# GrokImageCompression/Grok

Measured on NVIDIA H100. Metric: Mpixels/s encode+decode 8K RGB 12-bit HTJ2K; DWT HBM GB/s vs roofline, higher is better.
Workload: dtype i32

## Files before the change

### grok_b200/csrc/dwt.cu

```cuda
#include "b2k_internal.h"

namespace {

__device__ __noinline__ int mirror_rel_slow(int t, int n)
{
  if(n == 1)
    return 0;
  const int period = 2 * (n - 1);
  t %= period;
  if(t < 0)
    t += period;
  return t < n ? t : period - t;
}
__device__ __forceinline__ int mirror_rel(int t, int n)
{
  if((unsigned)t < (unsigned)n)
    return t;
  const int r = t < 0 ? -t : 2 * (n - 1) - t;
  if((unsigned)r < (unsigned)n)
    return r;
  return mirror_rel_slow(t, n);
}

__device__ __forceinline__ void load8_w32(const int32_t* __restrict__ row, int rel, int n, int (&v)[8])
{
  const int32_t* p = row + rel;
  if(rel >= 0 && rel + 8 <= n && ((reinterpret_cast<uintptr_t>(p) & 15) == 0))
  {
    const int4 a = __ldg(reinterpret_cast<const int4*>(p));
    const int4 b = __ldg(reinterpret_cast<const int4*>(p) + 1);
    v[0] = a.x; v[1] = a.y; v[2] = a.z; v[3] = a.w;
    v[4] = b.x; v[5] = b.y; v[6] = b.z; v[7] = b.w;
  }
  else
  {
#pragma unroll
    for(int i = 0; i < 8; ++i)
      v[i] = __ldg(row + mirror_rel(rel + i, n));
  }
}

__device__ __forceinline__ void load4_band(const int32_t* __restrict__ row, int k0, int kb0, int u0, int u1, int odd,
                                           int (&v)[4])
{
  const int ufirst = 2 * k0 + odd, ulast = ufirst + 6;
  const int32_t* p = row + (k0 - kb0);
  if(ufirst >= u0 && ulast < u1 && ((reinterpret_cast<uintptr_t>(p) & 15) == 0))
  {
    const int4 a = __ldg(reinterpret_cast<const int4*>(p));
    v[0] = a.x; v[1] = a.y; v[2] = a.z; v[3] = a.w;
  }
  else
  {
    const int n = u1 - u0;
#pragma unroll
    for(int i = 0; i < 4; ++i)
    {
      const int um = u0 + mirror_rel(ufirst + 2 * i - u0, n);
      v[i] = ((um & 1) == odd) ? __ldg(row + ((um >> 1) - kb0)) : 0;
    }
  }
}

struct Job
{
  int lane, ulane, jbeg, jend, wn, hn, nvalid;
  bool owner, need;
};
__device__ __forceinline__ bool decode_job(const DwtLevelDesc& D, Job& J)
{
  J.lane = threadIdx.x & 31;
  const int job = blockIdx.x * B2K_WARPS_PER_CTA + (threadIdx.x >> 5);
  if(job >= (int)D.nstrips * (int)D.nsegs)
    return false;
  const int strip = job % D.nstrips, seg = job / D.nstrips;
  J.wn = D.u1 - D.u0;
  J.hn = D.v1 - D.v0;
  J.nvalid = D.strip_w >> 3;
  J.ulane = (D.u0 & ~7) + strip * (int)D.strip_w + (J.lane - 1) * 8;
  J.owner = J.lane >= 1 && J.lane <= J.nvalid && J.ulane < D.u1;
  J.need = J.lane <= J.nvalid + 1 && J.ulane < D.u1 + 8;
  const int jlo = D.v0 >> 1, jhi = (D.v1 - 1) >> 1;
  J.jbeg = jlo + seg * (int)D.pairs_per_seg;
  J.jend = min(J.jbeg + (int)D.pairs_per_seg, jhi + 1);
  return true;
}

template <int NC, int N>
__device__ __forceinline__ void rct_fwd(const DwtLevelDesc& D, int (&x)[NC][N])
{
#pragma unroll
  for(int i = 0; i < N; ++i)
  {
    if constexpr(NC == 3)
    {
      const int r = x[0][i] + D.shift[0], g = x[1][i] + D.shift[1], b = x[2][i] + D.shift[2];
      x[0][i] = ((g + g) + b + r) >> 2;
      x[1][i] = b - g;
      x[2][i] = r - g;
    }
    else
      x[0][i] += D.shift[0];
  }
}

template <int NC, int N>
__device__ __forceinline__ void ict_fwd(const DwtLevelDesc& D, const int (&x)[NC][N], float (&out)[NC][N])
{
  const float a_r = 0.299f, a_g = 0.587f, a_b = 0.114f;
  const float cb = __fdiv_rn(0.5f, __fsub_rn(1.0f, a_b)), cr = __fdiv_rn(0.5f, __fsub_rn(1.0f, a_r));
#pragma unroll
  for(int i = 0; i < N; ++i)
  {
    if constexpr(NC == 3)
    {
      const float r = (float)(x[0][i] + D.shift[0]), g = (float)(x[1][i] + D.shift[1]), b = (float)(x[2][i] + D.shift[2]);
      const float y = __fmaf_rn(a_b, b, __fmaf_rn(a_g, g, __fmul_rn(a_r, r)));
      out[0][i] = y;
      out[1][i] = __fmul_rn(cb, __fsub_rn(b, y));
      out[2][i] = __fmul_rn(cr, __fsub_rn(r, y));
    }
    else
      out[0][i] = (float)(x[0][i] + D.shift[0]);
  }
}

template <int NC, int N>
__device__ __forceinline__ void rct_inv(const DwtLevelDesc& D, int (&x)[NC][N])
{
#pragma unroll
  for(int i = 0; i < N; ++i)
  {
    if constexpr(NC == 3)
    {
      const int y = x[0][i], u = x[1][i], w = x[2][i];
      const int gg = y - ((u + w) >> 2);
      x[0][i] = w + gg;
      x[1][i] = gg;
      x[2][i] = u + gg;
    }
#pragma unroll
    for(int c = 0; c < NC; ++c)
      x[c][i] = min(max(x[c][i] - D.shift[c], D.lo[c]), D.hi[c]);
  }
}

template <int NC, int N>
__device__ __forceinline__ void ict_inv(const DwtLevelDesc& D, const float (&x)[NC][N], int (&out)[NC][N])
{
#pragma unroll
  for(int i = 0; i < N; ++i)
  {
    float f[NC];
    if constexpr(NC == 3)
    {
      const float y = x[0][i], u = x[1][i], w = x[2][i];
      f[0] = __fmaf_rn(w, 1.402f, y);
      f[1] = __fmaf_rn(-w, 0.71414f, __fmaf_rn(-u, 0.34413f, y));
      f[2] = __fmaf_rn(u, 1.772f, y);
    }
    else
      f[0] = x[0][i];
#pragma unroll
    for(int c = 0; c < NC; ++c)
      out[c][i] = min(max(__float2int_rn(f[c]) - D.shift[c], D.lo[c]), D.hi[c]);
  }
}

template <int NC>
__device__ __forceinline__ void fetch_int_rows(const DwtLevelDesc& D, const Job& J, int v, int (&out)[NC][8])
{
  const int r = mirror_rel(v - D.v0, J.hn);
#pragma unroll
  for(int c = 0; c < NC; ++c)
  {
    if(!J.need)
    {
#pragma unroll
      for(int i = 0; i < 8; ++i)
        out[c][i] = 0;
      continue;
    }
    load8_w32(reinterpret_cast<const int32_t*>(D.in[c]) + (size_t)r * D.in_pitch, J.ulane - D.u0, J.wn, out[c]);
  }
}

template <int NC>
__device__ __forceinline__ void to_coeffs53(const DwtLevelDesc& D, int (&x)[NC][8])
{
  if(D.first_level)
    rct_fwd<NC>(D, x);
}

template <int NC>
__device__ __forceinline__ void to_coeffs97(const DwtLevelDesc& D, const int (&raw)[NC][8], float (&out)[NC][8])
{
  if(D.first_level)
    ict_fwd<NC>(D, raw, out);
  else
  {
#pragma unroll
    for(int c = 0; c < NC; ++c)
#pragma unroll
      for(int i = 0; i < 8; ++i)
        out[c][i] = __int_as_float(raw[c][i]);
  }
}

template <int NC>
__device__ __forceinline__ void fetch53(const DwtLevelDesc& D, const Job& J, int v, int (&out)[NC][8])
{
  fetch_int_rows<NC>(D, J, v, out);
  to_coeffs53<NC>(D, out);
}

template <int NC>
__device__ __forceinline__ void fetch97(const DwtLevelDesc& D, const Job& J, int v, float (&out)[NC][8])
{
  int raw[NC][8];
  fetch_int_rows<NC>(D, J, v, raw);
  to_coeffs97<NC>(D, raw, out);
}

struct BandGeom
{
  int x0l, x0h, y0l, y0h, snx, sny;
};
__device__ __forceinline__ BandGeom band_geom(const DwtLevelDesc& D)
{
  BandGeom g;
  g.x0l = (D.u0 + 1) >> 1;
  g.x0h = D.u0 >> 1;
  g.y0l = (D.v0 + 1) >> 1;
  g.y0h = D.v0 >> 1;
  g.snx = ((D.u1 + 1) >> 1) - g.x0l;
  g.sny = ((D.v1 + 1) >> 1) - g.y0l;
  return g;
}

struct StoreCtx
{
  unsigned mlo, mhi;
  bool vec_ll, vec_lo, vec_hi;
  int col_ll, col_lo, col_hi;
};
__device__ __forceinline__ StoreCtx store_ctx(const DwtLevelDesc& D, const Job& J, const BandGeom& g)
{
  StoreCtx s;
  s.mlo = s.mhi = 0;
  if(J.owner)
  {
#pragma unroll
    for(int i = 0; i < 4; ++i)
    {
      const int ue = J.ulane + 2 * i;
      if(ue >= D.u0 && ue < D.u1)
        s.mlo |= 1u << i;
      if(ue + 1 >= D.u0 && ue + 1 < D.u1)
        s.mhi |= 1u << i;
    }
  }
  const int k0 = J.ulane >> 1;
  s.col_ll = k0 - g.x0l;
  s.col_lo = k0 - g.x0l;
  s.col_hi = g.snx + k0 - g.x0h;
  const bool pitch_ok = ((D.ll_pitch | D.c_pitch) & 3u) == 0;
  s.vec_ll = pitch_ok && s.mlo == 0xF && (((reinterpret_cast<uintptr_t>(D.out_ll[0]) >> 2) + (unsigned)s.col_ll) & 3u) == 0;
  s.vec_lo = pitch_ok && s.mlo == 0xF && (((reinterpret_cast<uintptr_t>(D.out_c[0]) >> 2) + (unsigned)s.col_lo) & 3u) == 0;
  s.vec_hi = pitch_ok && s.mhi == 0xF && (((reinterpret_cast<uintptr_t>(D.out_c[0]) >> 2) + (unsigned)s.col_hi) & 3u) == 0;
  return s;
}
__device__ __forceinline__ void store4v(int32_t* __restrict__ p, const int (&v)[4], unsigned mask, bool vec)
{
  if(vec)
    *reinterpret_cast<int4*>(p) = make_int4(v[0], v[1], v[2], v[3]);
  else
  {
#pragma unroll
    for(int i = 0; i < 4; ++i)
      if(mask & (1u << i))
        p[i] = v[i];
  }
}
__device__ __forceinline__ void store_rows(const DwtLevelDesc& D, const BandGeom& g, const StoreCtx& S, int c, int j,
                                           bool vhigh, const int (&lo)[4], const int (&hi)[4])
{
  const int v = 2 * j + (vhigh ? 1 : 0);
  if(v < D.v0 || v >= D.v1 || (S.mlo | S.mhi) == 0)
    return;
  if(!vhigh)
  {
    const int r = j - g.y0l;
    store4v(reinterpret_cast<int32_t*>(D.out_ll[c]) + (r * (int)D.ll_pitch + S.col_ll), lo, S.mlo, S.vec_ll);
    store4v(reinterpret_cast<int32_t*>(D.out_c[c]) + (r * (int)D.c_pitch + S.col_hi), hi, S.mhi, S.vec_hi);
  }
  else
  {
    const int r = g.sny + j - g.y0h;
    int32_t* crow = reinterpret_cast<int32_t*>(D.out_c[c]) + r * (int)D.c_pitch;
    store4v(crow + S.col_lo, lo, S.mlo, S.vec_lo);
    store4v(crow + S.col_hi, hi, S.mhi, S.vec_hi);
  }
}

template <bool DEGEN = true>
__device__ __forceinline__ void hfwd53(const int (&r)[8], int wn, int (&lo)[4], int (&hi)[4])
{
  const int en = __shfl_down_sync(0xffffffffu, r[0], 1);
  hi[0] = r[1] - ((r[0] + r[2]) >> 1);
  hi[1] = r[3] - ((r[2] + r[4]) >> 1);
  hi[2] = r[5] - ((r[4] + r[6]) >> 1);
  hi[3] = r[7] - ((r[6] + en) >> 1);
  const int dp = __shfl_up_sync(0xffffffffu, hi[3], 1);
  lo[0] = r[0] + ((dp + hi[0] + 2) >> 2);
  lo[1] = r[2] + ((hi[0] + hi[1] + 2) >> 2);
  lo[2] = r[4] + ((hi[1] + hi[2] + 2) >> 2);
  lo[3] = r[6] + ((hi[2] + hi[3] + 2) >> 2);
  if(DEGEN && wn == 1)
  {
#pragma unroll
    for(int i = 0; i < 4; ++i)
    {
      lo[i] = r[2 * i];
      hi[i] = r[2 * i + 1] << 1;
    }
  }
}

#define F97_ALPHA (-1.586134342f)
#define F97_BETA (-0.052980118f)
#define F97_GAMMA (0.882911075f)
#define F97_DELTA (0.443506852f)
#define F97_K (1.230174105f)

__device__ __forceinline__ void hfwd97(const float (&r)[8], int wn, float invK, float deltaS, int (&lo)[4],
                                       int (&hi)[4])
{
  float e[5], d[4], s[5];
#pragma unroll
  for(int i = 0; i < 4; ++i)
    e[i] = r[2 * i];
  e[4] = __shfl_down_sync(0xffffffffu, r[0], 1);
#pragma unroll
  for(int i = 0; i < 4; ++i)
    d[i] = fmaf(e[i] + e[i + 1], F97_ALPHA, r[2 * i + 1]);
  float dm = __shfl_up_sync(0xffffffffu, d[3], 1);
  s[0] = fmaf(dm + d[0], F97_BETA, e[0]);
#pragma unroll
  for(int i = 1; i < 4; ++i)
    s[i] = fmaf(d[i - 1] + d[i], F97_BETA, e[i]);
  s[4] = __shfl_down_sync(0xffffffffu, s[0], 1);
#pragma unroll
  for(int i = 0; i < 4; ++i)
    d[i] = __fmul_rn(fmaf(s[i] + s[i + 1], F97_GAMMA, d[i]), F97_K);
  dm = __shfl_up_sync(0xffffffffu, d[3], 1);
  float o0 = __fmul_rn(fmaf(dm + d[0], deltaS, s[0]), invK);
  lo[0] = __float_as_int(o0);
#pragma unroll
  for(int i = 1; i < 4; ++i)
    lo[i] = __float_as_int(__fmul_rn(fmaf(d[i - 1] + d[i], deltaS, s[i]), invK));
#pragma unroll
  for(int i = 0; i < 4; ++i)
    hi[i] = __float_as_int(d[i]);
  if(wn == 1)
  {
#pragma unroll
    for(int i = 0; i < 4; ++i)
    {
      lo[i] = __float_as_int(r[2 * i]);
      hi[i] = __float_as_int(__fmul_rn(r[2 * i + 1], 2.0f));
    }
  }
}

__device__ __forceinline__ void cp_async16(void* smem_dst, const void* gmem_src)
{
  const unsigned s = (unsigned)__cvta_generic_to_shared(smem_dst);
  asm volatile("cp.async.cg.shared.global [%0], [%1], 16;" ::"r"(s), "l"(gmem_src) : "memory");
}
__device__ __forceinline__ void cp_async4(void* smem_dst, const void* gmem_src)
{
  const unsigned s = (unsigned)__cvta_generic_to_shared(smem_dst);
  asm volatile("cp.async.ca.shared.global [%0], [%1], 4;" ::"r"(s), "l"(gmem_src) : "memory");
}
__device__ __forceinline__ void cp_async_commit() { asm volatile("cp.async.commit_group;" ::: "memory"); }
template <int N>
__device__ __forceinline__ void cp_async_wait()
{
  asm volatile("cp.async.wait_group %0;" ::"n"(N) : "memory");
}

__device__ __forceinline__ void mbar_init(uint64_t* bar, unsigned count)
{
  asm volatile("mbarrier.init.shared::cta.b64 [%0], %1;" ::"r"((unsigned)__cvta_generic_to_shared(bar)), "r"(count) : "memory");
}
__device__ __forceinline__ void mbar_fence_init() { asm volatile("fence.mbarrier_init.release.cluster;" ::: "memory"); }
__device__ __forceinline__ void mbar_expect_tx(uint64_t* bar, unsigned bytes)
{
  asm volatile("mbarrier.arrive.expect_tx.shared::cta.b64 _, [%0], %1;" ::"r"((unsigned)__cvta_generic_to_shared(bar)), "r"(bytes)
               : "memory");
}
__device__ __forceinline__ void bulk_g2s(void* smem_dst, const void* gmem_src, unsigned bytes, uint64_t* bar)
{
  asm volatile("cp.async.bulk.shared::cluster.global.mbarrier::complete_tx::bytes [%0], [%1], %2, [%3];" ::"r"(
                   (unsigned)__cvta_generic_to_shared(smem_dst)),
               "l"(gmem_src), "r"(bytes), "r"((unsigned)__cvta_generic_to_shared(bar))
               : "memory");
}
__device__ __forceinline__ void mbar_wait(uint64_t* bar, unsigned parity)
{
  asm volatile("{\n"
               ".reg .pred p;\n"
               "MBAR_WAIT_%=:\n"
               "mbarrier.try_wait.parity.shared::cta.b64 p, [%0], %1;\n"
               "@p bra MBAR_DONE_%=;\n"
               "bra MBAR_WAIT_%=;\n"
               "MBAR_DONE_%=:\n"
               "}" ::"r"((unsigned)__cvta_generic_to_shared(bar)),
               "r"(parity)
               : "memory");
}

constexpr int DWT_STAGES = 3;

template <class Stage>
struct WarpPipe
{
  static constexpr size_t SLOT_BYTES = (size_t)B2K_WARPS_PER_CTA * DWT_STAGES * Stage::PAIRB;
  static constexpr size_t SMEM_BYTES = SLOT_BYTES + (size_t)B2K_WARPS_PER_CTA * DWT_STAGES * sizeof(uint64_t);

  uint8_t* slots;
  uint64_t* bars;
  int tfirst, tlast, tfill;
  bool bulk;

  __device__ __forceinline__ WarpPipe(uint8_t* smem, bool bulk_, int tfirst_, int tlast_)
      : slots(smem + (size_t)(threadIdx.x >> 5) * DWT_STAGES * Stage::PAIRB),
        bars(reinterpret_cast<uint64_t*>(smem + SLOT_BYTES) + (threadIdx.x >> 5) * DWT_STAGES), tfirst(tfirst_),
        tlast(tlast_), tfill(tfirst_), bulk(bulk_)
  {
  }
  template <class Bulk, class Async>
  __device__ __forceinline__ void refill(const Bulk& fill_bulk, const Async& fill_async)
  {
    if(tfill <= tlast)
    {
      const int slot = (tfill - tfirst) % DWT_STAGES;
      uint8_t* st = slots + (size_t)slot * Stage::PAIRB;
      if(bulk)
      {
        if((threadIdx.x & 31) == 0)
        {
          mbar_expect_tx(bars + slot, Stage::PAIRB);
          fill_bulk(st, tfill, bars + slot);
        }
      }
      else
        fill_async(st, tfill);
    }
    cp_async_commit();
    ++tfill;
  }
  template <class Bulk, class Async>
  __device__ __forceinline__ void prime(const Bulk& fill_bulk, const Async& fill_async)
  {
    if(bulk)
    {
      if((threadIdx.x & 31) == 0)
      {
#pragma unroll
        for(int s = 0; s < DWT_STAGES; ++s)
          mbar_init(bars + s, 1);
        mbar_fence_init();
      }
      __syncwarp();
    }
#pragma unroll
    for(int s = 0; s < DWT_STAGES - 1; ++s)
      refill(fill_bulk, fill_async);
  }
  template <class Bulk, class Async>
  __device__ __forceinline__ const uint8_t* acquire(int t, const Bulk& fill_bulk, const Async& fill_async)
  {
    if(Stage::COOPERATIVE || bulk)
      __syncwarp();
    refill(fill_bulk, fill_async);
    const int k = t - tfirst;
    if(bulk)
      mbar_wait(bars + k % DWT_STAGES, (unsigned)((k / DWT_STAGES) & 1));
    else
    {
      cp_async_wait<DWT_STAGES - 1>();
      if(Stage::COOPERATIVE)
        __syncwarp();
    }
    return slots + (size_t)(k % DWT_STAGES) * Stage::PAIRB;
  }
  __device__ __forceinline__ void drain() const { cp_async_wait<0>(); }
};

template <int NC>
struct RowStage
{
  static constexpr int ROWB = 1024;
  static constexpr int PAIRB = 2 * NC * ROWB;
  static constexpr bool COOPERATIVE = true;
  static __device__ __forceinline__ int swz(int k) { return k ^ ((k >> 3) & 1); }

  static __device__ __forceinline__ void fill(uint8_t* stage, int which, const DwtLevelDesc& D, const Job& J, int v,
                                              bool fast, unsigned fastmask, const int (&mcol)[8])
  {
    const int r = mirror_rel(v - D.v0, J.hn);
    const int rel = J.ulane - D.u0;
#pragma unroll
    for(int c = 0; c < NC; ++c)
    {
      uint8_t* dst = stage + (which * NC + c) * ROWB;
      const int32_t* row = reinterpret_cast<const int32_t*>(D.in[c]) + (size_t)r * D.in_pitch;
      const int rel0 = rel - 8 * J.lane;
#pragma unroll
      for(int h = 0; h < 2; ++h)
      {
        const int k = J.lane + 32 * h;
        if((fastmask >> (k >> 1)) & 1u)
          cp_async16(dst + swz(k) * 16, row + rel0 + 4 * k);
      }
      if(J.need && !fast)
      {
        uint8_t* d0 = dst + swz(2 * J.lane) * 16;
        uint8_t* d1 = dst + swz(2 * J.lane + 1) * 16;
#pragma unroll
        for(int i = 0; i < 4; ++i)
        {
          cp_async4(d0 + 4 * i, row + mcol[i]);
          cp_async4(d1 + 4 * i, row + mcol[4 + i]);
        }
      }
    }
  }
  static __device__ __forceinline__ void fill_bulk(uint8_t* stage, int which, const DwtLevelDesc& D, const Job& J, int v, uint64_t* bar)
  {
    const int r = mirror_rel(v - D.v0, J.hn);
    const int rel0 = J.ulane - D.u0 - 8 * J.lane;
#pragma unroll
    for(int c = 0; c < NC; ++c)
      bulk_g2s(stage + (which * NC + c) * ROWB, reinterpret_cast<const int32_t*>(D.in[c]) + (size_t)r * D.in_pitch + rel0, ROWB, bar);
  }
  static __device__ __forceinline__ void read(const uint8_t* stage, int which, const Job& J, bool linear, int (&out)[NC][8])
  {
#pragma unroll
    for(int c = 0; c < NC; ++c)
    {
      const uint8_t* row = stage + (which * NC + c) * ROWB;
      int4 a, b;
      if(linear)
      {
        a = *reinterpret_cast<const int4*>(row + J.lane * 32);
        b = *reinterpret_cast<const int4*>(row + J.lane * 32 + 16);
      }
      else
      {
        a = *reinterpret_cast<const int4*>(row + swz(2 * J.lane) * 16);
        b = *reinterpret_cast<const int4*>(row + swz(2 * J.lane + 1) * 16);
      }
      out[c][0] = a.x; out[c][1] = a.y; out[c][2] = a.z; out[c][3] = a.w;
      out[c][4] = b.x; out[c][5] = b.y; out[c][6] = b.z; out[c][7] = b.w;
    }
  }
  static __device__ __forceinline__ bool lane_fast(const DwtLevelDesc& D, const Job& J)
  {
    const int rel = J.ulane - D.u0;
    bool ok = J.need && rel >= 0 && rel + 8 <= J.wn && (D.in_pitch & 3u) == 0;
#pragma unroll
    for(int c = 0; c < NC; ++c)
      ok = ok && (((reinterpret_cast<uintptr_t>(D.in[c]) + (size_t)rel * 4) & 15) == 0);
    return ok;
  }
};

template <int NC>
__device__ __noinline__ void fwd53_degenerate_job(const DwtLevelDesc* __restrict__ dptr, const Job J)
{
  const DwtLevelDesc& D = *dptr;
  const BandGeom g = band_geom(D);
  int E[NC][8], DP[NC][8];
  {
    int A[NC][8], B[NC][8];
    fetch53<NC>(D, J, 2 * J.jbeg - 2, A);
    fetch53<NC>(D, J, 2 * J.jbeg - 1, B);
    fetch53<NC>(D, J, 2 * J.jbeg, E);
#pragma unroll
    for(int c = 0; c < NC; ++c)
#pragma unroll
      for(int i = 0; i < 8; ++i)
        DP[c][i] = B[c][i] - ((A[c][i] + E[c][i]) >> 1);
  }
  for(int j = J.jbeg; j < J.jend; ++j)
  {
    int O[NC][8], E2[NC][8];
    fetch53<NC>(D, J, 2 * j + 1, O);
    fetch53<NC>(D, J, 2 * j + 2, E2);
#pragma unroll 1
    for(int c = 0; c < NC; ++c)
    {
      int s[8], d[8];
#pragma unroll
      for(int i = 0; i < 8; ++i)
      {
        d[i] = O[c][i] - ((E[c][i] + E2[c][i]) >> 1);
        s[i] = E[c][i] + ((DP[c][i] + d[i] + 2) >> 2);
        if(J.hn == 1)
        {
          s[i] = E[c][i];
          d[i] = O[c][i] << 1;
        }
        DP[c][i] = d[i];
        E[c][i] = E2[c][i];
      }
      int lo[4], hi[4];
      hfwd53<true>(s, J.wn, lo, hi);
      store_rows(D, g, store_ctx(D, J, g), c, j, false, lo, hi);
      hfwd53<true>(d, J.wn, lo, hi);
      store_rows(D, g, store_ctx(D, J, g), c, j, true, lo, hi);
    }
  }
}

template <int NC>
__global__ void __launch_bounds__(B2K_WARPS_PER_CTA * 32) k_dwt53_fwd(const DwtLevelDesc* __restrict__ descs)
{
  extern __shared__ __align__(16) uint8_t smem_dwt[];
  typedef RowStage<NC> RS;
  const DwtLevelDesc D = descs[blockIdx.y];
  Job J;
  if(!decode_job(D, J))
    return;
  if(J.hn == 1 || J.wn == 1)
  {
    fwd53_degenerate_job<NC>(descs + blockIdx.y, J);
    return;
  }
  const BandGeom g = band_geom(D);
  const StoreCtx SC = store_ctx(D, J, g);
  const bool fast = RS::lane_fast(D, J);
  const unsigned fastmask = __ballot_sync(0xffffffffu, fast);
  int mcol[8];
#pragma unroll
  for(int i = 0; i < 8; ++i)
    mcol[i] = mirror_rel(J.ulane - D.u0 + i, J.wn);

  const int tfirst = J.jbeg - 1, tlast = J.jend - 1;
  WarpPipe<RS> pipe(smem_dwt, fastmask == 0xffffffffu, tfirst, tlast);
  auto fill_bulk = [&](uint8_t* st, int tf, uint64_t* bar) {
    RS::fill_bulk(st, 0, D, J, 2 * tf + 1, bar);
    RS::fill_bulk(st, 1, D, J, 2 * tf + 2, bar);
  };
  auto fill_async = [&](uint8_t* st, int tf) {
    RS::fill(st, 0, D, J, 2 * tf + 1, fast, fastmask, mcol);
    RS::fill(st, 1, D, J, 2 * tf + 2, fast, fastmask, mcol);
  };
  pipe.prime(fill_bulk, fill_async);
  int E[NC][8], DP[NC][8];
  fetch53<NC>(D, J, 2 * tfirst, E);
#pragma unroll
  for(int c = 0; c < NC; ++c)
#pragma unroll
    for(int i = 0; i < 8; ++i)
      DP[c][i] = 0;

  for(int t = tfirst; t <= tlast; ++t)
  {
    const uint8_t* st = pipe.acquire(t, fill_bulk, fill_async);
    int O[NC][8], E2[NC][8];
    RS::read(st, 0, J, pipe.bulk, O);
    RS::read(st, 1, J, pipe.bulk, E2);
    to_coeffs53<NC>(D, O);
    to_coeffs53<NC>(D, E2);
    const bool emit = t >= J.jbeg;
#pragma unroll
    for(int c = 0; c < NC; ++c)
    {
      int s[8], d[8];
#pragma unroll
      for(int i = 0; i < 8; ++i)
      {
        d[i] = O[c][i] - ((E[c][i] + E2[c][i]) >> 1);
        s[i] = E[c][i] + ((DP[c][i] + d[i] + 2) >> 2);
        DP[c][i] = d[i];
        E[c][i] = E2[c][i];
      }
      if(emit)
      {
        int lo[4], hi[4];
        hfwd53<false>(s, J.wn, lo, hi);
        store_rows(D, g, SC, c, t, false, lo, hi);
        hfwd53<false>(d, J.wn, lo, hi);
        store_rows(D, g, SC, c, t, true, lo, hi);
      }
    }
  }
  pipe.drain();
}

template <int NC>
__device__ __noinline__ void fwd97_degenerate_job(const DwtLevelDesc* __restrict__ dptr, const Job J)
{
  const DwtLevelDesc& D = *dptr;
  const BandGeom g = band_geom(D);
  const float invK = (float)(1.0 / 1.230174105);
  const float deltaS = __fmul_rn(F97_DELTA, invK);

  float Ev[NC][8], D1[NC][8], S1[NC][8], D2[NC][8];
  fetch97<NC>(D, J, 2 * (J.jbeg - 2), Ev);
#pragma unroll
  for(int c = 0; c < NC; ++c)
#pragma unroll
    for(int i = 0; i < 8; ++i)
      D1[c][i] = S1[c][i] = D2[c][i] = 0.f;

  for(int t = J.jbeg - 2; t <= J.jend; ++t)
  {
    float O[NC][8], E2[NC][8];
    fetch97<NC>(D, J, 2 * t + 1, O);
    fetch97<NC>(D, J, 2 * t + 2, E2);
    const bool emit = (t - 1) >= J.jbeg;
#pragma unroll
    for(int c = 0; c < NC; ++c)
    {
      float lowrow[8], highrow[8];
#pragma unroll
      for(int i = 0; i < 8; ++i)
      {
        const float d1 = fmaf(Ev[c][i] + E2[c][i], F97_ALPHA, O[c][i]);
        const float s1 = fmaf(D1[c][i] + d1, F97_BETA, Ev[c][i]);
        const float d2 = __fmul_rn(fmaf(S1[c][i] + s1, F97_GAMMA, D1[c][i]), F97_K);
        const float s2 = __fmul_rn(fmaf(D2[c][i] + d2, deltaS, S1[c][i]), invK);
        lowrow[i] = s2;
        highrow[i] = d2;
        if(J.hn == 1)
        {
          lowrow[i] = Ev[c][i];
          highrow[i] = __fmul_rn(O[c][i], 2.0f);
        }
        D2[c][i] = d2;
        D1[c][i] = d1;
        S1[c][i] = s1;
        Ev[c][i] = E2[c][i];
      }
      int lo[4], hi[4];
      hfwd97(lowrow, J.wn, invK, deltaS, lo, hi);
      if(emit)
        store_rows(D, g, store_ctx(D, J, g), c, t - 1, false, lo, hi);
      hfwd97(highrow, J.wn, invK, deltaS, lo, hi);
      if(emit)
        store_rows(D, g, store_ctx(D, J, g), c, t - 1, true, lo, hi);
    }
  }
}

template <int NC>
__global__ void __launch_bounds__(B2K_WARPS_PER_CTA * 32) k_dwt97_fwd(const DwtLevelDesc* __restrict__ descs)
{
  extern __shared__ __align__(16) uint8_t smem_dwt[];
  typedef RowStage<NC> RS;
  const DwtLevelDesc D = descs[blockIdx.y];
  Job J;
  if(!decode_job(D, J))
    return;
  if(J.hn == 1 || J.wn == 1)
  {
    fwd97_degenerate_job<NC>(descs + blockIdx.y, J);
    return;
  }
  const BandGeom g = band_geom(D);
  const StoreCtx SC = store_ctx(D, J, g);
  const bool fast = RS::lane_fast(D, J);
  const unsigned fastmask = __ballot_sync(0xffffffffu, fast);
  int mcol[8];
#pragma unroll
  for(int i = 0; i < 8; ++i)
    mcol[i] = mirror_rel(J.ulane - D.u0 + i, J.wn);
  const float invK = (float)(1.0 / 1.230174105);
  const float deltaS = __fmul_rn(F97_DELTA, invK);

  const int tfirst = J.jbeg - 2, tlast = J.jend;
  WarpPipe<RS> pipe(smem_dwt, fastmask == 0xffffffffu, tfirst, tlast);
  auto fill_bulk = [&](uint8_t* st, int tf, uint64_t* bar) {
    RS::fill_bulk(st, 0, D, J, 2 * tf + 1, bar);
    RS::fill_bulk(st, 1, D, J, 2 * tf + 2, bar);
  };
  auto fill_async = [&](uint8_t* st, int tf) {
    RS::fill(st, 0, D, J, 2 * tf + 1, fast, fastmask, mcol);
    RS::fill(st, 1, D, J, 2 * tf + 2, fast, fastmask, mcol);
  };
  pipe.prime(fill_bulk, fill_async);
  float Ev[NC][8], D1[NC][8], S1[NC][8], D2[NC][8];
  fetch97<NC>(D, J, 2 * tfirst, Ev);
#pragma unroll
  for(int c = 0; c < NC; ++c)
#pragma unroll
    for(int i = 0; i < 8; ++i)
      D1[c][i] = S1[c][i] = D2[c][i] = 0.f;

  for(int t = tfirst; t <= tlast; ++t)
  {
    const uint8_t* st = pipe.acquire(t, fill_bulk, fill_async);
    float O[NC][8], E2[NC][8];
    {
      int raw[NC][8];
      RS::read(st, 0, J, pipe.bulk, raw);
      to_coeffs97<NC>(D, raw, O);
      RS::read(st, 1, J, pipe.bulk, raw);
      to_coeffs97<NC>(D, raw, E2);
    }
    const bool emit = (t - 1) >= J.jbeg;
#pragma unroll
    for(int c = 0; c < NC; ++c)
    {
      float lowrow[8], highrow[8];
#pragma unroll
      for(int i = 0; i < 8; ++i)
      {
        const float d1 = fmaf(Ev[c][i] + E2[c][i], F97_ALPHA, O[c][i]);
        const float s1 = fmaf(D1[c][i] + d1, F97_BETA, Ev[c][i]);
        const float d2 = __fmul_rn(fmaf(S1[c][i] + s1, F97_GAMMA, D1[c][i]), F97_K);
        const float s2 = __fmul_rn(fmaf(D2[c][i] + d2, deltaS, S1[c][i]), invK);
        lowrow[i] = s2;
        highrow[i] = d2;
        D2[c][i] = d2;
        D1[c][i] = d1;
        S1[c][i] = s1;
        Ev[c][i] = E2[c][i];
      }
      if(emit)
      {
        int lo[4], hi[4];
        hfwd97(lowrow, 2, invK, deltaS, lo, hi);
        store_rows(D, g, SC, c, t - 1, false, lo, hi);
        hfwd97(highrow, 2, invK, deltaS, lo, hi);
        store_rows(D, g, SC, c, t - 1, true, lo, hi);
      }
    }
  }
  pipe.drain();
}

template <int NC>
__device__ __forceinline__ void fetch_band_rows(const DwtLevelDesc& D, const Job& J, const BandGeom& g, int j,
                                                bool vhigh, int (&lo)[NC][4], int (&hi)[NC][4])
{
  const int vm = D.v0 + mirror_rel(2 * j + (vhigh ? 1 : 0) - D.v0, J.hn);
  const int jm = vm >> 1;
  const int k0 = J.ulane >> 1;
#pragma unroll
  for(int c = 0; c < NC; ++c)
  {
    if(!J.need || (vm & 1) != (vhigh ? 1 : 0))
    {
#pragma unroll
      for(int i = 0; i < 4; ++i)
        lo[c][i] = hi[c][i] = 0;
      continue;
    }
    const int32_t* lrow;
    const int32_t* hrow;
    if(!vhigh)
    {
      lrow = reinterpret_cast<const int32_t*>(D.out_ll[c]) + (size_t)(jm - g.y0l) * D.ll_pitch;
      hrow = reinterpret_cast<const int32_t*>(D.out_c[c]) + (size_t)(jm - g.y0l) * D.c_pitch + g.snx;
    }
    else
    {
      lrow = reinterpret_cast<const int32_t*>(D.out_c[c]) + (size_t)(g.sny + jm - g.y0h) * D.c_pitch;
      hrow = lrow + g.snx;
    }
    load4_band(lrow, k0, g.x0l, D.u0, D.u1, 0, lo[c]);
    load4_band(hrow, k0, g.x0h, D.u0, D.u1, 1, hi[c]);
  }
}

template <bool DEGEN = true>
__device__ __forceinline__ void hinv53(const int (&lo)[4], const int (&hi)[4], int wn, int (&r)[8])
{
  const int dm = __shfl_up_sync(0xffffffffu, hi[3], 1);
  int e[5];
  e[0] = lo[0] - ((dm + hi[0] + 2) >> 2);
  e[1] = lo[1] - ((hi[0] + hi[1] + 2) >> 2);
  e[2] = lo[2] - ((hi[1] + hi[2] + 2) >> 2);
  e[3] = lo[3] - ((hi[2] + hi[3] + 2) >> 2);
  e[4] = __shfl_down_sync(0xffffffffu, e[0], 1);
#pragma unroll
  for(int i = 0; i < 4; ++i)
  {
    r[2 * i] = e[i];
    r[2 * i + 1] = hi[i] + ((e[i] + e[i + 1]) >> 1);
  }
  if(DEGEN && wn == 1)
  {
#pragma unroll
    for(int i = 0; i < 4; ++i)
    {
      r[2 * i] = lo[i];
      r[2 * i + 1] = hi[i] >> 1;
    }
  }
}

__device__ __forceinline__ void hinv97(const int (&loi)[4], const int (&hii)[4], int wn, float (&r)[8])
{
  const float K = 1.230174105f, twice_invK = 1.625732422f;
  float s[5], d[4];
#pragma unroll
  for(int i = 0; i < 4; ++i)
  {
    s[i] = __fmul_rn(__int_as_float(loi[i]), K);
    d[i] = __fmul_rn(__int_as_float(hii[i]), twice_invK);
  }
  float dm = __shfl_up_sync(0xffffffffu, d[3], 1);
  s[0] = fmaf(dm + d[0], -0.443506852f, s[0]);
#pragma unroll
  for(int i = 1; i < 4; ++i)
    s[i] = fmaf(d[i - 1] + d[i], -0.443506852f, s[i]);
  s[4] = __shfl_down_sync(0xffffffffu, s[0], 1);
#pragma unroll
  for(int i = 0; i < 4; ++i)
    d[i] = fmaf(s[i] + s[i + 1], -0.882911075f, d[i]);
  dm = __shfl_up_sync(0xffffffffu, d[3], 1);
  s[0] = fmaf(dm + d[0], 0.052980118f, s[0]);
#pragma unroll
  for(int i = 1; i < 4; ++i)
    s[i] = fmaf(d[i - 1] + d[i], 0.052980118f, s[i]);
  s[4] = __shfl_down_sync(0xffffffffu, s[0], 1);
#pragma unroll
  for(int i = 0; i < 4; ++i)
  {
    r[2 * i] = s[i];
    r[2 * i + 1] = fmaf(s[i] + s[i + 1], 1.586134342f, d[i]);
  }
  if(wn == 1)
  {
#pragma unroll
    for(int i = 0; i < 4; ++i)
    {
      r[2 * i] = __int_as_float(loi[i]);
      r[2 * i + 1] = __int_as_float(hii[i]);
    }
  }
}

struct OutCtx
{
  unsigned m;
  bool vec;
  int col;
};
__device__ __forceinline__ OutCtx out_ctx(const DwtLevelDesc& D, const Job& J)
{
  OutCtx o;
  o.m = 0;
  if(J.owner)
  {
#pragma unroll
    for(int i = 0; i < 8; ++i)
      if(J.ulane + i >= D.u0 && J.ulane + i < D.u1)
        o.m |= 1u << i;
  }
  o.col = J.ulane - D.u0;
  o.vec = o.m == 0xFF && (D.in_pitch & 3u) == 0 && (((reinterpret_cast<uintptr_t>(D.in[0]) >> 2) + (unsigned)o.col) & 3u) == 0;
  return o;
}
template <int NC>
__device__ __forceinline__ void store_out_rows(const DwtLevelDesc& D, const OutCtx& O, int v, const int (&x)[NC][8])
{
#pragma unroll
  for(int c = 0; c < NC; ++c)
  {
    int32_t* p = reinterpret_cast<int32_t*>(const_cast<void*>(D.in[c])) + ((v - D.v0) * (int)D.in_pitch + O.col);
    if(O.vec)
    {
      reinterpret_cast<int4*>(p)[0] = make_int4(x[c][0], x[c][1], x[c][2], x[c][3]);
      reinterpret_cast<int4*>(p)[1] = make_int4(x[c][4], x[c][5], x[c][6], x[c][7]);
    }
    else
    {
#pragma unroll
      for(int i = 0; i < 8; ++i)
        if(O.m & (1u << i))
          p[i] = x[c][i];
    }
  }
}
template <int NC>
__device__ __forceinline__ void store_rows53(const DwtLevelDesc& D, const OutCtx& O, int v, int (&x)[NC][8])
{
  if(v < D.v0 || v >= D.v1 || O.m == 0)
    return;
  if(D.first_level)
    rct_inv<NC>(D, x);
  store_out_rows<NC>(D, O, v, x);
}
template <int NC>
__device__ __forceinline__ void store_rows97(const DwtLevelDesc& D, const OutCtx& O, int v, const float (&x)[NC][8])
{
  if(v < D.v0 || v >= D.v1 || O.m == 0)
    return;
  int o[NC][8];
  if(D.first_level)
    ict_inv<NC>(D, x, o);
  else
  {
#pragma unroll
    for(int c = 0; c < NC; ++c)
#pragma unroll
      for(int i = 0; i < 8; ++i)
        o[c][i] = __float_as_int(x[c][i]);
  }
  store_out_rows<NC>(D, O, v, o);
}

template <int NC>
__device__ __noinline__ void inv53_degenerate_job(const DwtLevelDesc* __restrict__ dptr, const Job J)
{
  const DwtLevelDesc& D = *dptr;
  const BandGeom g = band_geom(D);
  int DV[NC][8], EP[NC][8];
#pragma unroll
  for(int c = 0; c < NC; ++c)
#pragma unroll
    for(int i = 0; i < 8; ++i)
      DV[c][i] = EP[c][i] = 0;

  for(int t = J.jbeg - 1; t <= J.jend; ++t)
  {
    int lo[NC][4], hi[NC][4];
    int sv[NC][8], dv[NC][8];
    fetch_band_rows<NC>(D, J, g, t, false, lo, hi);
#pragma unroll
    for(int c = 0; c < NC; ++c)
      hinv53(lo[c], hi[c], J.wn, sv[c]);
    fetch_band_rows<NC>(D, J, g, t, true, lo, hi);
#pragma unroll
    for(int c = 0; c < NC; ++c)
      hinv53(lo[c], hi[c], J.wn, dv[c]);
    int Er[NC][8], Or[NC][8];
#pragma unroll
    for(int c = 0; c < NC; ++c)
#pragma unroll
      for(int i = 0; i < 8; ++i)
      {
        const int e = sv[c][i] - ((DV[c][i] + dv[c][i] + 2) >> 2);
        Or[c][i] = DV[c][i] + ((EP[c][i] + e) >> 1);
        Er[c][i] = EP[c][i];
        EP[c][i] = e;
        DV[c][i] = dv[c][i];
      }
    if(J.hn == 1)
    {
      if(t >= J.jbeg && t < J.jend)
      {
        int hv[NC][8];
#pragma unroll
        for(int c = 0; c < NC; ++c)
#pragma unroll
          for(int i = 0; i < 8; ++i)
            hv[c][i] = dv[c][i] >> 1;
        store_rows53<NC>(D, out_ctx(D, J), 2 * t, sv);
        store_rows53<NC>(D, out_ctx(D, J), 2 * t + 1, hv);
      }
    }
    else if(t - 1 >= J.jbeg)
    {
      store_rows53<NC>(D, out_ctx(D, J), 2 * (t - 1), Er);
      store_rows53<NC>(D, out_ctx(D, J), 2 * (t - 1) + 1, Or);
    }
  }
}


template <int NC>
struct BandStage
{
  static constexpr int ROWB = 512;
  static constexpr int PAIRB = 4 * NC * ROWB;
  static constexpr bool COOPERATIVE = false;
  struct Lane
  {
    bool need;
    bool fast[4];
    int col[4];
    int mlo[4], mhi[4];
  };
  static __device__ __forceinline__ void setup(const DwtLevelDesc& D, const Job& J, const BandGeom& g, Lane& L)
  {
    const int k0 = J.ulane >> 1;
    L.need = J.need;
#pragma unroll
    for(int i = 0; i < 4; ++i)
    {
      const int ul = D.u0 + mirror_rel(2 * (k0 + i) - D.u0, J.wn), uh = D.u0 + mirror_rel(2 * (k0 + i) + 1 - D.u0, J.wn);
      L.mlo[i] = (ul >> 1) - g.x0l;
      L.mhi[i] = (uh >> 1) - g.x0h;
    }
    const bool in_lo = 2 * k0 >= D.u0 && 2 * k0 + 6 < D.u1, in_hi = 2 * k0 + 1 >= D.u0 && 2 * k0 + 7 < D.u1;
    const int clo = k0 - g.x0l, chi = k0 - g.x0h;
    L.col[0] = clo; L.col[1] = g.snx + chi; L.col[2] = clo; L.col[3] = g.snx + chi;
    const bool pitch_ok = ((D.ll_pitch | D.c_pitch) & 3u) == 0;
    L.fast[0] = J.need && pitch_ok && in_lo && (((reinterpret_cast<uintptr_t>(D.out_ll[0]) >> 2) + (unsigned)clo) & 3u) == 0;
    L.fast[1] = J.need && pitch_ok && in_hi && (((reinterpret_cast<uintptr_t>(D.out_c[0]) >> 2) + (unsigned)(g.snx + chi)) & 3u) == 0;
    L.fast[2] = J.need && pitch_ok && in_lo && (((reinterpret_cast<uintptr_t>(D.out_c[0]) >> 2) + (unsigned)clo) & 3u) == 0;
    L.fast[3] = L.fast[1];
  }
  static __device__ __forceinline__ void fill(uint8_t* stage, const DwtLevelDesc& D, const Job& J, const BandGeom& g,
                                              const Lane& L, int t)
  {
    if(!L.need)
      return;
    const int jl = ((D.v0 + mirror_rel(2 * t - D.v0, J.hn)) >> 1), jh = ((D.v0 + mirror_rel(2 * t + 1 - D.v0, J.hn)) >> 1);
#pragma unroll
    for(int c = 0; c < NC; ++c)
    {
      const int32_t* src[4];
      src[0] = reinterpret_cast<const int32_t*>(D.out_ll[c]) + (jl - g.y0l) * (int)D.ll_pitch;
      src[1] = reinterpret_cast<const int32_t*>(D.out_c[c]) + (jl - g.y0l) * (int)D.c_pitch;
      src[2] = reinterpret_cast<const int32_t*>(D.out_c[c]) + (g.sny + jh - g.y0h) * (int)D.c_pitch;
      src[3] = src[2];
#pragma unroll
      for(int b = 0; b < 4; ++b)
      {
        uint8_t* dst = stage + (b * NC + c) * ROWB + J.lane * 16;
        if(L.fast[b])
          cp_async16(dst, src[b] + L.col[b]);
        else
        {
          const int base = (b & 1) ? g.snx : 0;
#pragma unroll
          for(int i = 0; i < 4; ++i)
            cp_async4(dst + 4 * i, src[b] + base + ((b & 1) ? L.mhi[i] : L.mlo[i]));
        }
      }
    }
  }
  static __device__ __forceinline__ void fill_bulk(uint8_t* stage, const DwtLevelDesc& D, const Job& J, const BandGeom& g,
                                                   const Lane& L, int t, uint64_t* bar)
  {
    const int jl = ((D.v0 + mirror_rel(2 * t - D.v0, J.hn)) >> 1), jh = ((D.v0 + mirror_rel(2 * t + 1 - D.v0, J.hn)) >> 1);
#pragma unroll
    for(int c = 0; c < NC; ++c)
    {
      const int32_t* src[4];
      src[0] = reinterpret_cast<const int32_t*>(D.out_ll[c]) + (jl - g.y0l) * (int)D.ll_pitch;
      src[1] = reinterpret_cast<const int32_t*>(D.out_c[c]) + (jl - g.y0l) * (int)D.c_pitch;
      src[2] = reinterpret_cast<const int32_t*>(D.out_c[c]) + (g.sny + jh - g.y0h) * (int)D.c_pitch;
      src[3] = src[2];
#pragma unroll
      for(int b = 0; b < 4; ++b)
        bulk_g2s(stage + (b * NC + c) * ROWB, src[b] + L.col[b], ROWB, bar);
    }
  }
  static __device__ __forceinline__ bool all_fast(const Lane& L)
  {
    return __all_sync(0xffffffffu, L.fast[0] && L.fast[1] && L.fast[2] && L.fast[3]);
  }
  static __device__ __forceinline__ void read(const uint8_t* stage, const Job& J, int b, int c, int (&v)[4])
  {
    const int4 a = *reinterpret_cast<const int4*>(stage + (b * NC + c) * ROWB + J.lane * 16);
    v[0] = a.x; v[1] = a.y; v[2] = a.z; v[3] = a.w;
  }
};

template <int NC>
__global__ void __launch_bounds__(B2K_WARPS_PER_CTA * 32) k_dwt53_inv(const DwtLevelDesc* __restrict__ descs)
{
  extern __shared__ __align__(16) uint8_t smem_dwt[];
  typedef BandStage<NC> BS;
  const DwtLevelDesc D = descs[blockIdx.y];
  Job J;
  if(!decode_job(D, J))
    return;
  if(J.hn == 1 || J.wn == 1)
  {
    inv53_degenerate_job<NC>(descs + blockIdx.y, J);
    return;
  }
  const BandGeom g = band_geom(D);
  typename BS::Lane L;
  BS::setup(D, J, g, L);
  const OutCtx OC = out_ctx(D, J);

  const int tfirst = J.jbeg - 1, tlast = J.jend;
  WarpPipe<BS> pipe(smem_dwt, BS::all_fast(L), tfirst, tlast);
  auto fill_bulk = [&](uint8_t* st, int tf, uint64_t* bar) { BS::fill_bulk(st, D, J, g, L, tf, bar); };
  auto fill_async = [&](uint8_t* st, int tf) { BS::fill(st, D, J, g, L, tf); };
  pipe.prime(fill_bulk, fill_async);
  int DV[NC][8], EP[NC][8];
#pragma unroll
  for(int c = 0; c < NC; ++c)
#pragma unroll
    for(int i = 0; i < 8; ++i)
      DV[c][i] = EP[c][i] = 0;

  for(int t = tfirst; t <= tlast; ++t)
  {
    const uint8_t* st = pipe.acquire(t, fill_bulk, fill_async);
    int Er[NC][8], Or[NC][8];
#pragma unroll
    for(int c = 0; c < NC; ++c)
    {
      int lo[4], hi[4], sv[8], dv[8];
      BS::read(st, J, 0, c, lo);
      BS::read(st, J, 1, c, hi);
      hinv53<false>(lo, hi, J.wn, sv);
      BS::read(st, J, 2, c, lo);
      BS::read(st, J, 3, c, hi);
      hinv53<false>(lo, hi, J.wn, dv);
#pragma unroll
      for(int i = 0; i < 8; ++i)
      {
        const int e = sv[i] - ((DV[c][i] + dv[i] + 2) >> 2);
        Or[c][i] = DV[c][i] + ((EP[c][i] + e) >> 1);
        Er[c][i] = EP[c][i];
        EP[c][i] = e;
        DV[c][i] = dv[i];
      }
    }
    if(t - 1 >= J.jbeg)
    {
      store_rows53<NC>(D, OC, 2 * (t - 1), Er);
      store_rows53<NC>(D, OC, 2 * (t - 1) + 1, Or);
    }
  }
  pipe.drain();
}

template <int NC>
__device__ __noinline__ void inv97_degenerate_job(const DwtLevelDesc* __restrict__ dptr, const Job J)
{
  const DwtLevelDesc& D = *dptr;
  const BandGeom g = band_geom(D);
  const float K = 1.230174105f, twice_invK = 1.625732422f;
  float D0[NC][8], S1[NC][8], D1[NC][8], S2[NC][8];
#pragma unroll
  for(int c = 0; c < NC; ++c)
#pragma unroll
    for(int i = 0; i < 8; ++i)
      D0[c][i] = S1[c][i] = D1[c][i] = S2[c][i] = 0.f;

  for(int t = J.jbeg - 2; t <= J.jend + 1; ++t)
  {
    int lo[NC][4], hi[NC][4];
    float sv[NC][8], dv[NC][8];
    fetch_band_rows<NC>(D, J, g, t, false, lo, hi);
#pragma unroll
    for(int c = 0; c < NC; ++c)
      hinv97(lo[c], hi[c], J.wn, sv[c]);
    fetch_band_rows<NC>(D, J, g, t, true, lo, hi);
#pragma unroll
    for(int c = 0; c < NC; ++c)
      hinv97(lo[c], hi[c], J.wn, dv[c]);
    float Er[NC][8], Or[NC][8];
#pragma unroll
    for(int c = 0; c < NC; ++c)
#pragma unroll
      for(int i = 0; i < 8; ++i)
      {
        const float s0 = __fmul_rn(sv[c][i], K), d0 = __fmul_rn(dv[c][i], twice_invK);
        const float s1 = fmaf(D0[c][i] + d0, -0.443506852f, s0);
        const float d1 = fmaf(S1[c][i] + s1, -0.882911075f, D0[c][i]);
        const float s2 = fmaf(D1[c][i] + d1, 0.052980118f, S1[c][i]);
        const float d2 = fmaf(S2[c][i] + s2, 1.586134342f, D1[c][i]);
        Er[c][i] = S2[c][i];
        Or[c][i] = d2;
        D0[c][i] = d0;
        S1[c][i] = s1;
        D1[c][i] = d1;
        S2[c][i] = s2;
      }
    if(J.hn == 1)
    {
      if(t >= J.jbeg && t < J.jend)
      {
        store_rows97<NC>(D, out_ctx(D, J), 2 * t, sv);
        store_rows97<NC>(D, out_ctx(D, J), 2 * t + 1, dv);
      }
    }
    else if(t - 2 >= J.jbeg)
    {
      store_rows97<NC>(D, out_ctx(D, J), 2 * (t - 2), Er);
      store_rows97<NC>(D, out_ctx(D, J), 2 * (t - 2) + 1, Or);
    }
  }
}

template <int NC>
__global__ void __launch_bounds__(B2K_WARPS_PER_CTA * 32) k_dwt97_inv(const DwtLevelDesc* __restrict__ descs)
{
  extern __shared__ __align__(16) uint8_t smem_dwt[];
  typedef BandStage<NC> BS;
  const DwtLevelDesc D = descs[blockIdx.y];
  Job J;
  if(!decode_job(D, J))
    return;
  if(J.hn == 1 || J.wn == 1)
  {
    inv97_degenerate_job<NC>(descs + blockIdx.y, J);
    return;
  }
  const BandGeom g = band_geom(D);
  typename BS::Lane L;
  BS::setup(D, J, g, L);
  const OutCtx OC = out_ctx(D, J);
  const float K = 1.230174105f, twice_invK = 1.625732422f;

  const int tfirst = J.jbeg - 2, tlast = J.jend + 1;
  WarpPipe<BS> pipe(smem_dwt, BS::all_fast(L), tfirst, tlast);
  auto fill_bulk = [&](uint8_t* st, int tf, uint64_t* bar) { BS::fill_bulk(st, D, J, g, L, tf, bar); };
  auto fill_async = [&](uint8_t* st, int tf) { BS::fill(st, D, J, g, L, tf); };
  pipe.prime(fill_bulk, fill_async);
  float D0[NC][8], S1[NC][8], D1[NC][8], S2[NC][8];
#pragma unroll
  for(int c = 0; c < NC; ++c)
#pragma unroll
    for(int i = 0; i < 8; ++i)
      D0[c][i] = S1[c][i] = D1[c][i] = S2[c][i] = 0.f;

  for(int t = tfirst; t <= tlast; ++t)
  {
    const uint8_t* st = pipe.acquire(t, fill_bulk, fill_async);
    float Er[NC][8], Or[NC][8];
#pragma unroll
    for(int c = 0; c < NC; ++c)
    {
      int lo[4], hi[4];
      float sv[8], dv[8];
      BS::read(st, J, 0, c, lo);
      BS::read(st, J, 1, c, hi);
      hinv97(lo, hi, 2, sv);
      BS::read(st, J, 2, c, lo);
      BS::read(st, J, 3, c, hi);
      hinv97(lo, hi, 2, dv);
#pragma unroll
      for(int i = 0; i < 8; ++i)
      {
        const float s0 = __fmul_rn(sv[i], K), d0 = __fmul_rn(dv[i], twice_invK);
        const float s1 = fmaf(D0[c][i] + d0, -0.443506852f, s0);
        const float d1 = fmaf(S1[c][i] + s1, -0.882911075f, D0[c][i]);
        const float s2 = fmaf(D1[c][i] + d1, 0.052980118f, S1[c][i]);
        const float d2 = fmaf(S2[c][i] + s2, 1.586134342f, D1[c][i]);
        Er[c][i] = S2[c][i];
        Or[c][i] = d2;
        D0[c][i] = d0;
        S1[c][i] = s1;
        D1[c][i] = d1;
        S2[c][i] = s2;
      }
    }
    if(t - 2 >= J.jbeg)
    {
      store_rows97<NC>(D, OC, 2 * (t - 2), Er);
      store_rows97<NC>(D, OC, 2 * (t - 2) + 1, Or);
    }
  }
  pipe.drain();
}

template <int S> struct Sample;
template <> struct Sample<1> { typedef uint8_t U; typedef int8_t I; };
template <> struct Sample<2> { typedef uint16_t U; typedef int16_t I; };
template <> struct Sample<4> { typedef uint32_t U; typedef int32_t I; };

template <int S>
__device__ __forceinline__ int widen_sample(uint32_t u, int sgnd)
{
  if constexpr(S == 4)
    return (int)u;
  else
  {
    u &= (1u << (8 * S)) - 1;
    return sgnd ? (int)(typename Sample<S>::I)u : (int)u;
  }
}

template <int BYTES>
__device__ __forceinline__ void load_group(const void* p, uint32_t (&wd)[BYTES / 4])
{
  if constexpr(BYTES % 16 == 0)
  {
#pragma unroll
    for(int i = 0; i < BYTES / 16; ++i)
    {
      const uint4 a = __ldg(reinterpret_cast<const uint4*>(p) + i);
      wd[4 * i] = a.x; wd[4 * i + 1] = a.y; wd[4 * i + 2] = a.z; wd[4 * i + 3] = a.w;
    }
  }
  else
  {
#pragma unroll
    for(int i = 0; i < BYTES / 8; ++i)
    {
      const uint2 a = __ldg(reinterpret_cast<const uint2*>(p) + i);
      wd[2 * i] = a.x; wd[2 * i + 1] = a.y;
    }
  }
}
template <int BYTES>
__device__ __forceinline__ void store_group(void* p, const uint32_t (&wd)[BYTES / 4])
{
  if constexpr(BYTES % 16 == 0)
  {
#pragma unroll
    for(int i = 0; i < BYTES / 16; ++i)
      reinterpret_cast<uint4*>(p)[i] = make_uint4(wd[4 * i], wd[4 * i + 1], wd[4 * i + 2], wd[4 * i + 3]);
  }
  else
  {
#pragma unroll
    for(int i = 0; i < BYTES / 8; ++i)
      reinterpret_cast<uint2*>(p)[i] = make_uint2(wd[2 * i], wd[2 * i + 1]);
  }
}

struct Ptr4
{
  int32_t* p[4];
};
struct CPtr4
{
  const int32_t* p[4];
};

template <int S, int NC>
__global__ void __launch_bounds__(128) k_container_to_planes(const void* __restrict__ src, uint32_t spitch, uint32_t step, Ptr4 dst,
                                                             uint32_t dpitch, uint32_t w, uint32_t h, int sgnd)
{
  typedef typename Sample<S>::U U;
  constexpr int BYTES = 8 * NC * S, V = BYTES % 16 == 0 ? 16 : 8;
  const uint32_t x8 = (blockIdx.x * blockDim.x + threadIdx.x) * 8;
  if(x8 >= w)
    return;
  for(uint32_t y = blockIdx.y; y < h; y += gridDim.y)
  {
    const U* s = static_cast<const U*>(src) + (size_t)y * spitch + (size_t)x8 * step;
    const size_t doff = (size_t)y * dpitch + x8;
    bool vec = x8 + 8 <= w && step == NC && (reinterpret_cast<uintptr_t>(s) & (V - 1)) == 0;
#pragma unroll
    for(int c = 0; c < NC; ++c)
      vec = vec && (reinterpret_cast<uintptr_t>(dst.p[c] + doff) & 15) == 0;
    if(vec)
    {
      uint32_t wd[BYTES / 4];
      load_group<BYTES>(s, wd);
#pragma unroll
      for(int c = 0; c < NC; ++c)
      {
        int v[8];
#pragma unroll
        for(int i = 0; i < 8; ++i)
        {
          const int e = (i * NC + c) * S;
          v[i] = widen_sample<S>(wd[e >> 2] >> ((e & 3) * 8), sgnd);
        }
        int4* d = reinterpret_cast<int4*>(dst.p[c] + doff);
        d[0] = make_int4(v[0], v[1], v[2], v[3]);
        d[1] = make_int4(v[4], v[5], v[6], v[7]);
      }
    }
    else
    {
      const uint32_t n = w - x8 < 8 ? w - x8 : 8;
#pragma unroll 1
      for(uint32_t i = 0; i < n; ++i)
#pragma unroll
        for(int c = 0; c < NC; ++c)
          dst.p[c][doff + i] = widen_sample<S>(s[(size_t)i * step + c], sgnd);
    }
  }
}

template <int S, int NC>
__global__ void __launch_bounds__(128) k_planes_to_container(CPtr4 src, uint32_t spitch, void* __restrict__ dst, uint32_t dpitch,
                                                             uint32_t step, uint32_t w, uint32_t h)
{
  typedef typename Sample<S>::U U;
  constexpr int BYTES = 8 * NC * S, V = BYTES % 16 == 0 ? 16 : 8;
  constexpr uint32_t MASK = S == 4 ? 0xFFFFFFFFu : (1u << (8 * S)) - 1;
  const uint32_t x8 = (blockIdx.x * blockDim.x + threadIdx.x) * 8;
  if(x8 >= w)
    return;
  for(uint32_t y = blockIdx.y; y < h; y += gridDim.y)
  {
    const size_t soff = (size_t)y * spitch + x8;
    U* d = static_cast<U*>(dst) + (size_t)y * dpitch + (size_t)x8 * step;
    bool vec = x8 + 8 <= w && step == NC && (reinterpret_cast<uintptr_t>(d) & (V - 1)) == 0;
#pragma unroll
    for(int c = 0; c < NC; ++c)
      vec = vec && (reinterpret_cast<uintptr_t>(src.p[c] + soff) & 15) == 0;
    if(vec)
    {
      uint32_t wd[BYTES / 4];
#pragma unroll
      for(int k = 0; k < BYTES / 4; ++k)
        wd[k] = 0;
#pragma unroll
      for(int c = 0; c < NC; ++c)
      {
        const int4 a = __ldg(reinterpret_cast<const int4*>(src.p[c] + soff)), b = __ldg(reinterpret_cast<const int4*>(src.p[c] + soff) + 1);
        const int v[8] = {a.x, a.y, a.z, a.w, b.x, b.y, b.z, b.w};
#pragma unroll
        for(int i = 0; i < 8; ++i)
        {
          const int e = (i * NC + c) * S;
          wd[e >> 2] |= ((uint32_t)v[i] & MASK) << ((e & 3) * 8);
        }
      }
      store_group<BYTES>(d, wd);
    }
    else
    {
      const uint32_t n = w - x8 < 8 ? w - x8 : 8;
#pragma unroll 1
      for(uint32_t i = 0; i < n; ++i)
#pragma unroll
        for(int c = 0; c < NC; ++c)
          d[(size_t)i * step + c] = (U)src.p[c][soff + i];
    }
  }
}

dim3 convert_grid(uint32_t w, uint32_t h) { return dim3((w + 8 * 128 - 1) / (8 * 128), h < 65535u ? h : 65535u); }

template <int S>
void launch_container_to_planes(const void* src, uint32_t spitch, uint32_t step, const Ptr4& P, int nc, uint32_t dpitch, uint32_t w,
                                uint32_t h, int sgnd, cudaStream_t st)
{
  const dim3 grid = convert_grid(w, h), block(128);
  switch(nc)
  {
    case 1: k_container_to_planes<S, 1><<<grid, block, 0, st>>>(src, spitch, step, P, dpitch, w, h, sgnd); break;
    case 2: k_container_to_planes<S, 2><<<grid, block, 0, st>>>(src, spitch, step, P, dpitch, w, h, sgnd); break;
    case 3: k_container_to_planes<S, 3><<<grid, block, 0, st>>>(src, spitch, step, P, dpitch, w, h, sgnd); break;
    default: k_container_to_planes<S, 4><<<grid, block, 0, st>>>(src, spitch, step, P, dpitch, w, h, sgnd); break;
  }
}
template <int S>
void launch_planes_to_container(const CPtr4& P, int nc, uint32_t spitch, void* dst, uint32_t dpitch, uint32_t step, uint32_t w,
                                uint32_t h, cudaStream_t st)
{
  const dim3 grid = convert_grid(w, h), block(128);
  switch(nc)
  {
    case 1: k_planes_to_container<S, 1><<<grid, block, 0, st>>>(P, spitch, dst, dpitch, step, w, h); break;
    case 2: k_planes_to_container<S, 2><<<grid, block, 0, st>>>(P, spitch, dst, dpitch, step, w, h); break;
    case 3: k_planes_to_container<S, 3><<<grid, block, 0, st>>>(P, spitch, dst, dpitch, step, w, h); break;
    default: k_planes_to_container<S, 4><<<grid, block, 0, st>>>(P, spitch, dst, dpitch, step, w, h); break;
  }
}

}

void b2k_launch_container_to_planes(const void* src, uint32_t spitch, uint32_t step, uint32_t sample_bytes, int32_t* const* dst, int nc,
                                    uint32_t dpitch, uint32_t w, uint32_t h, int sgnd, cudaStream_t st)
{
  if(!w || !h)
    return;
  Ptr4 P{};
  for(int c = 0; c < nc && c < 4; ++c)
    P.p[c] = dst[c];
  switch(sample_bytes)
  {
    case 1: launch_container_to_planes<1>(src, spitch, step, P, nc, dpitch, w, h, sgnd, st); break;
    case 2: launch_container_to_planes<2>(src, spitch, step, P, nc, dpitch, w, h, sgnd, st); break;
    default: launch_container_to_planes<4>(src, spitch, step, P, nc, dpitch, w, h, sgnd, st); break;
  }
  b2k_count_launch();
}
void b2k_launch_planes_to_container(const int32_t* const* src, int nc, uint32_t spitch, void* dst, uint32_t dpitch, uint32_t step,
                                    uint32_t sample_bytes, uint32_t w, uint32_t h, cudaStream_t st)
{
  if(!w || !h)
    return;
  CPtr4 P{};
  for(int c = 0; c < nc && c < 4; ++c)
    P.p[c] = src[c];
  switch(sample_bytes)
  {
    case 1: launch_planes_to_container<1>(P, nc, spitch, dst, dpitch, step, w, h, st); break;
    case 2: launch_planes_to_container<2>(P, nc, spitch, dst, dpitch, step, w, h, st); break;
    default: launch_planes_to_container<4>(P, nc, spitch, dst, dpitch, step, w, h, st); break;
  }
  b2k_count_launch();
}

template <class Stage, void (*KERNEL)(const DwtLevelDesc*)>
static void launch_dwt(dim3 grid, dim3 block, cudaStream_t st, const DwtLevelDesc* d)
{
  const size_t smem = WarpPipe<Stage>::SMEM_BYTES;
  static DeviceOnce once;
  once.run([&] { cudaFuncSetAttribute(KERNEL, cudaFuncAttributeMaxDynamicSharedMemorySize, (int)smem); });
  KERNEL<<<grid, block, smem, st>>>(d);
}

void b2k_launch_dwt_fwd(const DwtLevelDesc* d, int ndesc, int max_jobs, int nc, bool irreversible, cudaStream_t st)
{
  if(ndesc <= 0 || max_jobs <= 0)
    return;
  dim3 grid((max_jobs + B2K_WARPS_PER_CTA - 1) / B2K_WARPS_PER_CTA, ndesc), block(B2K_WARPS_PER_CTA * 32);
  if(!irreversible)
  {
    if(nc == 3) launch_dwt<RowStage<3>, k_dwt53_fwd<3>>(grid, block, st, d);
    else launch_dwt<RowStage<1>, k_dwt53_fwd<1>>(grid, block, st, d);
  }
  else
  {
    if(nc == 3) launch_dwt<RowStage<3>, k_dwt97_fwd<3>>(grid, block, st, d);
    else launch_dwt<RowStage<1>, k_dwt97_fwd<1>>(grid, block, st, d);
  }
  b2k_count_launch();
}

template <int NC, bool IRREV, bool FWD>
__global__ void k_point_transform(const DwtLevelDesc* __restrict__ descs, int ndesc)
{
  for(int di = blockIdx.z; di < ndesc; di += gridDim.z)
  {
  const DwtLevelDesc& D = descs[di];
  const int w = D.u1 - D.u0, h = D.v1 - D.v0;
  const int x = blockIdx.x * blockDim.x + threadIdx.x;
  if(x >= w)
    continue;
  for(int y = blockIdx.y; y < h; y += gridDim.y)
  {
  const size_t ii = (size_t)y * D.in_pitch + x, oi = (size_t)y * D.c_pitch + x;
  if(FWD)
  {
    int v[NC][1];
#pragma unroll
    for(int c = 0; c < NC; ++c)
      v[c][0] = static_cast<const int32_t*>(D.in[c])[ii];
    if(!IRREV)
    {
      rct_fwd<NC>(D, v);
#pragma unroll
      for(int c = 0; c < NC; ++c)
        static_cast<int32_t*>(D.out_c[c])[oi] = v[c][0];
    }
    else
    {
      float f[NC][1];
      ict_fwd<NC>(D, v, f);
#pragma unroll
      for(int c = 0; c < NC; ++c)
        static_cast<float*>(D.out_c[c])[oi] = f[c][0];
    }
  }
  else
  {
    int o[NC][1];
    if(!IRREV)
    {
#pragma unroll
      for(int c = 0; c < NC; ++c)
        o[c][0] = static_cast<const int32_t*>(D.out_c[c])[oi];
      rct_inv<NC>(D, o);
    }
    else
    {
      float f[NC][1];
#pragma unroll
      for(int c = 0; c < NC; ++c)
        f[c][0] = static_cast<const float*>(D.out_c[c])[oi];
      ict_inv<NC>(D, f, o);
    }
#pragma unroll
    for(int c = 0; c < NC; ++c)
      static_cast<int32_t*>(const_cast<void*>(D.in[c]))[ii] = o[c][0];
  }
  }
  }
}

void b2k_launch_point_transform(const DwtLevelDesc* d, int ndesc, uint32_t max_w, uint32_t max_h, int nc, bool irreversible,
                                bool forward, cudaStream_t st)
{
  if(ndesc <= 0 || !max_w || !max_h)
    return;
  dim3 grid((max_w + 127) / 128, std::min<uint32_t>(max_h, 65535u), (unsigned)std::min(ndesc, 65535)), block(128);
#define B2K_PT(NC_, IR_, FW_) k_point_transform<NC_, IR_, FW_><<<grid, block, 0, st>>>(d, ndesc)
  if(nc == 3)
  {
    if(irreversible) { if(forward) B2K_PT(3, true, true); else B2K_PT(3, true, false); }
    else { if(forward) B2K_PT(3, false, true); else B2K_PT(3, false, false); }
  }
  else
  {
    if(irreversible) { if(forward) B2K_PT(1, true, true); else B2K_PT(1, true, false); }
    else { if(forward) B2K_PT(1, false, true); else B2K_PT(1, false, false); }
  }
#undef B2K_PT
  b2k_count_launch();
}

void b2k_launch_dwt_inv(const DwtLevelDesc* d, int ndesc, int max_jobs, int nc, bool irreversible, cudaStream_t st)
{
  if(ndesc <= 0 || max_jobs <= 0)
    return;
  dim3 grid((max_jobs + B2K_WARPS_PER_CTA - 1) / B2K_WARPS_PER_CTA, ndesc), block(B2K_WARPS_PER_CTA * 32);
  if(!irreversible)
  {
    if(nc == 3) launch_dwt<BandStage<3>, k_dwt53_inv<3>>(grid, block, st, d);
    else launch_dwt<BandStage<1>, k_dwt53_inv<1>>(grid, block, st, d);
  }
  else
  {
    if(nc == 3) launch_dwt<BandStage<3>, k_dwt97_inv<3>>(grid, block, st, d);
    else launch_dwt<BandStage<1>, k_dwt97_inv<1>>(grid, block, st, d);
  }
  b2k_count_launch();
}
```

### grok_b200/csrc/engine.cu

```cuda
#include <algorithm>
#include <atomic>
#include <chrono>
#include <cstdio>
#include <cstdlib>
#include <cstring>
#include <functional>
#include <map>
#include <mutex>
#include <unordered_map>
#include <string>
#include <vector>

#include "b2k_internal.h"
#include "geometry.h"

using namespace b2k;

static thread_local std::string g_err;
static std::atomic<uint64_t> g_launches{0};
static std::atomic<int> g_pack_policy{-1};
static std::atomic<int> g_last_pack[2]{{-1}, {-1}};
void b2k_count_launch(void) { g_launches.fetch_add(1, std::memory_order_relaxed); }

#define CUDA_TRY(expr)                                                                             \
  do                                                                                               \
  {                                                                                                \
    cudaError_t _e = (expr);                                                                       \
    if(_e != cudaSuccess)                                                                          \
    {                                                                                              \
      g_err = std::string(#expr) + ": " + cudaGetErrorString(_e);                                  \
      return -1;                                                                                   \
    }                                                                                              \
  } while(0)

struct b2k_engine
{
  int device = 0;
  cudaStream_t stream = nullptr, copy_stream = nullptr, h2d_stream = nullptr;
  cudaStream_t aux[4] = {nullptr, nullptr, nullptr, nullptr};
  cudaDeviceProp prop{};
  std::mutex mu;
  b2k_device_job* cached = nullptr;
  cudaEvent_t caller_ev = nullptr;
};

namespace {
struct DevCache
{
  std::mutex mu;
  std::multimap<size_t, void*> free_;
  std::unordered_map<void*, size_t> live;
  size_t cached = 0;
};
DevCache g_devcache[32];
size_t dev_cache_limit()
{
  static const size_t v = [] {
    const char* e = getenv("B2K_DEV_CACHE_GB");
    return (size_t)(e ? atof(e) : 16.0) << 30;
  }();
  return v;
}
cudaError_t dev_alloc(void** p, size_t n)
{
  int dev = 0;
  cudaGetDevice(&dev);
  DevCache& C = g_devcache[dev & 31];
  const size_t gran = std::max<size_t>(256u << 10, n >> 4);
  const size_t want = (n + gran - 1) / gran * gran;
  {
    std::lock_guard<std::mutex> lk(C.mu);
    auto it = C.free_.lower_bound(want);
    if(it != C.free_.end() && it->first <= want + want / 4)
    {
      *p = it->second;
      C.live[*p] = it->first;
      C.cached -= it->first;
      C.free_.erase(it);
      return cudaSuccess;
    }
  }
  cudaError_t e = cudaMalloc(p, want);
  if(e != cudaSuccess)
  {
    (void)cudaGetLastError();
    std::vector<void*> drop;
    {
      std::lock_guard<std::mutex> lk(C.mu);
      for(auto& kv : C.free_)
        drop.push_back(kv.second);
      C.free_.clear();
      C.cached = 0;
    }
    for(void* q : drop)
      cudaFree(q);
    e = cudaMalloc(p, want);
  }
  if(e == cudaSuccess)
  {
    std::lock_guard<std::mutex> lk(C.mu);
    C.live[*p] = want;
  }
  return e;
}
cudaError_t dev_free(void* p)
{
  if(!p)
    return cudaSuccess;
  int dev = 0;
  cudaGetDevice(&dev);
  DevCache& C = g_devcache[dev & 31];
  std::vector<void*> drop;
  {
    std::lock_guard<std::mutex> lk(C.mu);
    auto it = C.live.find(p);
    if(it == C.live.end())
      drop.push_back(p);
    else
    {
      C.free_.insert({it->second, p});
      C.cached += it->second;
      C.live.erase(it);
      while(C.cached > dev_cache_limit() && !C.free_.empty())
      {
        auto big = std::prev(C.free_.end());
        drop.push_back(big->second);
        C.cached -= big->first;
        C.free_.erase(big);
      }
    }
  }
  for(void* q : drop)
    cudaFree(q);
  return cudaSuccess;
}
}
template <class T>
static inline cudaError_t dev_alloc_t(T** p, size_t n) { return dev_alloc(reinterpret_cast<void**>(p), n); }

namespace {
struct HostCache
{
  std::mutex mu;
  std::multimap<size_t, void*> free_;
  std::unordered_map<void*, size_t> live;
  size_t cached = 0;
} g_hostcache;
cudaError_t host_alloc(void** p, size_t n)
{
  const size_t gran = std::max<size_t>(64u << 10, n >> 4);
  const size_t want = (n + gran - 1) / gran * gran;
  {
    std::lock_guard<std::mutex> lk(g_hostcache.mu);
    auto it = g_hostcache.free_.lower_bound(want);
    if(it != g_hostcache.free_.end() && it->first <= want + want / 4)
    {
      *p = it->second;
      g_hostcache.live[*p] = it->first;
      g_hostcache.cached -= it->first;
      g_hostcache.free_.erase(it);
      return cudaSuccess;
    }
  }
  const cudaError_t e = cudaHostAlloc(p, want, cudaHostAllocDefault);
  if(e == cudaSuccess)
  {
    std::lock_guard<std::mutex> lk(g_hostcache.mu);
    g_hostcache.live[*p] = want;
  }
  return e;
}
cudaError_t host_free(void* p)
{
  if(!p)
    return cudaSuccess;
  std::vector<void*> drop;
  {
    std::lock_guard<std::mutex> lk(g_hostcache.mu);
    auto it = g_hostcache.live.find(p);
    if(it == g_hostcache.live.end())
      drop.push_back(p);
    else
    {
      g_hostcache.free_.insert({it->second, p});
      g_hostcache.cached += it->second;
      g_hostcache.live.erase(it);
      while(g_hostcache.cached > ((size_t)8 << 30) && !g_hostcache.free_.empty())
      {
        auto big = std::prev(g_hostcache.free_.end());
        drop.push_back(big->second);
        g_hostcache.cached -= big->first;
        g_hostcache.free_.erase(big);
      }
    }
  }
  for(void* q : drop)
    cudaFreeHost(q);
  return cudaSuccess;
}
}
template <class T>
static inline cudaError_t host_alloc_t(T** p, size_t n) { return host_alloc(reinterpret_cast<void**>(p), n); }
#define cudaMalloc(p, n) dev_alloc_t((p), (n))
#define cudaFree(p) dev_free((void*)(p))
#define cudaHostAlloc(p, n, flags) host_alloc_t((p), (n))
#define cudaFreeHost(p) host_free((void*)(p))

struct Planes
{
  int32_t* base = nullptr;
  uint32_t pitch = 0, rows = 0;
  uint32_t X0 = 0, Y0 = 0;
  int n = 0;
  size_t plane_elems() const { return (size_t)pitch * rows; }
  int32_t* at(int c, uint32_t x, uint32_t y) const { return base + (size_t)c * plane_elems() + (size_t)(y - Y0) * pitch + (x - X0); }
};

static int alloc_planes(Planes& p, int n, uint32_t cx0, uint32_t cy0, uint32_t cx1, uint32_t cy1)
{
  p.n = n;
  p.X0 = cx0 & ~31u;
  p.Y0 = cy0;
  p.pitch = ((cx1 - p.X0) + 31u + 32u) & ~31u;
  p.rows = (cy1 - cy0) + 2;
  CUDA_TRY(cudaMalloc(&p.base, (size_t)n * p.plane_elems() * sizeof(int32_t)));
  CUDA_TRY(cudaMemset(p.base, 0, (size_t)n * p.plane_elems() * sizeof(int32_t)));
  return 0;
}

struct LevelLaunch
{
  std::vector<DwtLevelDesc> descs;
  DwtLevelDesc* d_descs = nullptr;
  int nc = 1, max_jobs = 0;
  bool point = false;
  uint32_t max_w = 0, max_h = 0;
  uint64_t alg_bytes = 0;
  std::vector<uint32_t> tile_first;
};

#define B2K_MAX_CHUNKS 32
#define CEV(purpose, k) ((purpose) * (B2K_MAX_CHUNKS + 1) + (int)(k))

struct PackTuner
{
  int calls = 0;
  double best[2] = {1e30, 1e30};
  double recent = 0;
  int choice = -1;
  bool probing_other = false;
  bool next_mode()
  {
    if(choice < 0)
      return (calls & 1) == 0;
    probing_other = (calls % 64) == 63;
    return probing_other ? !choice : (choice != 0);
  }
  void record(bool packed, double ms)
  {
    ++calls;
    if(choice < 0)
    {
      if(calls > 1 || !packed)
        best[packed ? 1 : 0] = std::min(best[packed ? 1 : 0], ms);
      if(calls >= 6)
      {
        choice = best[1] < best[0] ? 1 : 0;
        recent = best[choice];
      }
      return;
    }
    if(probing_other)
    {
      if(ms < 0.9 * recent)
      {
        choice = packed ? 1 : 0;
        recent = ms;
      }
      probing_other = false;
      return;
    }
    recent = 0.9 * recent + 0.1 * ms;
  }
};

struct b2k_device_job
{
  b2k_engine* eng = nullptr;
  b2k_coding cp{};
  uint32_t tile_mod = 1, tile_rem = 0;
  TileGrid grid{};
  std::vector<uint32_t> tiles;
  std::vector<Rect> tile_rects;
  std::vector<BandQuant> quant;
  std::vector<b2k_block> blocks;
  std::vector<uint32_t> coded_index;
  std::vector<float> dec_quant;
  std::vector<uint32_t> coded_first;
  std::vector<uint32_t> chunk_tile;
  cudaEvent_t chunk_ev[4 * (B2K_MAX_CHUNKS + 1)]{};
  uint32_t max_cblk_w = 0;
  HtEncodeLimits enc_limits{0, 0};

  Planes img, coef, ll[2];
  uint16_t* d_stage = nullptr;
  std::vector<LevelLaunch> fwd, inv;
  HtBlockDesc* d_enc_desc = nullptr;
  HtBlockDesc* d_dec_desc = nullptr;
  std::vector<HtBlockDesc> h_enc_desc;
  HtBlockDesc* h_dec_desc = nullptr;
  HtBlockOut* d_out = nullptr;
  uint64_t* d_offsets = nullptr;
  uint32_t* d_recs = nullptr;
  float* d_dec_quant = nullptr;
  HtBlockOut* d_dec_status = nullptr;
  uint64_t total_quads = 0, group_quads = 0;
  uint8_t* d_scratch = nullptr;
  uint64_t scratch_bytes = 0;
  uint8_t* d_bytes = nullptr;
  uint64_t bytes_cap = 0, bytes_used = 0;
  int* d_err = nullptr;
  HtBlockOut* h_out = nullptr;
  uint64_t* h_offsets = nullptr;
  cudaEvent_t ev[8]{};
  float last_level1_ms = 0.f, last_inv_level1_ms = 0.f;
  uint64_t level1_alg_bytes = 0;
  uint16_t* h_ring = nullptr;
  uint32_t ring_slots = 0;
  uint64_t ring_slot_elems = 0, ring_elems = 0;
  cudaEvent_t ring_ev[16]{};
  PackTuner tune_enc, tune_dec;
  std::vector<cudaEvent_t> q_ev;
  std::vector<cudaEvent_t> p_ev;
  std::vector<cudaStream_t> p_streams;
  bool dec_has_refinement = false;
};

extern "C" const char* b2k_last_error(void) { return g_err.c_str(); }
void b2k_set_error(const char* msg) { g_err = msg ? msg : ""; }
extern "C" uint64_t b2k_launch_count(void) { return g_launches.load(); }

extern "C" int32_t b2k_engine_create(int32_t device, b2k_engine** out)
{
  if(!out)
    return -1;
  *out = nullptr;
  int n = 0;
  cudaError_t e = cudaGetDeviceCount(&n);
  if(e != cudaSuccess || n == 0)
  {
    g_err = std::string("no CUDA device: ") + cudaGetErrorString(e) +
            " (this engine has no CPU path; the host keeps its own)";
    return -1;
  }
  if(device < 0 || device >= n)
  {
    g_err = "device index out of range";
    return -1;
  }
  CUDA_TRY(cudaSetDevice(device));
  b2k_engine* eng = new b2k_engine();
  eng->device = device;
  CUDA_TRY(cudaGetDeviceProperties(&eng->prop, device));
  CUDA_TRY(cudaStreamCreateWithFlags(&eng->stream, cudaStreamNonBlocking));
  CUDA_TRY(cudaStreamCreateWithFlags(&eng->copy_stream, cudaStreamNonBlocking));
  CUDA_TRY(cudaStreamCreateWithFlags(&eng->h2d_stream, cudaStreamNonBlocking));
  for(cudaStream_t& a : eng->aux)
    CUDA_TRY(cudaStreamCreateWithFlags(&a, cudaStreamNonBlocking));
  CUDA_TRY(cudaEventCreateWithFlags(&eng->caller_ev, cudaEventDisableTiming));
  *out = eng;
  return 0;
}

extern "C" void b2k_engine_destroy(b2k_engine* e)
{
  if(!e)
    return;
  cudaSetDevice(e->device);
  if(e->cached)
  {
    b2k_job_destroy(e->cached);
    e->cached = nullptr;
  }
  if(e->stream)
    cudaStreamDestroy(e->stream);
  if(e->copy_stream)
    cudaStreamDestroy(e->copy_stream);
  if(e->h2d_stream)
    cudaStreamDestroy(e->h2d_stream);
  for(cudaStream_t a : e->aux)
    if(a)
      cudaStreamDestroy(a);
  if(e->caller_ev)
    cudaEventDestroy(e->caller_ev);
  delete e;
}

extern "C" void* b2k_host_alloc(size_t bytes)
{
  void* p = nullptr;
  if(cudaHostAlloc(&p, bytes, cudaHostAllocDefault) != cudaSuccess)
    return nullptr;
  return p;
}
extern "C" int32_t b2k_set_host_threads(int32_t n)
{
  b2k_host_set_threads(n);
  g_pack_policy.store(n < 0 ? -1 : n == 0 ? 0 : 1);
  return b2k_host_threads();
}

extern "C" int32_t b2k_host_pack_last(int32_t decode) { return g_last_pack[decode ? 1 : 0].load(); }

extern "C" void b2k_host_free(void* p)
{
  if(p)
    cudaFreeHost(p);
}

extern "C" int64_t b2k_enumerate(const b2k_coding* cp, uint32_t tile_mod, uint32_t tile_rem, b2k_block* out, uint64_t cap)
{
  if(!cp || tile_mod == 0)
    return -1;
  if(const char* why = unsupported_reason(*cp))
  {
    g_err = why;
    return -1;
  }
  const TileGrid g = tile_grid(*cp);
  const std::vector<BandQuant> q = band_quant(*cp);
  std::vector<b2k_block> v;
  for(uint32_t t = 0; t < g.nx * g.ny; ++t)
    if(t % tile_mod == tile_rem)
      enumerate_tile_blocks(*cp, t, tile_rect(*cp, g, t), q, v);
  for(uint64_t i = 0; i < v.size() && i < cap; ++i)
    out[i] = v[i];
  return (int64_t)v.size();
}

static void fill_strips(DwtLevelDesc& d, int pairs_per_seg)
{
  const int span = d.u1 - (d.u0 & ~7);
  const int nstrips = std::max(1, (span + 239) / 240);
  int sw = (span + nstrips - 1) / nstrips;
  sw = (sw + 7) & ~7;
  d.nstrips = (uint16_t)nstrips;
  d.strip_w = (uint16_t)sw;
  const int npairs = ((d.v1 - 1) >> 1) - (d.v0 >> 1) + 1;
  d.pairs_per_seg = (uint16_t)pairs_per_seg;
  d.nsegs = (uint16_t)((npairs + pairs_per_seg - 1) / pairs_per_seg);
}

static int upload_descs(LevelLaunch& L)
{
  L.max_jobs = 0;
  for(const DwtLevelDesc& d : L.descs)
    L.max_jobs = std::max(L.max_jobs, (int)d.nstrips * (int)d.nsegs);
  if(L.descs.empty())
    return 0;
  CUDA_TRY(cudaMalloc(&L.d_descs, L.descs.size() * sizeof(DwtLevelDesc)));
  CUDA_TRY(cudaMemcpy(L.d_descs, L.descs.data(), L.descs.size() * sizeof(DwtLevelDesc), cudaMemcpyHostToDevice));
  return 0;
}

static int build_dwt_plan(b2k_device_job* J)
{
  const b2k_coding& cp = J->cp;
  const int L = cp.numres - 1;
  const int ncomp = cp.numcomps;
  const int pairs53 = 32, pairs97 = 32;
  const int P = cp.irreversible ? pairs97 : pairs53;
  const int32_t dc = cp.sgnd ? 0 : -(1 << (cp.prec - 1));
  const int32_t lo = cp.sgnd ? -(1 << (cp.prec - 1)) : 0, hi = cp.sgnd ? (1 << (cp.prec - 1)) - 1 : (1 << cp.prec) - 1;

  if(L == 0)
  {
    for(int dir = 0; dir < 2; ++dir)
    {
      std::vector<LevelLaunch>& out = dir == 0 ? J->fwd : J->inv;
      LevelLaunch mctL, sglL;
      mctL.nc = 3;
      sglL.nc = 1;
      mctL.point = sglL.point = true;
      for(size_t ti = 0; ti < J->tiles.size(); ++ti)
      {
        mctL.tile_first.push_back((uint32_t)mctL.descs.size());
        sglL.tile_first.push_back((uint32_t)sglL.descs.size());
        const Rect tc = J->tile_rects[ti];
        if(tc.empty())
          continue;
        for(int c = 0; c < ncomp;)
        {
          const bool group = cp.mct && c == 0;
          const int nc = group ? 3 : 1;
          LevelLaunch& LL = group ? mctL : sglL;
          DwtLevelDesc d{};
          d.u0 = (int32_t)tc.x0; d.v0 = (int32_t)tc.y0; d.u1 = (int32_t)tc.x1; d.v1 = (int32_t)tc.y1;
          d.first_level = 1;
          d.comp0 = (uint8_t)c;
          for(int k = 0; k < nc; ++k)
          {
            d.in[k] = J->img.at(c + k, tc.x0, tc.y0);
            d.in_pitch = J->img.pitch;
            d.out_c[k] = J->coef.at(c + k, tc.x0, tc.y0);
            d.out_ll[k] = d.out_c[k];
            d.c_pitch = d.ll_pitch = J->coef.pitch;
            d.shift[k] = dc;
            d.lo[k] = lo;
            d.hi[k] = hi;
          }
          LL.descs.push_back(d);
          LL.max_w = std::max(LL.max_w, tc.w());
          LL.max_h = std::max(LL.max_h, tc.h());
          LL.alg_bytes += (uint64_t)tc.w() * tc.h() * nc * 8;
          c += nc;
        }
      }
      mctL.tile_first.push_back((uint32_t)mctL.descs.size());
      sglL.tile_first.push_back((uint32_t)sglL.descs.size());
      if(!mctL.descs.empty()) out.push_back(std::move(mctL));
      if(!sglL.descs.empty()) out.push_back(std::move(sglL));
      for(LevelLaunch& Lh : out)
      {
        Lh.max_jobs = 1;
        if(upload_descs(Lh))
          return -1;
      }
    }
    return 0;
  }
  for(int dir = 0; dir < 2; ++dir)
  {
    std::vector<LevelLaunch>& out = dir == 0 ? J->fwd : J->inv;
    for(int lvl = 1; lvl <= L; ++lvl)
    {
      const int resno = cp.numres - lvl;
      LevelLaunch mctL, sglL;
      mctL.nc = 3;
      sglL.nc = 1;
      for(size_t ti = 0; ti < J->tiles.size(); ++ti)
      {
        mctL.tile_first.push_back((uint32_t)mctL.descs.size());
        sglL.tile_first.push_back((uint32_t)sglL.descs.size());
        const Rect tc = J->tile_rects[ti];
        const Rect r = resolution_rect(tc, cp.numres, resno);
        if(r.empty())
          continue;
        for(int c = 0; c < ncomp;)
        {
          const bool group = (lvl == 1 && cp.mct && c == 0);
          const int nc = group ? 3 : 1;
          DwtLevelDesc d{};
          d.u0 = (int32_t)r.x0; d.v0 = (int32_t)r.y0; d.u1 = (int32_t)r.x1; d.v1 = (int32_t)r.y1;
          d.first_level = lvl == 1;
          d.comp0 = (uint8_t)c;
          const uint32_t llx = (r.x0 + 1) >> 1, lly = (r.y0 + 1) >> 1;
          for(int k = 0; k < nc; ++k)
          {
            const int cc = c + k;
            const Planes& fine = (lvl == 1) ? J->img : J->ll[(lvl - 1) & 1];
            d.in[k] = fine.at(cc, r.x0, r.y0);
            d.in_pitch = fine.pitch;
            d.out_c[k] = J->coef.at(cc, tc.x0, tc.y0);
            d.c_pitch = J->coef.pitch;
            if(lvl == L)
            {
              d.out_ll[k] = d.out_c[k];
              d.ll_pitch = J->coef.pitch;
            }
            else
            {
              const Planes& coarse = J->ll[lvl & 1];
              d.out_ll[k] = coarse.at(cc, llx, lly);
              d.ll_pitch = coarse.pitch;
            }
            d.shift[k] = dc;
            d.lo[k] = lo;
            d.hi[k] = hi;
          }
          fill_strips(d, P);
          (group ? mctL : sglL).descs.push_back(d);
          const uint64_t samples = (uint64_t)r.w() * r.h() * nc;
          (group ? mctL : sglL).alg_bytes += samples * 8;
          c += nc;
        }
      }
      mctL.tile_first.push_back((uint32_t)mctL.descs.size());
      sglL.tile_first.push_back((uint32_t)sglL.descs.size());
      for(LevelLaunch* LL : {&mctL, &sglL})
      {
        int Pl = P;
        auto jobs = [&] {
          uint64_t n = 0;
          for(const DwtLevelDesc& d : LL->descs)
            n += (uint64_t)d.nstrips * d.nsegs;
          return n;
        };
        while(!LL->descs.empty() && Pl > 8 && jobs() < 3552)
        {
          Pl >>= 1;
          for(DwtLevelDesc& d : LL->descs)
            fill_strips(d, Pl);
        }
      }
      if(dir == 0)
      {
        if(!mctL.descs.empty()) out.push_back(std::move(mctL));
        if(!sglL.descs.empty()) out.push_back(std::move(sglL));
      }
      else
      {
        if(!sglL.descs.empty()) out.insert(out.begin(), std::move(sglL));
        if(!mctL.descs.empty()) out.insert(out.begin(), std::move(mctL));
      }
    }
    for(LevelLaunch& Lh : out)
      if(upload_descs(Lh))
        return -1;
  }
  return 0;
}

static uint32_t slot_capacity(uint32_t w, uint32_t h, uint32_t kmax)
{
  const uint64_t samples = (uint64_t)w * h, quads = (uint64_t)((w + 1) / 2) * ((h + 1) / 2);
  const uint64_t ms = (samples * (kmax + 2) + 6) / 7 + 16;
  const uint64_t vlc = (quads * 15 + 6) / 7 + 16;
  return (uint32_t)((ms + vlc + 256 + 15) & ~15ull);
}

static int build_block_plan(b2k_device_job* J)
{
  const b2k_coding& cp = J->cp;
  J->blocks.clear();
  for(size_t ti = 0; ti < J->tiles.size(); ++ti)
    enumerate_tile_blocks(cp, J->tiles[ti], J->tile_rects[ti], J->quant, J->blocks);
  std::vector<Rect> rect_of(J->grid.nx * J->grid.ny);
  for(size_t ti = 0; ti < J->tiles.size(); ++ti)
    rect_of[J->tiles[ti]] = J->tile_rects[ti];
  uint64_t off = 0;
  std::vector<uint32_t> sel_of(J->grid.nx * J->grid.ny, 0);
  for(size_t ti = 0; ti < J->tiles.size(); ++ti)
    sel_of[J->tiles[ti]] = (uint32_t)ti;
  J->coded_first.assign(J->tiles.size() + 1, 0);
  for(uint32_t i = 0; i < J->blocks.size(); ++i)
  {
    const b2k_block& b = J->blocks[i];
    if(b.x1 <= b.x0 || b.y1 <= b.y0)
      continue;
    J->coded_first[sel_of[b.tile] + 1] = (uint32_t)J->h_enc_desc.size() + 1;
    const Rect& tr = rect_of[b.tile];
    const BandQuant& bq = J->quant[band_quant_index(b.resno, b.orient)];
    HtBlockDesc d{};
    d.coef = J->coef.at(b.comp, tr.x0 + b.buf_x, tr.y0 + b.buf_y);
    d.pitch = J->coef.pitch;
    d.w = (uint16_t)(b.x1 - b.x0);
    d.h = (uint16_t)(b.y1 - b.y0);
    d.kmax = bq.kmax;
    d.irreversible = cp.irreversible;
    d.quant = 1.0f / bq.step_enc;
    d.slot_cap = slot_capacity(d.w, d.h, bq.kmax);
    d.slot_off = off;
    off += d.slot_cap;
    {
      const size_t j = J->h_enc_desc.size() & 31u;
      const uint64_t quads = (uint64_t)((d.w + 1) / 2) * ((d.h + 1) / 2);
      if(j == 0)
      {
        J->total_quads += 32 * J->group_quads;
        J->group_quads = 0;
      }
      J->group_quads = std::max(J->group_quads, quads);
      d.rec_off = (uint32_t)(J->total_quads + j);
    }
    J->max_cblk_w = std::max<uint32_t>(J->max_cblk_w, d.w);
    J->enc_limits.stage_words = std::max(J->enc_limits.stage_words, b2k_ht_encode_stage_words(d.w));
    J->enc_limits.max_kmax = std::max<uint32_t>(J->enc_limits.max_kmax, d.kmax);
    J->h_enc_desc.push_back(d);
    J->dec_quant.push_back(bq.step_dec / (float)(1u << (31 - bq.kmax)));
    J->coded_index.push_back(i);
  }
  J->scratch_bytes = off;
  for(size_t ti = 1; ti <= J->tiles.size(); ++ti)
    J->coded_first[ti] = std::max(J->coded_first[ti], J->coded_first[ti - 1]);
  {
    const uint32_t nt = (uint32_t)J->tiles.size();
    uint32_t want = 8;
    if(const char* ev = getenv("B2K_CHUNKS"))
      want = (uint32_t)std::max(1, std::min(B2K_MAX_CHUNKS, atoi(ev)));
    const uint32_t nchunks = std::max(1u, std::min(want, nt));
    J->chunk_tile.clear();
    for(uint32_t k = 0; k <= nchunks; ++k)
      J->chunk_tile.push_back((uint32_t)((uint64_t)k * nt / nchunks));
  }
  const size_t n = J->h_enc_desc.size();
  if(n)
  {
    CUDA_TRY(cudaMalloc(&J->d_enc_desc, n * sizeof(HtBlockDesc)));
    CUDA_TRY(cudaMemcpy(J->d_enc_desc, J->h_enc_desc.data(), n * sizeof(HtBlockDesc), cudaMemcpyHostToDevice));
    CUDA_TRY(cudaMalloc(&J->d_dec_desc, n * sizeof(HtBlockDesc)));
    CUDA_TRY(cudaMalloc(&J->d_out, n * sizeof(HtBlockOut)));
    CUDA_TRY(cudaMalloc(&J->d_offsets, (n + 1) * sizeof(uint64_t)));
    CUDA_TRY(cudaMemset(J->d_offsets, 0, (n + 1) * sizeof(uint64_t)));
    CUDA_TRY(cudaMalloc(&J->d_scratch, J->scratch_bytes + 64));
    CUDA_TRY(cudaMalloc(&J->d_recs, (J->total_quads + 32 * J->group_quads + 64) * sizeof(uint32_t)));
    CUDA_TRY(cudaMalloc(&J->d_dec_status, n * sizeof(HtBlockOut)));
    CUDA_TRY(cudaMalloc(&J->d_dec_quant, n * sizeof(float)));
    CUDA_TRY(cudaMemcpy(J->d_dec_quant, J->dec_quant.data(), n * sizeof(float), cudaMemcpyHostToDevice));
    CUDA_TRY(cudaHostAlloc(&J->h_out, n * sizeof(HtBlockOut), cudaHostAllocDefault));
    CUDA_TRY(cudaHostAlloc(&J->h_dec_desc, n * sizeof(HtBlockDesc), cudaHostAllocDefault));
    CUDA_TRY(cudaHostAlloc(&J->h_offsets, (n + 1) * sizeof(uint64_t), cudaHostAllocDefault));
  }
  CUDA_TRY(cudaMalloc(&J->d_err, sizeof(int)));
  CUDA_TRY(cudaMemset(J->d_err, 0, sizeof(int)));
  return 0;
}

extern "C" int32_t b2k_job_create(b2k_engine* e, const b2k_coding* cp, uint32_t tile_mod, uint32_t tile_rem,
                                  b2k_device_job** out)
{
  if(!e || !cp || !out || tile_mod == 0)
    return -1;
  *out = nullptr;
  if(const char* why = unsupported_reason(*cp))
  {
    g_err = why;
    return 1;
  }
  CUDA_TRY(cudaSetDevice(e->device));
  b2k_device_job* J = new b2k_device_job();
  J->eng = e;
  J->cp = *cp;
  J->tile_mod = tile_mod;
  J->tile_rem = tile_rem;
  J->grid = tile_grid(*cp);
  J->quant = band_quant(*cp);
  for(uint32_t t = 0; t < J->grid.nx * J->grid.ny; ++t)
    if(t % tile_mod == tile_rem)
    {
      const Rect r = tile_rect(*cp, J->grid, t);
      if(r.empty())
        continue;
      J->tiles.push_back(t);
      J->tile_rects.push_back(r);
    }
  const int nc = cp->numcomps;
  if(alloc_planes(J->img, nc, cp->x0, cp->y0, cp->x1, cp->y1) || alloc_planes(J->coef, nc, cp->x0, cp->y0, cp->x1, cp->y1))
  {
    b2k_job_destroy(J);
    return -1;
  }
  if(alloc_planes(J->ll[1], nc, 0, 0, ((cp->x1 + 1) >> 1) + 1, ((cp->y1 + 1) >> 1) + 1) ||
     alloc_planes(J->ll[0], nc, 0, 0, ((cp->x1 + 3) >> 2) + 1, ((cp->y1 + 3) >> 2) + 1))
  {
    b2k_job_destroy(J);
    return -1;
  }
  if(build_dwt_plan(J) || build_block_plan(J))
  {
    b2k_job_destroy(J);
    return -1;
  }
  for(cudaEvent_t& ev : J->ev)
    CUDA_TRY(cudaEventCreate(&ev));
  for(cudaEvent_t& ev : J->chunk_ev)
    CUDA_TRY(cudaEventCreateWithFlags(&ev, cudaEventDisableTiming));
  *out = J;
  return 0;
}

extern "C" void b2k_job_destroy(b2k_device_job* J)
{
  if(!J)
    return;
  cudaSetDevice(J->eng->device);
  cudaStreamSynchronize(J->eng->stream);
  cudaFree(J->img.base);
  cudaFree(J->d_stage);
  cudaFree(J->coef.base);
  cudaFree(J->ll[0].base);
  cudaFree(J->ll[1].base);
  for(LevelLaunch& L : J->fwd) cudaFree(L.d_descs);
  for(LevelLaunch& L : J->inv) cudaFree(L.d_descs);
  cudaFree(J->d_enc_desc);
  cudaFree(J->d_dec_desc);
  cudaFree(J->d_out);
  cudaFree(J->d_offsets);
  cudaFree(J->d_scratch);
  cudaFree(J->d_recs);
  cudaFree(J->d_dec_quant);
  cudaFree(J->d_dec_status);
  cudaFree(J->d_bytes);
  cudaFree(J->d_err);
  cudaFreeHost(J->h_out);
  cudaFreeHost(J->h_dec_desc);
  cudaFreeHost(J->h_offsets);
  cudaFreeHost(J->h_ring);
  for(cudaEvent_t ev : J->q_ev)
    cudaEventDestroy(ev);
  for(cudaEvent_t ev : J->p_ev)
    cudaEventDestroy(ev);
  for(cudaStream_t ps : J->p_streams)
    cudaStreamDestroy(ps);
  for(cudaEvent_t& ev : J->ring_ev)
    if(ev)
      cudaEventDestroy(ev);
  for(cudaEvent_t& ev : J->ev)
    if(ev)
      cudaEventDestroy(ev);
  for(cudaEvent_t& ev : J->chunk_ev)
    if(ev)
      cudaEventDestroy(ev);
  delete J;
}

extern "C" uint64_t b2k_job_num_blocks(const b2k_device_job* J) { return J ? J->blocks.size() : 0; }

struct Container
{
  b2k_device_planes d{};
  uint32_t ox = 0, oy = 0;
  bool device = false;
  bool interleaved = false;
  uint8_t* at(int c, uint32_t x, uint32_t y) const
  {
    return static_cast<uint8_t*>(d.comp[c]) +
           ((size_t)(y - oy) * d.row_pitch[c] + (size_t)(x - ox) * d.col_step[c]) * d.sample_bytes;
  }
};

static Container planar_container(int nc, void* const* comp, const uint32_t* pitch, uint32_t sample_bytes, uint32_t ox, uint32_t oy,
                                  bool device)
{
  Container C;
  for(int c = 0; c < nc && c < 4; ++c)
  {
    C.d.comp[c] = comp[c];
    C.d.row_pitch[c] = pitch[c];
    C.d.col_step[c] = 1;
  }
  C.d.sample_bytes = sample_bytes;
  C.ox = ox;
  C.oy = oy;
  C.device = device;
  return C;
}
static Container interleaved_container(int nc, void* base, uint32_t pitch, uint32_t sample_bytes, uint32_t ox, uint32_t oy, bool device)
{
  Container C;
  for(int c = 0; c < nc && c < 4; ++c)
  {
    C.d.comp[c] = static_cast<uint8_t*>(base) + (size_t)c * sample_bytes;
    C.d.row_pitch[c] = pitch;
    C.d.col_step[c] = (uint32_t)nc;
  }
  C.d.sample_bytes = sample_bytes;
  C.ox = ox;
  C.oy = oy;
  C.device = device;
  C.interleaved = true;
  return C;
}
static Container plane_container(const Planes& P)
{
  void* comp[4];
  uint32_t pitch[4];
  for(int c = 0; c < P.n && c < 4; ++c)
  {
    comp[c] = P.at(c, P.X0, P.Y0);
    pitch[c] = P.pitch;
  }
  return planar_container(P.n, comp, pitch, 4, P.X0, P.Y0, true);
}

static uint32_t stage_pitch(const b2k_coding& cp, bool interleaved)
{
  return interleaved ? ((cp.x1 - cp.x0) * cp.numcomps + 7u) & ~7u : ((cp.x1 - (cp.x0 & ~63u)) + 7u) & ~7u;
}
static size_t stage_plane_elems(const b2k_coding& cp) { return (size_t)stage_pitch(cp, false) * (cp.y1 - cp.y0 + 2); }
static Container stage_container(const b2k_device_job* J, bool interleaved)
{
  const b2k_coding& cp = J->cp;
  const uint32_t pitch = stage_pitch(cp, interleaved);
  if(interleaved)
    return interleaved_container(cp.numcomps, J->d_stage, pitch, 2, cp.x0, cp.y0, true);
  void* comp[4];
  const uint32_t pitches[4] = {pitch, pitch, pitch, pitch};
  for(int c = 0; c < cp.numcomps; ++c)
    comp[c] = J->d_stage + c * stage_plane_elems(cp);
  return planar_container(cp.numcomps, comp, pitches, 2, cp.x0 & ~63u, cp.y0, true);
}
static int ensure_stage(b2k_device_job* J)
{
  if(J->d_stage)
    return 0;
  const b2k_coding& cp = J->cp;
  const size_t bytes = std::max(cp.numcomps * stage_plane_elems(cp), (size_t)stage_pitch(cp, true) * (cp.y1 - cp.y0)) * sizeof(uint16_t);
  CUDA_TRY(cudaMalloc(&J->d_stage, bytes));
  CUDA_TRY(cudaMemset(J->d_stage, 0, bytes));
  CUDA_TRY(cudaStreamSynchronize(0));
  return 0;
}

template <typename F>
static void for_tile_row_runs(const b2k_device_job* J, size_t t0, size_t t1, const Rect* window, F&& fn)
{
  t1 = std::min(t1, J->tiles.size());
  for(size_t ti = t0; ti < t1;)
  {
    Rect r = J->tile_rects[ti];
    size_t tj = ti + 1;
    while(tj < t1 && J->tile_rects[tj].y0 == r.y0 && J->tile_rects[tj].y1 == r.y1 && J->tile_rects[tj].x0 == r.x1)
    {
      r.x1 = J->tile_rects[tj].x1;
      ++tj;
    }
    ti = tj;
    if(window)
    {
      r.x0 = std::max(r.x0, window->x0); r.y0 = std::max(r.y0, window->y0);
      r.x1 = std::min(r.x1, window->x1); r.y1 = std::min(r.y1, window->y1);
      if(r.empty())
        continue;
    }
    fn(r);
  }
}

static cudaError_t copy_rows(void* dst, size_t dpitch, const void* src, size_t spitch, size_t row, uint32_t rows, cudaMemcpyKind kind,
                             cudaStream_t st)
{
  if(dpitch == row && spitch == row)
    return cudaMemcpyAsync(dst, src, row * rows, kind, st);
  return cudaMemcpy2DAsync(dst, dpitch, src, spitch, row, rows, kind, st);
}

static int copy_runs(const b2k_device_job* J, const Container& dst, const Container& src, cudaStream_t st, size_t t0, size_t t1,
                     const Rect* window)
{
  const int nc = J->cp.numcomps, group = src.interleaved ? nc : 1;
  const size_t sb = src.d.sample_bytes;
  const cudaMemcpyKind kind = !src.device ? cudaMemcpyHostToDevice : dst.device ? cudaMemcpyDeviceToDevice : cudaMemcpyDeviceToHost;
  cudaError_t err = cudaSuccess;
  for_tile_row_runs(J, t0, t1, window, [&](const Rect& r) {
    for(int c = 0; c < nc; c += group)
    {
      const cudaError_t e = copy_rows(dst.at(c, r.x0, r.y0), dst.d.row_pitch[c] * sb, src.at(c, r.x0, r.y0), src.d.row_pitch[c] * sb,
                                      (size_t)r.w() * group * sb, r.h(), kind, st);
      if(e != cudaSuccess)
        err = e;
    }
  });
  CUDA_TRY(err);
  return 0;
}

extern "C" int32_t b2k_job_upload(b2k_device_job* J, const int32_t* const* planes, const uint32_t* strides)
{
  if(!J) return -1;
  CUDA_TRY(cudaSetDevice(J->eng->device));
  const Container host = planar_container(J->cp.numcomps, (void* const*)planes, strides, 4, J->cp.x0, J->cp.y0, false);
  if(copy_runs(J, plane_container(J->img), host, J->eng->stream, 0, J->tiles.size(), nullptr)) return -1;
  CUDA_TRY(cudaStreamSynchronize(J->eng->stream));
  return 0;
}
extern "C" int32_t b2k_job_download(b2k_device_job* J, int32_t* const* planes, const uint32_t* strides)
{
  if(!J) return -1;
  CUDA_TRY(cudaSetDevice(J->eng->device));
  const Container host = planar_container(J->cp.numcomps, (void* const*)planes, strides, 4, J->cp.x0, J->cp.y0, false);
  if(copy_runs(J, host, plane_container(J->img), J->eng->stream, 0, J->tiles.size(), nullptr)) return -1;
  CUDA_TRY(cudaStreamSynchronize(J->eng->stream));
  return 0;
}
extern "C" int32_t b2k_job_download_coeffs(b2k_device_job* J, int32_t* const* planes, const uint32_t* strides)
{
  if(!J) return -1;
  CUDA_TRY(cudaSetDevice(J->eng->device));
  const Container host = planar_container(J->cp.numcomps, (void* const*)planes, strides, 4, J->cp.x0, J->cp.y0, false);
  if(copy_runs(J, host, plane_container(J->coef), J->eng->stream, 0, J->tiles.size(), nullptr)) return -1;
  CUDA_TRY(cudaStreamSynchronize(J->eng->stream));
  return 0;
}
extern "C" int32_t b2k_job_upload_coeffs(b2k_device_job* J, const int32_t* const* planes, const uint32_t* strides)
{
  if(!J) return -1;
  CUDA_TRY(cudaSetDevice(J->eng->device));
  const Container host = planar_container(J->cp.numcomps, (void* const*)planes, strides, 4, J->cp.x0, J->cp.y0, false);
  if(copy_runs(J, plane_container(J->coef), host, J->eng->stream, 0, J->tiles.size(), nullptr)) return -1;
  CUDA_TRY(cudaStreamSynchronize(J->eng->stream));
  return 0;
}

static int check_device_planes(const b2k_engine* e, const b2k_coding* cp, const b2k_device_planes* img)
{
  if(!img)
  {
    g_err = "no device image";
    return -1;
  }
  if(img->sample_bytes != 1 && img->sample_bytes != 2 && img->sample_bytes != 4)
  {
    g_err = "sample_bytes must be 1, 2 or 4";
    return -1;
  }
  if(cp->numcomps > 4)
  {
    g_err = "a device image holds at most 4 components";
    return 1;
  }
  if(img->sample_bytes * 8 < cp->prec)
  {
    g_err = std::to_string(img->sample_bytes * 8) + "-bit containers cannot hold " + std::to_string(cp->prec) + "-bit samples";
    return 1;
  }
  for(int c = 0; c < cp->numcomps; ++c)
  {
    const std::string comp = "device image component " + std::to_string(c) + ": ";
    cudaPointerAttributes a{};
    const cudaError_t err = img->comp[c] ? cudaPointerGetAttributes(&a, img->comp[c]) : cudaErrorInvalidValue;
    if(err != cudaSuccess)
      (void)cudaGetLastError();
    if(err != cudaSuccess || (a.type != cudaMemoryTypeDevice && a.type != cudaMemoryTypeManaged) || a.device != e->device)
    {
      g_err = comp + "not device or managed memory of the engine's device (" + std::to_string(e->device) + ")";
      return -1;
    }
    if(reinterpret_cast<uintptr_t>(img->comp[c]) % img->sample_bytes)
    {
      g_err = comp + "address not a multiple of sample_bytes";
      return -1;
    }
    if(!img->col_step[c])
    {
      g_err = comp + "col_step is 0";
      return -1;
    }
  }
  return 0;
}

static int device_group(const b2k_device_planes& img, int nc)
{
  const uint8_t* base = static_cast<const uint8_t*>(img.comp[0]);
  for(int c = 1; c < nc; ++c)
    if(static_cast<const uint8_t*>(img.comp[c]) != base + (size_t)c * img.sample_bytes || img.row_pitch[c] != img.row_pitch[0] ||
       img.col_step[c] != img.col_step[0])
      return 1;
  return nc;
}

static int device_convert(b2k_device_job* J, const Container& img, bool to_planes, cudaStream_t st, size_t t0, size_t t1,
                          const Rect* window)
{
  const b2k_coding& cp = J->cp;
  const int nc = cp.numcomps;
  bool planar32 = img.d.sample_bytes == 4;
  for(int c = 0; c < nc; ++c)
    planar32 = planar32 && img.d.col_step[c] == 1;
  if(planar32)
  {
    const Container planes = plane_container(J->img);
    return to_planes ? copy_runs(J, planes, img, st, t0, t1, window) : copy_runs(J, img, planes, st, t0, t1, window);
  }
  const int group = device_group(img.d, nc);
  for_tile_row_runs(J, t0, t1, window, [&](const Rect& r) {
    for(int c = 0; c < nc; c += group)
    {
      int32_t* planes[4];
      for(int k = 0; k < group; ++k)
        planes[k] = J->img.at(c + k, r.x0, r.y0);
      if(to_planes)
        b2k_launch_container_to_planes(img.at(c, r.x0, r.y0), img.d.row_pitch[c], img.d.col_step[c], img.d.sample_bytes, planes, group,
                                       J->img.pitch, r.w(), r.h(), cp.sgnd, st);
      else
        b2k_launch_planes_to_container(planes, group, J->img.pitch, img.at(c, r.x0, r.y0), img.d.row_pitch[c], img.d.col_step[c],
                                       img.d.sample_bytes, r.w(), r.h(), st);
    }
  });
  CUDA_TRY(cudaGetLastError());
  return 0;
}

static bool host_pack_eligible(const b2k_device_job* J)
{
  const b2k_coding& cp = J->cp;
  const uint64_t samples = (uint64_t)(cp.x1 - cp.x0) * (cp.y1 - cp.y0) * cp.numcomps;
  return cp.prec <= 16 && samples >= (1u << 22) && J->chunk_tile.size() > 2 && b2k_host_threads() > 0;
}

struct StagePiece
{
  uint32_t chunk, comp, x0, y0, w, rows;
};
struct RingGeom
{
  uint32_t slot_mb, slots;
};
static RingGeom ring_geom(bool decode)
{
  auto parse = [](const char* name, RingGeom r) {
    if(const char* e = getenv(name))
    {
      r.slot_mb = (uint32_t)std::max(1, atoi(e));
      if(const char* c = strchr(e, ','))
        r.slots = (uint32_t)std::max(2, std::min(16, atoi(c + 1)));
    }
    return r;
  };
  static const RingGeom g[2] = {parse("B2K_RING_ENC", {8, 4}), parse("B2K_RING_DEC", {16, 4})};
  return g[decode ? 1 : 0];
}
static int ensure_ring(b2k_device_job* J, bool decode)
{
  const RingGeom g = ring_geom(decode);
  const uint64_t min_elems = (uint64_t)(J->cp.x1 - J->cp.x0) * 4;
  const uint64_t slot_elems = std::max<uint64_t>((uint64_t)g.slot_mb * (1u << 20) / sizeof(uint16_t), min_elems);
  const uint64_t need = slot_elems * g.slots;
  if(need > J->ring_elems)
  {
    if(J->h_ring)
      cudaFreeHost(J->h_ring);
    J->h_ring = nullptr;
    CUDA_TRY(cudaHostAlloc(&J->h_ring, need * sizeof(uint16_t), cudaHostAllocDefault));
    J->ring_elems = need;
  }
  for(uint32_t i = 0; i < g.slots; ++i)
    if(!J->ring_ev[i])
      CUDA_TRY(cudaEventCreateWithFlags(&J->ring_ev[i], cudaEventDisableTiming));
  J->ring_slots = g.slots;
  J->ring_slot_elems = slot_elems;
  return 0;
}
static void chunk_pieces(const b2k_device_job* J, uint32_t chunk, std::vector<StagePiece>& out)
{
  for_tile_row_runs(J, J->chunk_tile[chunk], J->chunk_tile[chunk + 1], nullptr, [&](const Rect& r) {
    const uint32_t rows_per = (uint32_t)std::max<uint64_t>(1, J->ring_slot_elems / r.w());
    for(uint32_t y = r.y0; y < r.y1; y += rows_per)
      for(uint32_t c = 0; c < J->cp.numcomps; ++c)
        out.push_back({chunk, c, r.x0, y, r.w(), std::min(rows_per, r.y1 - y)});
  });
}
static int ring_upload_chunk(b2k_device_job* J, const Container& user, const Container& stage, uint32_t chunk, cudaStream_t cs,
                             uint64_t& counter, const std::function<int()>& between_pieces)
{
  std::vector<StagePiece> pcs;
  chunk_pieces(J, chunk, pcs);
  for(const StagePiece& pc : pcs)
  {
    const uint32_t slot = (uint32_t)(counter % J->ring_slots);
    if(counter >= J->ring_slots)
      CUDA_TRY(cudaEventSynchronize(J->ring_ev[slot]));
    uint16_t* sp = J->h_ring + (uint64_t)slot * J->ring_slot_elems;
    const b2k_host_rect hr{user.at(pc.comp, pc.x0, pc.y0), sp, user.d.row_pitch[pc.comp], pc.w, pc.w, pc.rows};
    b2k_host_convert(&hr, 1, false, J->cp.sgnd != 0, true);
    CUDA_TRY(copy_rows(stage.at(pc.comp, pc.x0, pc.y0), (size_t)stage.d.row_pitch[pc.comp] * 2, sp, (size_t)pc.w * 2,
                       (size_t)pc.w * 2, pc.rows, cudaMemcpyHostToDevice, cs));
    CUDA_TRY(cudaEventRecord(J->ring_ev[slot], cs));
    ++counter;
    if(between_pieces())
      return -1;
  }
  return 0;
}
static int ring_download_all(b2k_device_job* J, const Container& user, const Container& stage, cudaStream_t cs)
{
  std::vector<StagePiece> pcs;
  for(uint32_t k = 0; k + 1 < J->chunk_tile.size(); ++k)
    chunk_pieces(J, k, pcs);
  const size_t N = pcs.size(), S = J->ring_slots;
  auto issue = [&](size_t p) -> int {
    const StagePiece& pc = pcs[p];
    const uint32_t slot = (uint32_t)(p % S);
    uint16_t* sp = J->h_ring + (uint64_t)slot * J->ring_slot_elems;
    if(p == 0 || pcs[p - 1].chunk != pc.chunk)
      CUDA_TRY(cudaStreamWaitEvent(cs, J->chunk_ev[CEV(0, pc.chunk)], 0));
    CUDA_TRY(copy_rows(sp, (size_t)pc.w * 2, stage.at(pc.comp, pc.x0, pc.y0), (size_t)stage.d.row_pitch[pc.comp] * 2,
                       (size_t)pc.w * 2, pc.rows, cudaMemcpyDeviceToHost, cs));
    CUDA_TRY(cudaEventRecord(J->ring_ev[slot], cs));
    return 0;
  };
  for(size_t p = 0; p < std::min(S, N); ++p)
    if(issue(p)) return -1;
  for(size_t p = 0; p < N; ++p)
  {
    const StagePiece& pc = pcs[p];
    const uint32_t slot = (uint32_t)(p % S);
    CUDA_TRY(cudaEventSynchronize(J->ring_ev[slot]));
    const uint16_t* sp = J->h_ring + (uint64_t)slot * J->ring_slot_elems;
    const b2k_host_rect hr{sp, user.at(pc.comp, pc.x0, pc.y0), pc.w, user.d.row_pitch[pc.comp], pc.w, pc.rows};
    b2k_host_convert(&hr, 1, true, J->cp.sgnd != 0);
    if(p + S < N)
      if(issue(p + S)) return -1;
  }
  return 0;
}

struct Transport
{
  Container user;
  const Rect* window = nullptr;
  Container stage;
  bool staged = false;
  bool ring = false;
  uint64_t ring_pieces = 0;
  PackTuner* tuner = nullptr;
  Transport() = default;
  Transport(const Transport&) = delete;
  ~Transport()
  {
    if(ring)
      b2k_host_session(false);
  }
};

static int resolve_transport(b2k_device_job* J, Transport& T, bool decode)
{
  if(T.user.device)
    return 0;
  if(T.user.d.sample_bytes == 4)
  {
    const bool eligible = !T.window && host_pack_eligible(J);
    const bool tuned = eligible && g_pack_policy.load() < 0 && b2k_host_local_peers() == 1;
    PackTuner& tuner = decode ? J->tune_dec : J->tune_enc;
    const bool pack = eligible && (tuned ? tuner.next_mode() : g_pack_policy.load() > 0);
    g_last_pack[decode ? 1 : 0].store(pack ? 1 : 0);
    T.tuner = tuned ? &tuner : nullptr;
    if(!pack)
      return 0;
    if(ensure_ring(J, decode))
      return -1;
    T.ring = true;
    b2k_host_session(true);
  }
  if(ensure_stage(J))
    return -1;
  T.stage = stage_container(J, T.user.interleaved);
  T.staged = true;
  return 0;
}

static int upload_chunk(b2k_device_job* J, Transport& T, size_t k, cudaStream_t st, cudaStream_t cs,
                        const std::function<int()>& between_pieces)
{
  if(T.ring ? ring_upload_chunk(J, T.user, T.stage, (uint32_t)k, cs, T.ring_pieces, between_pieces)
            : copy_runs(J, T.staged ? T.stage : plane_container(J->img), T.user, cs, J->chunk_tile[k], J->chunk_tile[k + 1], nullptr))
    return -1;
  CUDA_TRY(cudaEventRecord(J->chunk_ev[CEV(0, k)], cs));
  CUDA_TRY(cudaStreamWaitEvent(st, J->chunk_ev[CEV(0, k)], 0));
  return 0;
}

static int download_chunk(b2k_device_job* J, const Transport& T, size_t k, cudaStream_t st, cudaStream_t cs)
{
  const size_t t0 = J->chunk_tile[k], t1 = J->chunk_tile[k + 1];
  if(T.user.device)
    return device_convert(J, T.user, false, st, t0, t1, T.window);
  if(T.staged && device_convert(J, T.stage, false, st, t0, t1, T.window))
    return -1;
  CUDA_TRY(cudaEventRecord(J->chunk_ev[CEV(0, k)], st));
  if(T.ring)
    return 0;
  CUDA_TRY(cudaStreamWaitEvent(cs, J->chunk_ev[CEV(0, k)], 0));
  return copy_runs(J, T.user, T.staged ? T.stage : plane_container(J->img), cs, t0, t1, T.window);
}

static int enqueue_forward(b2k_device_job* J, cudaStream_t st, bool time_level1, size_t t0 = 0, size_t t1 = (size_t)-1,
                           cudaEvent_t l1_begin = nullptr, cudaEvent_t l1_end = nullptr)
{
  if(!l1_begin) l1_begin = J->ev[4];
  if(!l1_end) l1_end = J->ev[5];
  t1 = std::min(t1, J->tiles.size());
  bool first = true;
  for(size_t li = 0; li < J->fwd.size(); ++li)
  {
    LevelLaunch& L = J->fwd[li];
    const uint32_t d0 = L.tile_first[t0], d1 = L.tile_first[t1];
    if(first && time_level1)
      CUDA_TRY(cudaEventRecord(l1_begin, st));
    if(d1 > d0 && L.point)
      b2k_launch_point_transform(L.d_descs + d0, (int)(d1 - d0), L.max_w, L.max_h, L.nc, J->cp.irreversible, true, st);
    else if(d1 > d0)
      b2k_launch_dwt_fwd(L.d_descs + d0, (int)(d1 - d0), L.max_jobs, L.nc, J->cp.irreversible, st);
    if(first && time_level1)
    {
      CUDA_TRY(cudaEventRecord(l1_end, st));
      J->level1_alg_bytes = L.alg_bytes;
    }
    first = false;
  }
  CUDA_TRY(cudaGetLastError());
  return 0;
}

static int enqueue_inverse(b2k_device_job* J, cudaStream_t st, size_t t0 = 0, size_t t1 = (size_t)-1)
{
  t1 = std::min(t1, J->tiles.size());
  for(size_t li = 0; li < J->inv.size(); ++li)
  {
    LevelLaunch& L = J->inv[li];
    const uint32_t d0 = L.tile_first[t0], d1 = L.tile_first[t1];
    if(d1 > d0 && L.point)
      b2k_launch_point_transform(L.d_descs + d0, (int)(d1 - d0), L.max_w, L.max_h, L.nc, J->cp.irreversible, false, st);
    else if(d1 > d0)
      b2k_launch_dwt_inv(L.d_descs + d0, (int)(d1 - d0), L.max_jobs, L.nc, J->cp.irreversible, st);
  }
  CUDA_TRY(cudaGetLastError());
  return 0;
}

static int enqueue_t1_blocks(b2k_device_job* J, cudaStream_t st, size_t t0, size_t t1)
{
  t1 = std::min(t1, J->tiles.size());
  const uint32_t b0 = J->coded_first[t0], b1 = J->coded_first[t1];
  if(b1 > b0)
    b2k_launch_ht_encode(J->d_enc_desc + b0, J->d_out + b0, J->d_scratch, b1 - b0, J->enc_limits, J->cp.irreversible, st);
  CUDA_TRY(cudaGetLastError());
  return 0;
}

static int enqueue_t1_encode(b2k_device_job* J, cudaStream_t st)
{
  const uint32_t n = (uint32_t)J->h_enc_desc.size();
  b2k_launch_ht_encode(J->d_enc_desc, J->d_out, J->d_scratch, n, J->enc_limits, J->cp.irreversible, st);
  b2k_launch_scan_lengths(J->d_out, J->d_offsets, n, st);
  CUDA_TRY(cudaGetLastError());
  return 0;
}

static int finish_t1_encode(b2k_device_job* J, cudaStream_t st)
{
  const uint32_t n = (uint32_t)J->h_enc_desc.size();
  uint64_t total = 0;
  CUDA_TRY(cudaMemcpyAsync(&J->h_offsets[n], J->d_offsets + n, sizeof(uint64_t), cudaMemcpyDeviceToHost, st));
  CUDA_TRY(cudaStreamSynchronize(st));
  total = J->h_offsets[n];
  if(total + 64 > J->bytes_cap)
  {
    cudaFree(J->d_bytes);
    J->bytes_cap = total + total / 8 + 4096;
    CUDA_TRY(cudaMalloc(&J->d_bytes, J->bytes_cap));
  }
  J->bytes_used = total;
  b2k_launch_ht_gather(J->d_enc_desc, J->d_out, J->d_offsets, J->d_scratch, J->d_bytes, n, J->bytes_cap, st);
  CUDA_TRY(cudaGetLastError());
  return 0;
}

extern "C" int32_t b2k_job_forward(b2k_device_job* J, float* ms)
{
  if(!J) return -1;
  CUDA_TRY(cudaSetDevice(J->eng->device));
  cudaStream_t st = J->eng->stream;
  CUDA_TRY(cudaEventRecord(J->ev[0], st));
  if(enqueue_forward(J, st, true)) return -1;
  CUDA_TRY(cudaEventRecord(J->ev[1], st));
  CUDA_TRY(cudaEventSynchronize(J->ev[1]));
  float t = 0;
  CUDA_TRY(cudaEventElapsedTime(&t, J->ev[0], J->ev[1]));
  if(ms) *ms = t;
  CUDA_TRY(cudaEventElapsedTime(&J->last_level1_ms, J->ev[4], J->ev[5]));
  return 0;
}

extern "C" int32_t b2k_job_inverse(b2k_device_job* J, float* ms)
{
  if(!J) return -1;
  CUDA_TRY(cudaSetDevice(J->eng->device));
  cudaStream_t st = J->eng->stream;
  CUDA_TRY(cudaEventRecord(J->ev[0], st));
  if(enqueue_inverse(J, st)) return -1;
  CUDA_TRY(cudaEventRecord(J->ev[1], st));
  CUDA_TRY(cudaEventSynchronize(J->ev[1]));
  float t = 0;
  CUDA_TRY(cudaEventElapsedTime(&t, J->ev[0], J->ev[1]));
  if(ms) *ms = t;
  return 0;
}

extern "C" int32_t b2k_job_t1_encode(b2k_device_job* J, float* ms, uint64_t* total_bytes)
{
  if(!J) return -1;
  CUDA_TRY(cudaSetDevice(J->eng->device));
  cudaStream_t st = J->eng->stream;
  CUDA_TRY(cudaEventRecord(J->ev[0], st));
  if(enqueue_t1_encode(J, st)) return -1;
  if(finish_t1_encode(J, st)) return -1;
  CUDA_TRY(cudaEventRecord(J->ev[1], st));
  CUDA_TRY(cudaEventSynchronize(J->ev[1]));
  float t = 0;
  CUDA_TRY(cudaEventElapsedTime(&t, J->ev[0], J->ev[1]));
  if(ms) *ms = t;
  if(total_bytes) *total_bytes = J->bytes_used;
  return 0;
}

static int prepare_decode(b2k_device_job* J, const b2k_block* blocks, uint64_t num_blocks, cudaStream_t st, size_t k0 = 0,
                          size_t k1 = (size_t)-1)
{
  const size_t n = J->h_enc_desc.size();
  k1 = std::min(k1, n);
  if(num_blocks != J->blocks.size())
  {
    g_err = "block count does not match this coding's enumeration";
    return -1;
  }
  for(size_t k = k0; k < k1; ++k)
  {
    const b2k_block& b = blocks[J->coded_index[k]];
    HtBlockDesc d = J->h_enc_desc[k];
    d.length = b.length;
    d.slot_off = b.offset;
    if(b.numpasses > 3)
    {
      g_err = "an HT code block with more than 3 coding passes";
      return 1;
    }
    const int nb = b.length ? b.numbps : 0;
    d.mmsbs = (uint8_t)std::max(0, (int)d.kmax - nb);
    d.passes = (b.length && b.numpasses > 1 && b.length2 > 0 && d.mmsbs < 29) ? b.numpasses : 1;
    d.length2 = d.passes > 1 ? b.length2 : 0;
    if(d.passes > 1)
      J->dec_has_refinement = true;
    d.quant = J->dec_quant[k];
    J->h_dec_desc[k] = d;
  }
  if(k1 > k0)
    CUDA_TRY(cudaMemcpyAsync(J->d_dec_desc + k0, J->h_dec_desc + k0, (k1 - k0) * sizeof(HtBlockDesc), cudaMemcpyHostToDevice, st));
  return 0;
}

static int enqueue_t1_decode_own(b2k_device_job* J, cudaStream_t st)
{
  const uint32_t n = (uint32_t)J->h_enc_desc.size();
  b2k_launch_build_dec_desc(J->d_enc_desc, J->d_out, J->d_offsets, J->d_dec_quant, J->d_dec_desc, n, st);
  b2k_launch_ht_decode(J->d_dec_desc, J->d_bytes, J->d_recs, J->d_dec_status, n, J->max_cblk_w, J->d_err, J->cp.irreversible, 0, st);
  CUDA_TRY(cudaGetLastError());
  return 0;
}

extern "C" int32_t b2k_job_t1_decode(b2k_device_job* J, float* ms)
{
  if(!J) return -1;
  CUDA_TRY(cudaSetDevice(J->eng->device));
  cudaStream_t st = J->eng->stream;
  CUDA_TRY(cudaMemsetAsync(J->d_err, 0, sizeof(int), st));
  CUDA_TRY(cudaEventRecord(J->ev[0], st));
  if(enqueue_t1_decode_own(J, st)) return -1;
  CUDA_TRY(cudaEventRecord(J->ev[1], st));
  CUDA_TRY(cudaEventSynchronize(J->ev[1]));
  float t = 0;
  CUDA_TRY(cudaEventElapsedTime(&t, J->ev[0], J->ev[1]));
  if(ms) *ms = t;
  int herr = 0;
  CUDA_TRY(cudaMemcpy(&herr, J->d_err, sizeof(int), cudaMemcpyDeviceToHost));
  if(herr)
  {
    g_err = "HT decoder rejected " + std::to_string(herr) + " block(s)";
    return -2;
  }
  return 0;
}

extern "C" int32_t b2k_job_t1_decode_blocks(b2k_device_job* J, const b2k_block* blocks, uint64_t num_blocks,
                                            const uint8_t* bytes, uint64_t num_bytes, float* ms)
{
  if(!J || !blocks || (!bytes && num_bytes)) return -1;
  CUDA_TRY(cudaSetDevice(J->eng->device));
  cudaStream_t st = J->eng->stream;
  if(num_bytes + 64 > J->bytes_cap)
  {
    CUDA_TRY(cudaStreamSynchronize(st));
    cudaFree(J->d_bytes);
    J->bytes_cap = num_bytes + 4096;
    CUDA_TRY(cudaMalloc(&J->d_bytes, J->bytes_cap));
  }
  J->dec_has_refinement = false;
  if(int prc = prepare_decode(J, blocks, num_blocks, st)) return prc;
  const uint32_t n = (uint32_t)J->h_enc_desc.size();
  for(uint32_t k = 0; k < n; ++k)
    if((uint64_t)J->h_dec_desc[k].slot_off + J->h_dec_desc[k].length + J->h_dec_desc[k].length2 > num_bytes)
    {
      g_err = "block offsets exceed the byte arena";
      return -1;
    }
  CUDA_TRY(cudaMemsetAsync(J->d_err, 0, sizeof(int), st));
  if(num_bytes)
    CUDA_TRY(cudaMemcpyAsync(J->d_bytes, bytes, num_bytes, cudaMemcpyHostToDevice, st));
  CUDA_TRY(cudaEventRecord(J->ev[0], st));
  b2k_launch_ht_decode(J->d_dec_desc, J->d_bytes, J->d_recs, J->d_dec_status, n, J->max_cblk_w, J->d_err, J->cp.irreversible,
                       J->dec_has_refinement, st);
  if(J->dec_has_refinement)
    b2k_launch_ht_decode_refine(J->d_dec_desc, J->d_bytes, J->d_dec_status, n, (J->cp.cblk_sty & 0x08) != 0, st);
  CUDA_TRY(cudaEventRecord(J->ev[1], st));
  CUDA_TRY(cudaEventSynchronize(J->ev[1]));
  CUDA_TRY(cudaGetLastError());
  float t = 0;
  CUDA_TRY(cudaEventElapsedTime(&t, J->ev[0], J->ev[1]));
  if(ms) *ms = t;
  int herr = 0;
  CUDA_TRY(cudaMemcpy(&herr, J->d_err, sizeof(int), cudaMemcpyDeviceToHost));
  if(herr)
  {
    g_err = "HT decoder rejected " + std::to_string(herr) + " block(s)";
    return -2;
  }
  return 0;
}

extern "C" int32_t b2k_job_roundtrip(b2k_device_job* J, float* ms_total, float* stage_ms, uint64_t* total_bytes)
{
  if(!J) return -1;
  CUDA_TRY(cudaSetDevice(J->eng->device));
  cudaStream_t st = J->eng->stream;
  const uint32_t n = (uint32_t)J->h_enc_desc.size();
  if(J->bytes_cap == 0)
  {
    float t;
    uint64_t b;
    if(int rc = b2k_job_forward(J, &t)) return rc;
    if(int rc = b2k_job_t1_encode(J, &t, &b)) return rc;
  }
  CUDA_TRY(cudaMemsetAsync(J->d_err, 0, sizeof(int), st));
  CUDA_TRY(cudaEventRecord(J->ev[0], st));
  if(enqueue_forward(J, st, true)) return -1;
  CUDA_TRY(cudaEventRecord(J->ev[1], st));
  if(enqueue_t1_encode(J, st)) return -1;
  b2k_launch_ht_gather(J->d_enc_desc, J->d_out, J->d_offsets, J->d_scratch, J->d_bytes, n, J->bytes_cap, st);
  CUDA_TRY(cudaMemcpyAsync(&J->h_offsets[n], J->d_offsets + n, sizeof(uint64_t), cudaMemcpyDeviceToHost, st));
  CUDA_TRY(cudaEventRecord(J->ev[2], st));
  if(enqueue_t1_decode_own(J, st)) return -1;
  CUDA_TRY(cudaEventRecord(J->ev[3], st));
  if(enqueue_inverse(J, st)) return -1;
  CUDA_TRY(cudaEventRecord(J->ev[6], st));
  CUDA_TRY(cudaEventSynchronize(J->ev[6]));
  CUDA_TRY(cudaGetLastError());
  if(J->h_offsets[n] > J->bytes_cap)
  {
    cudaFree(J->d_bytes);
    J->bytes_cap = J->h_offsets[n] + J->h_offsets[n] / 8 + 4096;
    CUDA_TRY(cudaMalloc(&J->d_bytes, J->bytes_cap));
    g_err = "coded size grew past the arena: arena resized, call again";
    return 2;
  }
  J->bytes_used = J->h_offsets[n];
  float t[5] = {0, 0, 0, 0, 0};
  cudaEventElapsedTime(&t[0], J->ev[0], J->ev[1]);
  cudaEventElapsedTime(&t[1], J->ev[1], J->ev[2]);
  cudaEventElapsedTime(&t[2], J->ev[2], J->ev[3]);
  cudaEventElapsedTime(&t[3], J->ev[3], J->ev[6]);
  cudaEventElapsedTime(&t[4], J->ev[0], J->ev[6]);
  cudaEventElapsedTime(&J->last_level1_ms, J->ev[4], J->ev[5]);
  if(ms_total) *ms_total = t[4];
  if(stage_ms)
    for(int i = 0; i < 4; ++i)
      stage_ms[i] = t[i];
  if(total_bytes) *total_bytes = J->bytes_used;
  int herr = 0;
  CUDA_TRY(cudaMemcpy(&herr, J->d_err, sizeof(int), cudaMemcpyDeviceToHost));
  if(herr)
  {
    g_err = "HT decoder rejected " + std::to_string(herr) + " block(s)";
    return -2;
  }
  return 0;
}

extern "C" int32_t b2k_job_roundtrip_n(b2k_device_job* J, uint32_t steps, float* ms_total, float* stage_ms, float* level1_ms,
                                       uint64_t* total_bytes)
{
  if(!J || !steps) return -1;
  CUDA_TRY(cudaSetDevice(J->eng->device));
  cudaStream_t st = J->eng->stream;
  const uint32_t n = (uint32_t)J->h_enc_desc.size();
  if(J->bytes_cap == 0)
  {
    float t;
    uint64_t b;
    if(int rc = b2k_job_forward(J, &t)) return rc;
    if(int rc = b2k_job_t1_encode(J, &t, &b)) return rc;
  }
  const size_t per = 7;
  while(J->q_ev.size() < per * steps)
  {
    cudaEvent_t ev;
    CUDA_TRY(cudaEventCreate(&ev));
    J->q_ev.push_back(ev);
  }
  CUDA_TRY(cudaMemsetAsync(J->d_err, 0, sizeof(int), st));
  for(uint32_t s = 0; s < steps; ++s)
  {
    cudaEvent_t* e = J->q_ev.data() + per * s;
    CUDA_TRY(cudaEventRecord(e[0], st));
    if(enqueue_forward(J, st, true, 0, (size_t)-1, e[1], e[2])) return -1;
    CUDA_TRY(cudaEventRecord(e[3], st));
    if(enqueue_t1_encode(J, st)) return -1;
    b2k_launch_ht_gather(J->d_enc_desc, J->d_out, J->d_offsets, J->d_scratch, J->d_bytes, n, J->bytes_cap, st);
    if(s + 1 == steps)
      CUDA_TRY(cudaMemcpyAsync(&J->h_offsets[n], J->d_offsets + n, sizeof(uint64_t), cudaMemcpyDeviceToHost, st));
    CUDA_TRY(cudaEventRecord(e[4], st));
    if(enqueue_t1_decode_own(J, st)) return -1;
    CUDA_TRY(cudaEventRecord(e[5], st));
    if(enqueue_inverse(J, st)) return -1;
    CUDA_TRY(cudaEventRecord(e[6], st));
  }
  CUDA_TRY(cudaEventSynchronize(J->q_ev[per * (steps - 1) + 6]));
  CUDA_TRY(cudaGetLastError());
  if(J->h_offsets[n] > J->bytes_cap)
  {
    cudaFree(J->d_bytes);
    J->bytes_cap = J->h_offsets[n] + J->h_offsets[n] / 8 + 4096;
    CUDA_TRY(cudaMalloc(&J->d_bytes, J->bytes_cap));
    g_err = "coded size grew past the arena: arena resized, call again";
    return 2;
  }
  J->bytes_used = J->h_offsets[n];
  float sums[4] = {0, 0, 0, 0}, l1 = 0, tot = 0;
  for(uint32_t s = 0; s < steps; ++s)
  {
    cudaEvent_t* e = J->q_ev.data() + per * s;
    float t = 0;
    cudaEventElapsedTime(&t, e[0], e[3]); sums[0] += t;
    cudaEventElapsedTime(&t, e[3], e[4]); sums[1] += t;
    cudaEventElapsedTime(&t, e[4], e[5]); sums[2] += t;
    cudaEventElapsedTime(&t, e[5], e[6]); sums[3] += t;
    cudaEventElapsedTime(&t, e[1], e[2]); l1 += t;
  }
  cudaEventElapsedTime(&tot, J->q_ev[0], J->q_ev[per * (steps - 1) + 6]);
  J->last_level1_ms = l1 / steps;
  if(ms_total) *ms_total = tot;
  if(stage_ms)
    for(int i = 0; i < 4; ++i)
      stage_ms[i] = sums[i];
  if(level1_ms) *level1_ms = l1;
  if(total_bytes) *total_bytes = J->bytes_used;
  int herr = 0;
  CUDA_TRY(cudaMemcpy(&herr, J->d_err, sizeof(int), cudaMemcpyDeviceToHost));
  if(herr)
  {
    g_err = "HT decoder rejected " + std::to_string(herr) + " block(s)";
    return -2;
  }
  return 0;
}

extern "C" int32_t b2k_job_roundtrip_pipelined_n(b2k_device_job* J, uint32_t steps, uint32_t chunks, uint32_t streams, float* ms_total,
                                                 float* stage_ms, float* level1_ms, uint64_t* total_bytes)
{
  if(!J || !steps) return -1;
  CUDA_TRY(cudaSetDevice(J->eng->device));
  cudaStream_t st = J->eng->stream;
  const uint32_t n = (uint32_t)J->h_enc_desc.size();
  if(J->bytes_cap == 0)
  {
    float t;
    uint64_t b;
    if(int rc = b2k_job_forward(J, &t)) return rc;
    if(int rc = b2k_job_t1_encode(J, &t, &b)) return rc;
  }
  chunks = std::max(1u, std::min(chunks ? chunks : 2u, 64u));
  streams = std::max(1u, std::min(streams ? streams : 2u, 8u));
  const uint32_t per_chunk = std::max(128u, (((n + chunks - 1) / chunks) + 127u) & ~127u);
  const uint32_t nch = n ? (n + per_chunk - 1) / per_chunk : 0;
  while(J->p_streams.size() < streams)
  {
    cudaStream_t ps;
    CUDA_TRY(cudaStreamCreateWithFlags(&ps, cudaStreamNonBlocking));
    J->p_streams.push_back(ps);
  }
  while(J->p_ev.size() < 2 * (size_t)nch)
  {
    cudaEvent_t ev;
    CUDA_TRY(cudaEventCreateWithFlags(&ev, cudaEventDisableTiming));
    J->p_ev.push_back(ev);
  }
  const size_t per = 5;
  while(J->q_ev.size() < per * steps + 1)
  {
    cudaEvent_t ev;
    CUDA_TRY(cudaEventCreate(&ev));
    J->q_ev.push_back(ev);
  }
  CUDA_TRY(cudaMemsetAsync(J->d_err, 0, sizeof(int), st));
  for(uint32_t s = 0; s < steps; ++s)
  {
    cudaEvent_t* e = J->q_ev.data() + per * s;
    CUDA_TRY(cudaEventRecord(e[0], st));
    if(enqueue_forward(J, st, true, 0, (size_t)-1, e[1], e[2])) return -1;
    CUDA_TRY(cudaEventRecord(e[3], st));
    for(uint32_t k = 0; k < streams && k < nch; ++k)
      CUDA_TRY(cudaStreamWaitEvent(J->p_streams[k], e[3], 0));
    for(uint32_t c = 0; c < nch; ++c)
    {
      cudaStream_t ps = J->p_streams[c % streams];
      const uint32_t b0 = c * per_chunk, b1 = std::min(n, b0 + per_chunk), nb = b1 - b0;
      b2k_launch_ht_encode(J->d_enc_desc + b0, J->d_out + b0, J->d_scratch, nb, J->enc_limits, J->cp.irreversible, ps);
      if(c > 0)
        CUDA_TRY(cudaStreamWaitEvent(ps, J->p_ev[2 * (c - 1)], 0));
      b2k_launch_scan_lengths(J->d_out + b0, J->d_offsets + b0, nb, ps);
      CUDA_TRY(cudaEventRecord(J->p_ev[2 * c], ps));
      b2k_launch_ht_gather(J->d_enc_desc + b0, J->d_out + b0, J->d_offsets + b0, J->d_scratch, J->d_bytes, nb, J->bytes_cap, ps);
      b2k_launch_build_dec_desc(J->d_enc_desc + b0, J->d_out + b0, J->d_offsets + b0, J->d_dec_quant + b0, J->d_dec_desc + b0, nb, ps);
      b2k_launch_ht_decode(J->d_dec_desc + b0, J->d_bytes, J->d_recs, J->d_dec_status + b0, nb, J->max_cblk_w, J->d_err,
                           J->cp.irreversible, 0, ps);
      CUDA_TRY(cudaEventRecord(J->p_ev[2 * c + 1], ps));
    }
    for(uint32_t c = 0; c < nch; ++c)
      CUDA_TRY(cudaStreamWaitEvent(st, J->p_ev[2 * c + 1], 0));
    if(s + 1 == steps)
      CUDA_TRY(cudaMemcpyAsync(&J->h_offsets[n], J->d_offsets + n, sizeof(uint64_t), cudaMemcpyDeviceToHost, st));
    CUDA_TRY(cudaEventRecord(e[4], st));
    if(enqueue_inverse(J, st)) return -1;
  }
  cudaEvent_t last = J->q_ev[per * steps];
  CUDA_TRY(cudaEventRecord(last, st));
  CUDA_TRY(cudaEventSynchronize(last));
  CUDA_TRY(cudaGetLastError());
  if(J->h_offsets[n] > J->bytes_cap)
  {
    cudaFree(J->d_bytes);
    J->bytes_cap = J->h_offsets[n] + J->h_offsets[n] / 8 + 4096;
    CUDA_TRY(cudaMalloc(&J->d_bytes, J->bytes_cap));
    g_err = "coded size grew past the arena: arena resized, call again";
    return 2;
  }
  J->bytes_used = J->h_offsets[n];
  float sums[3] = {0, 0, 0}, l1 = 0, tot = 0;
  for(uint32_t s = 0; s < steps; ++s)
  {
    cudaEvent_t* e = J->q_ev.data() + per * s;
    float t = 0;
    cudaEventElapsedTime(&t, e[0], e[3]); sums[0] += t;
    cudaEventElapsedTime(&t, e[3], e[4]); sums[1] += t;
    cudaEventElapsedTime(&t, e[4], e[per]); sums[2] += t;
    cudaEventElapsedTime(&t, e[1], e[2]); l1 += t;
  }
  cudaEventElapsedTime(&tot, J->q_ev[0], last);
  J->last_level1_ms = l1 / steps;
  if(ms_total) *ms_total = tot;
  if(stage_ms)
    for(int i = 0; i < 3; ++i)
      stage_ms[i] = sums[i];
  if(level1_ms) *level1_ms = l1;
  if(total_bytes) *total_bytes = J->bytes_used;
  int herr = 0;
  CUDA_TRY(cudaMemcpy(&herr, J->d_err, sizeof(int), cudaMemcpyDeviceToHost));
  if(herr)
  {
    g_err = "HT decoder rejected " + std::to_string(herr) + " block(s)";
    return -2;
  }
  return 0;
}

extern "C" int32_t b2k_job_last_kernel_stats(const b2k_device_job* J, int which, float* ms, uint64_t* alg_bytes)
{
  if(!J) return -1;
  if(which == 0)
  {
    if(ms) *ms = J->last_level1_ms;
    if(alg_bytes) *alg_bytes = J->level1_alg_bytes;
    return 0;
  }
  return 1;
}

struct PinnedPool
{
  std::mutex mu;
  std::vector<std::pair<uint8_t*, uint64_t>> free_list;
  std::vector<std::pair<uint8_t*, uint64_t>> live;
  std::vector<uint8_t*> heap;
};
static PinnedPool g_pool;
static uint8_t* pool_get(uint64_t bytes)
{
  std::lock_guard<std::mutex> lock(g_pool.mu);
  for(size_t i = 0; i < g_pool.free_list.size(); ++i)
    if(g_pool.free_list[i].second >= bytes)
    {
      auto e = g_pool.free_list[i];
      g_pool.free_list.erase(g_pool.free_list.begin() + i);
      g_pool.live.push_back(e);
      return e.first;
    }
  uint8_t* p = nullptr;
  const uint64_t cap = bytes + bytes / 4 + 4096;
  if(cudaHostAlloc(&p, cap, cudaHostAllocDefault) != cudaSuccess)
    return nullptr;
  g_pool.live.push_back({p, cap});
  return p;
}
static void pool_put(uint8_t* p)
{
  std::lock_guard<std::mutex> lock(g_pool.mu);
  for(size_t i = 0; i < g_pool.heap.size(); ++i)
    if(g_pool.heap[i] == p)
    {
      g_pool.heap.erase(g_pool.heap.begin() + i);
      free(p);
      return;
    }
  for(size_t i = 0; i < g_pool.live.size(); ++i)
    if(g_pool.live[i].first == p)
    {
      g_pool.free_list.push_back(g_pool.live[i]);
      g_pool.live.erase(g_pool.live.begin() + i);
      while(g_pool.free_list.size() > 16)
      {
        cudaFreeHost(g_pool.free_list.front().first);
        g_pool.free_list.erase(g_pool.free_list.begin());
      }
      return;
    }
  cudaFreeHost(p);
}

static b2k_result* result_shell(b2k_device_job* J)
{
  b2k_result* R = new b2k_result();
  memset(R, 0, sizeof(*R));
  R->num_blocks = J->blocks.size();
  R->blocks = (b2k_block*)malloc(sizeof(b2k_block) * std::max<size_t>(1, J->blocks.size()));
  memcpy(R->blocks, J->blocks.data(), sizeof(b2k_block) * J->blocks.size());
  R->num_tiles = (uint32_t)J->tiles.size();
  return R;
}

static int fetch_result(b2k_device_job* J, cudaStream_t st, b2k_result** out, uint8_t* host_bytes = nullptr,
                        b2k_result* shell = nullptr, bool meta_on_host = false)
{
  const uint32_t n = (uint32_t)J->h_enc_desc.size();
  b2k_result* R = shell ? shell : result_shell(J);
  R->num_bytes = J->bytes_used;
  R->bytes = host_bytes ? host_bytes : pool_get(std::max<uint64_t>(64, J->bytes_used));
  if(!R->bytes)
  {
    g_err = "cudaHostAlloc(result bytes) failed";
    free(R->blocks);
    delete R;
    return -1;
  }
  struct ResultGuard
  {
    b2k_result* r;
    ~ResultGuard() { if(r) b2k_result_free(r); }
  } guard{R};
  if(!host_bytes)
    CUDA_TRY(cudaMemcpyAsync(R->bytes, J->d_bytes, J->bytes_used, cudaMemcpyDeviceToHost, st));
  if(!meta_on_host)
  {
    CUDA_TRY(cudaMemcpyAsync(J->h_out, J->d_out, n * sizeof(HtBlockOut), cudaMemcpyDeviceToHost, st));
    CUDA_TRY(cudaMemcpyAsync(J->h_offsets, J->d_offsets, (n + 1) * sizeof(uint64_t), cudaMemcpyDeviceToHost, st));
  }
  CUDA_TRY(cudaStreamSynchronize(st));
  int bad = 0;
  for(uint32_t k = 0; k < n; ++k)
  {
    b2k_block& b = R->blocks[J->coded_index[k]];
    if(J->h_out[k].total == 0xFFFFFFFFu)
    {
      bad++;
      continue;
    }
    b.length = J->h_out[k].total;
    b.offset = J->h_offsets[k];
    b.numbps = 1;
    b.numpasses = 1;
  }
  if(bad)
  {
    g_err = std::to_string(bad) + " code block(s) overflowed the coder's buffers";
    return -2;
  }
  guard.r = nullptr;
  *out = R;
  return 0;
}

extern "C" int32_t b2k_job_fetch_result(b2k_device_job* J, b2k_result** out)
{
  if(!J || !out) return -1;
  CUDA_TRY(cudaSetDevice(J->eng->device));
  return fetch_result(J, J->eng->stream, out);
}

extern "C" void b2k_result_free(b2k_result* r)
{
  if(!r) return;
  free(r->blocks);
  if(r->bytes) pool_put(r->bytes);
  delete r;
}

extern "C" int32_t b2k_result_merge(const b2k_coding* cp, const b2k_result* const* shards, uint32_t nshards, b2k_result** out)
{
  if(!cp || !shards || !nshards || !out)
    return -1;
  if(const char* why = unsupported_reason(*cp))
  {
    g_err = why;
    return -1;
  }
  const TileGrid g = tile_grid(*cp);
  const uint32_t ntiles = g.nx * g.ny;
  const std::vector<BandQuant> q = band_quant(*cp);
  std::vector<b2k_block> all;
  for(uint32_t t = 0; t < ntiles; ++t)
    enumerate_tile_blocks(*cp, t, tile_rect(*cp, g, t), q, all);
  uint64_t total_bytes = 0;
  std::vector<uint64_t> base(nshards, 0);
  for(uint32_t s = 0; s < nshards; ++s)
  {
    if(!shards[s])
    {
      g_err = "missing shard";
      return -1;
    }
    base[s] = total_bytes;
    total_bytes += shards[s]->num_bytes;
  }
  b2k_result* R = new b2k_result();
  memset(R, 0, sizeof(*R));
  R->num_blocks = all.size();
  R->num_tiles = ntiles;
  R->num_bytes = total_bytes;
  R->blocks = (b2k_block*)malloc(sizeof(b2k_block) * std::max<size_t>(1, all.size()));
  uint8_t* arena = pool_get(std::max<uint64_t>(64, total_bytes));
  if(!arena)
  {
    (void)cudaGetLastError();
    arena = (uint8_t*)malloc(std::max<uint64_t>(64, total_bytes));
    std::lock_guard<std::mutex> lock(g_pool.mu);
    g_pool.heap.push_back(arena);
  }
  R->bytes = arena;
  if(!R->blocks || !arena)
  {
    b2k_result_free(R);
    g_err = "out of memory";
    return -1;
  }
  std::vector<uint64_t> next(nshards, 0);
  for(size_t i = 0; i < all.size(); ++i)
  {
    const uint32_t s = all[i].tile % nshards;
    const b2k_result* S = shards[s];
    if(next[s] >= S->num_blocks)
    {
      b2k_result_free(R);
      g_err = "a shard holds fewer blocks than its tiles have";
      return -1;
    }
    const b2k_block& b = S->blocks[next[s]++];
    if(b.tile != all[i].tile || b.comp != all[i].comp || b.resno != all[i].resno || b.band_index != all[i].band_index ||
       b.precno != all[i].precno || b.cblkno != all[i].cblkno)
    {
      b2k_result_free(R);
      g_err = "a shard's block table is not the enumeration of the tiles t % nshards == shard";
      return -1;
    }
    R->blocks[i] = b;
    R->blocks[i].offset = b.offset + base[s];
  }
  for(uint32_t s = 0; s < nshards; ++s)
  {
    if(next[s] != shards[s]->num_blocks)
    {
      b2k_result_free(R);
      g_err = "a shard holds more blocks than its tiles have";
      return -1;
    }
  }
  {
    struct Piece { uint8_t* dst; const uint8_t* src; size_t n; };
    std::vector<Piece> pieces;
    const size_t step = (size_t)8 << 20;
    for(uint32_t s = 0; s < nshards; ++s)
      for(size_t o = 0; o < shards[s]->num_bytes; o += step)
        pieces.push_back({arena + base[s] + o, shards[s]->bytes + o, std::min<size_t>(step, shards[s]->num_bytes - o)});
    b2k_host_parallel(pieces.size(), [&](size_t i) { memcpy(pieces[i].dst, pieces[i].src, pieces[i].n); });
  }
  *out = R;
  return 0;
}

static bool dbg_timing()
{
  static const bool v = getenv("B2K_DEBUG_TIMING") != nullptr;
  return v;
}
#define DBG_T(label)                                                                                              \
  do                                                                                                              \
  {                                                                                                               \
    if(dbg_timing())                                                                                              \
      fprintf(stderr, "[b2k] %-28s %8.3f ms\n", label,                                                            \
              std::chrono::duration<double, std::milli>(std::chrono::steady_clock::now() - wall0).count());       \
  } while(0)

static b2k_device_job* cached_job(b2k_engine* e, const b2k_coding* cp, uint32_t mod, uint32_t rem, int* rc)
{
  b2k_device_job*& J = e->cached;
  cudaSetDevice(e->device);
  if(J && (memcmp(&J->cp, cp, sizeof(b2k_coding)) != 0 || J->tile_mod != mod || J->tile_rem != rem))
  {
    b2k_job_destroy(J);
    J = nullptr;
  }
  if(!J)
    *rc = b2k_job_create(e, cp, mod, rem, &J);
  else
    *rc = 0;
  return J;
}

static int32_t encode_common(b2k_engine* e, const b2k_coding* cp, uint32_t mod, uint32_t rem, b2k_result** out, Transport& T,
                             cudaStream_t caller = nullptr)
{
  if(!e || !cp || !out)
    return -1;
  std::lock_guard<std::mutex> lock(e->mu);
  int rc = 0;
  b2k_device_job* J = cached_job(e, cp, mod, rem, &rc);
  if(rc)
    return rc;
  CUDA_TRY(cudaSetDevice(e->device));
  const auto wall0 = std::chrono::steady_clock::now();
  if(resolve_transport(J, T, false))
    return -1;
  const bool dev = T.user.device;
  cudaStream_t st = e->stream;
  cudaStream_t cs = e->copy_stream;
  if(dev)
  {
    CUDA_TRY(cudaEventRecord(e->caller_ev, caller));
    CUDA_TRY(cudaStreamWaitEvent(st, e->caller_ev, 0));
  }
  CUDA_TRY(cudaEventRecord(J->ev[0], st));
  CUDA_TRY(cudaStreamWaitEvent(cs, J->ev[0], 0));
  const size_t nchunks = J->chunk_tile.size() - 1;
  const bool streamed = J->bytes_cap > 0 && nchunks > 1;
  uint8_t* hb = nullptr;
  struct ArenaGuard
  {
    uint8_t*& p;
    ~ArenaGuard() { if(p) pool_put(p); }
  } arena_guard{hb};
  if(streamed)
  {
    hb = pool_get(J->bytes_cap);
    if(!hb)
    {
      g_err = "cudaHostAlloc(result bytes) failed";
      return -1;
    }
  }
  cudaStream_t ds = e->h2d_stream;
  size_t next_out = 0, enqueued = 0;
  uint64_t total = 0;
  bool overflow = false;
  auto return_chunks = [&](bool block) -> int {
    while(next_out < enqueued)
    {
      const size_t k = next_out;
      if(block)
        CUDA_TRY(cudaEventSynchronize(J->chunk_ev[CEV(2, k)]));
      else if(cudaEventQuery(J->chunk_ev[CEV(2, k)]) != cudaSuccess)
        break;
      const uint32_t b0 = J->coded_first[J->chunk_tile[k]], b1 = J->coded_first[J->chunk_tile[k + 1]];
      const uint64_t lo = k == 0 ? 0 : J->h_offsets[b0], hi = J->h_offsets[b1];
      total = hi;
      if(hi > J->bytes_cap)
        overflow = true;
      else if(hi > lo)
      {
        CUDA_TRY(cudaStreamWaitEvent(ds, J->chunk_ev[CEV(2, k)], 0));
        CUDA_TRY(cudaMemcpyAsync(hb + lo, J->d_bytes + lo, hi - lo, cudaMemcpyDeviceToHost, ds));
      }
      if(b1 > b0)
      {
        CUDA_TRY(cudaStreamWaitEvent(ds, J->chunk_ev[CEV(2, k)], 0));
        CUDA_TRY(cudaMemcpyAsync(J->h_out + b0, J->d_out + b0, (size_t)(b1 - b0) * sizeof(HtBlockOut), cudaMemcpyDeviceToHost, ds));
        CUDA_TRY(cudaMemcpyAsync(J->h_offsets + b0, J->d_offsets + b0, (size_t)(b1 - b0) * sizeof(uint64_t),
                                 cudaMemcpyDeviceToHost, ds));
      }
      ++next_out;
    }
    (void)cudaGetLastError();
    return 0;
  };
  for(size_t k = 0; k < nchunks; ++k)
  {
    const size_t t0 = J->chunk_tile[k], t1 = J->chunk_tile[k + 1];
    if(dev ? device_convert(J, T.user, true, st, t0, t1, nullptr) : upload_chunk(J, T, k, st, cs, [&] { return return_chunks(false); }))
      return -1;
    if(k == nchunks - 1)
      CUDA_TRY(cudaEventRecord(J->ev[1], st));
    if(T.staged && device_convert(J, T.stage, true, st, t0, t1, nullptr)) return -1;
    if(enqueue_forward(J, st, k == 0, t0, t1)) return -1;
    if(enqueue_t1_blocks(J, st, t0, t1)) return -1;
    if(streamed)
    {
      const uint32_t b0 = J->coded_first[t0], b1 = J->coded_first[t1];
      if(b1 > b0)
      {
        b2k_launch_scan_lengths(J->d_out + b0, J->d_offsets + b0, b1 - b0, st);
        b2k_launch_ht_gather(J->d_enc_desc + b0, J->d_out + b0, J->d_offsets + b0, J->d_scratch, J->d_bytes, b1 - b0,
                             J->bytes_cap, st);
      }
      CUDA_TRY(cudaMemcpyAsync(&J->h_offsets[b1], J->d_offsets + b1, sizeof(uint64_t), cudaMemcpyDeviceToHost, st));
      CUDA_TRY(cudaEventRecord(J->chunk_ev[CEV(2, k)], st));
      enqueued = k + 1;
      if(return_chunks(false)) return -1;
    }
  }
  CUDA_TRY(cudaEventRecord(J->ev[2], st));
  if(dev)
  {
    CUDA_TRY(cudaEventRecord(e->caller_ev, st));
    CUDA_TRY(cudaStreamWaitEvent(caller, e->caller_ev, 0));
  }
  DBG_T("encode: chunks enqueued");
  b2k_result* R = nullptr;
  const uint32_t nb_all = (uint32_t)J->h_enc_desc.size();
  b2k_result* shell = result_shell(J);
  if(streamed)
  {
    if(return_chunks(true)) return -1;
    CUDA_TRY(cudaEventRecord(J->chunk_ev[CEV(3, 0)], ds));
    CUDA_TRY(cudaStreamWaitEvent(st, J->chunk_ev[CEV(3, 0)], 0));
    DBG_T("encode: last chunk coded");
    J->bytes_used = total;
    if(overflow)
    {
      pool_put(hb);
      hb = nullptr;
      CUDA_TRY(cudaStreamSynchronize(st));
      cudaFree(J->d_bytes);
      J->bytes_cap = total + total / 8 + 4096;
      CUDA_TRY(cudaMalloc(&J->d_bytes, J->bytes_cap));
      b2k_launch_ht_gather(J->d_enc_desc, J->d_out, J->d_offsets, J->d_scratch, J->d_bytes, nb_all, J->bytes_cap, st);
      CUDA_TRY(cudaEventRecord(J->ev[3], st));
      if(int frc = fetch_result(J, st, &R, nullptr, shell)) return frc;
    }
    else
    {
      CUDA_TRY(cudaEventRecord(J->ev[3], st));
      uint8_t* owned = hb;
      hb = nullptr;
      if(int frc = fetch_result(J, st, &R, owned, shell, true)) return frc;
    }
  }
  if(!streamed)
  {
    b2k_launch_scan_lengths(J->d_out, J->d_offsets, nb_all, st);
    if(finish_t1_encode(J, st)) return -1;
    CUDA_TRY(cudaEventRecord(J->ev[3], st));
    if(int frc = fetch_result(J, st, &R, nullptr, shell)) return frc;
  }
  DBG_T("encode: result fetched");
  CUDA_TRY(cudaEventRecord(J->ev[6], st));
  CUDA_TRY(cudaEventSynchronize(J->ev[6]));
  DBG_T("encode: done");
  float a = 0, b = 0, c = 0, d = 0;
  cudaEventElapsedTime(&a, J->ev[0], J->ev[1]);
  cudaEventElapsedTime(&b, J->ev[1], J->ev[2]);
  cudaEventElapsedTime(&c, J->ev[2], J->ev[3]);
  cudaEventElapsedTime(&d, J->ev[3], J->ev[6]);
  cudaEventElapsedTime(&J->last_level1_ms, J->ev[4], J->ev[5]);
  R->ms_h2d = a; R->ms_dwt = b; R->ms_t1 = c; R->ms_d2h = d; R->ms_total = a + b + c + d;
  if(T.tuner)
    T.tuner->record(T.ring, std::chrono::duration<double, std::milli>(std::chrono::steady_clock::now() - wall0).count());
  *out = R;
  return 0;
}

static int32_t host_samples(Transport& T, const b2k_coding* cp, const void* const* planes, const uint32_t* strides, uint32_t sample_bytes,
                            uint32_t x0, uint32_t y0)
{
  if(!planes || !strides)
    return -1;
  T.user = planar_container(cp->numcomps, const_cast<void* const*>(planes), strides, sample_bytes, x0, y0, false);
  return 0;
}
static void device_samples(Transport& T, const b2k_device_planes& img, uint32_t x0, uint32_t y0)
{
  T.user.d = img;
  T.user.ox = x0;
  T.user.oy = y0;
  T.user.device = true;
}

extern "C" int32_t b2k_encode(b2k_engine* e, const b2k_coding* cp, const int32_t* const* planes, const uint32_t* strides,
                              uint32_t tile_mod, uint32_t tile_rem, b2k_result** out)
{
  Transport T;
  if(!cp || host_samples(T, cp, (const void* const*)planes, strides, 4, cp->x0, cp->y0))
    return -1;
  return encode_common(e, cp, tile_mod, tile_rem, out, T);
}

extern "C" int32_t b2k_encode16(b2k_engine* e, const b2k_coding* cp, const uint16_t* const* planes, const uint32_t* strides,
                                uint32_t tile_mod, uint32_t tile_rem, b2k_result** out)
{
  Transport T;
  if(!cp || host_samples(T, cp, (const void* const*)planes, strides, 2, cp->x0, cp->y0))
    return -1;
  return encode_common(e, cp, tile_mod, tile_rem, out, T);
}

extern "C" int32_t b2k_encode16_interleaved(b2k_engine* e, const b2k_coding* cp, const uint16_t* pixels, uint32_t stride,
                                            uint32_t tile_mod, uint32_t tile_rem, b2k_result** out)
{
  if(!cp || !pixels || stride < (uint32_t)(cp->x1 - cp->x0) * cp->numcomps)
    return -1;
  Transport T;
  T.user = interleaved_container(cp->numcomps, const_cast<uint16_t*>(pixels), stride, 2, cp->x0, cp->y0, false);
  return encode_common(e, cp, tile_mod, tile_rem, out, T);
}

static int32_t decode_common(b2k_engine* e, const b2k_coding* cp, const b2k_block* blocks, uint64_t num_blocks,
                             const uint8_t* bytes, uint64_t num_bytes, uint32_t tile_mod, uint32_t tile_rem, double* ms_total,
                             Transport& T, const uint32_t* window = nullptr, cudaStream_t caller = nullptr);

extern "C" int32_t b2k_decode(b2k_engine* e, const b2k_coding* cp, const b2k_block* blocks, uint64_t num_blocks,
                              const uint8_t* bytes, uint64_t num_bytes, int32_t* const* planes, const uint32_t* strides,
                              uint32_t tile_mod, uint32_t tile_rem, double* ms_total)
{
  Transport T;
  if(!cp || host_samples(T, cp, (const void* const*)planes, strides, 4, cp->x0, cp->y0))
    return -1;
  return decode_common(e, cp, blocks, num_blocks, bytes, num_bytes, tile_mod, tile_rem, ms_total, T);
}
extern "C" int32_t b2k_decode16(b2k_engine* e, const b2k_coding* cp, const b2k_block* blocks, uint64_t num_blocks,
                                const uint8_t* bytes, uint64_t num_bytes, uint16_t* const* planes, const uint32_t* strides,
                                uint32_t tile_mod, uint32_t tile_rem, double* ms_total)
{
  Transport T;
  if(!cp || host_samples(T, cp, (const void* const*)planes, strides, 2, cp->x0, cp->y0))
    return -1;
  return decode_common(e, cp, blocks, num_blocks, bytes, num_bytes, tile_mod, tile_rem, ms_total, T);
}

extern "C" int32_t b2k_decode_window(b2k_engine* e, const b2k_coding* cp, const b2k_block* blocks, uint64_t num_blocks,
                                     const uint8_t* bytes, uint64_t num_bytes, void* const* planes, const uint32_t* strides,
                                     const uint32_t* window, uint32_t sample_bytes, double* ms_total)
{
  Transport T;
  if(!cp || !window || (sample_bytes != 2 && sample_bytes != 4) ||
     host_samples(T, cp, (const void* const*)planes, strides, sample_bytes, window[0], window[1]))
    return -1;
  return decode_common(e, cp, blocks, num_blocks, bytes, num_bytes, 1, 0, ms_total, T, window);
}

static cudaStream_t caller_stream(void* s) { return s ? static_cast<cudaStream_t>(s) : cudaStreamLegacy; }

extern "C" int32_t b2k_encode_device(b2k_engine* e, const b2k_coding* cp, const b2k_device_planes* img, uint32_t tile_mod,
                                     uint32_t tile_rem, void* cuda_stream, b2k_result** out)
{
  if(!e || !cp || !out)
    return -1;
  if(int rc = check_device_planes(e, cp, img))
    return rc;
  Transport T;
  device_samples(T, *img, cp->x0, cp->y0);
  return encode_common(e, cp, tile_mod, tile_rem, out, T, caller_stream(cuda_stream));
}

extern "C" int32_t b2k_decode_device(b2k_engine* e, const b2k_coding* cp, const b2k_block* blocks, uint64_t num_blocks,
                                     const uint8_t* bytes, uint64_t num_bytes, const b2k_device_planes* img, const uint32_t* window,
                                     uint32_t tile_mod, uint32_t tile_rem, void* cuda_stream, double* ms_total)
{
  if(!e || !cp)
    return -1;
  if(window && tile_mod != 1)
  {
    g_err = "a windowed decode takes every tile: tile_mod must be 1";
    return -1;
  }
  if(int rc = check_device_planes(e, cp, img))
    return rc;
  Transport T;
  device_samples(T, *img, window ? window[0] : cp->x0, window ? window[1] : cp->y0);
  return decode_common(e, cp, blocks, num_blocks, bytes, num_bytes, tile_mod, tile_rem, ms_total, T, window, caller_stream(cuda_stream));
}

static int32_t decode_common(b2k_engine* e, const b2k_coding* cp, const b2k_block* blocks, uint64_t num_blocks,
                             const uint8_t* bytes, uint64_t num_bytes, uint32_t tile_mod, uint32_t tile_rem, double* ms_total,
                             Transport& T, const uint32_t* window, cudaStream_t caller)
{
  if(!e || !cp || !blocks)
    return -1;
  if(window &&
     (window[0] >= window[2] || window[1] >= window[3] || window[0] < cp->x0 || window[1] < cp->y0 || window[2] > cp->x1 || window[3] > cp->y1))
  {
    g_err = "window outside the image";
    return -1;
  }
  std::lock_guard<std::mutex> lock(e->mu);
  int rc = 0;
  b2k_device_job* J = cached_job(e, cp, tile_mod, tile_rem, &rc);
  if(rc)
    return rc;
  CUDA_TRY(cudaSetDevice(e->device));
  const Rect win = window ? Rect{window[0], window[1], window[2], window[3]} : Rect{};
  T.window = window ? &win : nullptr;
  const auto wall0 = std::chrono::steady_clock::now();
  if(resolve_transport(J, T, true))
    return -1;
  const bool dev = T.user.device;
  cudaStream_t st = e->stream;
  if(num_bytes + 64 > J->bytes_cap)
  {
    cudaFree(J->d_bytes);
    J->bytes_cap = num_bytes + 4096;
    CUDA_TRY(cudaMalloc(&J->d_bytes, J->bytes_cap));
  }
  if(dev)
  {
    CUDA_TRY(cudaEventRecord(e->caller_ev, caller));
    CUDA_TRY(cudaStreamWaitEvent(st, e->caller_ev, 0));
  }
  CUDA_TRY(cudaEventRecord(J->ev[0], st));
  CUDA_TRY(cudaMemsetAsync(J->d_err, 0, sizeof(int), st));
  J->dec_has_refinement = false;
  cudaStream_t cs = e->copy_stream;
  const size_t nchunks = J->chunk_tile.size() - 1;
  CUDA_TRY(cudaStreamWaitEvent(cs, J->ev[0], 0));
  CUDA_TRY(cudaStreamWaitEvent(e->h2d_stream, J->ev[0], 0));
  bool all_uploaded = false;
  uint64_t prev_end = 0;
  for(size_t k = 0; k < nchunks; ++k)
  {
    const size_t t0 = J->chunk_tile[k], t1 = J->chunk_tile[k + 1];
    const uint32_t b0 = J->coded_first[t0], b1 = J->coded_first[t1];
    if(int prc = prepare_decode(J, blocks, num_blocks, e->h2d_stream, b0, b1)) return prc;
    uint64_t lo = UINT64_MAX, hi = 0;
    for(uint32_t b = b0; b < b1; ++b)
    {
      const HtBlockDesc& d = J->h_dec_desc[b];
      if(!d.length)
        continue;
      lo = std::min<uint64_t>(lo, d.slot_off);
      hi = std::max<uint64_t>(hi, d.slot_off + d.length + d.length2);
    }
    if(hi > num_bytes)
    {
      g_err = "block offsets exceed the byte arena";
      return -1;
    }
    if(!all_uploaded && lo != UINT64_MAX)
    {
      if(lo < prev_end)
      {
        CUDA_TRY(cudaMemcpyAsync(J->d_bytes, bytes, num_bytes, cudaMemcpyHostToDevice, e->h2d_stream));
        all_uploaded = true;
      }
      else
      {
        CUDA_TRY(cudaMemcpyAsync(J->d_bytes + lo, bytes + lo, hi - lo, cudaMemcpyHostToDevice, e->h2d_stream));
        prev_end = hi;
      }
    }
    CUDA_TRY(cudaEventRecord(J->chunk_ev[CEV(1, k)], e->h2d_stream));
    CUDA_TRY(cudaStreamWaitEvent(st, J->chunk_ev[CEV(1, k)], 0));
    if(b1 > b0)
    {
      cudaStream_t ax = e->aux[k & 3];
      CUDA_TRY(cudaStreamWaitEvent(ax, J->chunk_ev[CEV(1, k)], 0));
      b2k_launch_ht_decode_vlc(J->d_dec_desc + b0, J->d_bytes, J->d_recs, J->d_dec_status + b0, b1 - b0, J->max_cblk_w, ax);
      CUDA_TRY(cudaEventRecord(J->chunk_ev[CEV(2, k)], ax));
      CUDA_TRY(cudaStreamWaitEvent(st, J->chunk_ev[CEV(2, k)], 0));
      b2k_launch_ht_decode_magsgn(J->d_dec_desc + b0, J->d_bytes, J->d_recs, J->d_dec_status + b0, b1 - b0, J->max_cblk_w,
                                  J->d_err, J->cp.irreversible, J->dec_has_refinement, st);
      if(J->dec_has_refinement)
        b2k_launch_ht_decode_refine(J->d_dec_desc + b0, J->d_bytes, J->d_dec_status + b0, b1 - b0,
                                    (J->cp.cblk_sty & 0x08) != 0, st);
    }
    if(enqueue_inverse(J, st, t0, t1)) return -1;
    if(download_chunk(J, T, k, st, cs)) return -1;
  }
  DBG_T("decode: chunks enqueued");
  if(T.ring && ring_download_all(J, T.user, T.stage, cs)) return -1;
  CUDA_TRY(cudaEventRecord(J->chunk_ev[CEV(0, nchunks)], cs));
  CUDA_TRY(cudaStreamWaitEvent(st, J->chunk_ev[CEV(0, nchunks)], 0));
  CUDA_TRY(cudaEventRecord(J->ev[1], st));
  if(dev)
  {
    CUDA_TRY(cudaEventRecord(e->caller_ev, st));
    CUDA_TRY(cudaStreamWaitEvent(caller, e->caller_ev, 0));
  }
  CUDA_TRY(cudaEventSynchronize(J->ev[1]));
  CUDA_TRY(cudaGetLastError());
  DBG_T("decode: done");
  float t = 0;
  cudaEventElapsedTime(&t, J->ev[0], J->ev[1]);
  if(ms_total) *ms_total = t;
  if(T.tuner)
    T.tuner->record(T.ring, std::chrono::duration<double, std::milli>(std::chrono::steady_clock::now() - wall0).count());
  int herr = 0;
  CUDA_TRY(cudaMemcpy(&herr, J->d_err, sizeof(int), cudaMemcpyDeviceToHost));
  if(herr)
  {
    g_err = "HT decoder rejected " + std::to_string(herr) + " block(s)";
    return -2;
  }
  return 0;
}
```

Before: 13750.

## Use whole-warp 256-column strips with ghost columns for reversible 5/3 DWT

For the reversible 5/3 forward and inverse DWT, each warp now owns all 32 lanes of output (256 columns) instead of reserving two halo lanes. The few boundary samples needed at strip edges are fetched separately as ghost columns and staged in a small extra shared-memory region alongside the bulk row data. Lanes 0 and 31 use these ghosts in the horizontal lifting. This removes the wasted halo lanes and the overlapping loads between neighbouring strips, at the cost of extra per-lane branching, additional cp.async traffic and an added wait for ghost data even on the bulk (TMA) path. Launch bounds also now request 3 CTAs per SM.

```diff
diff --git a/grok_b200/csrc/dwt.cu b/grok_b200/csrc/dwt.cu
--- a/grok_b200/csrc/dwt.cu
+++ b/grok_b200/csrc/dwt.cu
@@ -67,6 +67,7 @@
   int lane, ulane, jbeg, jend, wn, hn, nvalid;
   bool owner, need;
 };
+template <bool WHOLE>
 __device__ __forceinline__ bool decode_job(const DwtLevelDesc& D, Job& J)
 {
   J.lane = threadIdx.x & 31;
@@ -74,12 +75,13 @@
   if(job >= (int)D.nstrips * (int)D.nsegs)
     return false;
   const int strip = job % D.nstrips, seg = job / D.nstrips;
+  constexpr int halo = WHOLE ? 0 : 1;
   J.wn = D.u1 - D.u0;
   J.hn = D.v1 - D.v0;
   J.nvalid = D.strip_w >> 3;
-  J.ulane = (D.u0 & ~7) + strip * (int)D.strip_w + (J.lane - 1) * 8;
-  J.owner = J.lane >= 1 && J.lane <= J.nvalid && J.ulane < D.u1;
-  J.need = J.lane <= J.nvalid + 1 && J.ulane < D.u1 + 8;
+  J.ulane = (D.u0 & ~7) + strip * (int)D.strip_w + (J.lane - halo) * 8;
+  J.owner = J.lane >= halo && J.lane < J.nvalid + halo && J.ulane < D.u1;
+  J.need = J.lane <= J.nvalid + halo && J.ulane < D.u1 + 8;
   const int jlo = D.v0 >> 1, jhi = (D.v1 - 1) >> 1;
   J.jbeg = jlo + seg * (int)D.pairs_per_seg;
   J.jend = min(J.jbeg + (int)D.pairs_per_seg, jhi + 1);
@@ -185,11 +187,11 @@
   }
 }
 
-template <int NC>
-__device__ __forceinline__ void to_coeffs53(const DwtLevelDesc& D, int (&x)[NC][8])
+template <int NC, int N>
+__device__ __forceinline__ void to_coeffs53(const DwtLevelDesc& D, int (&x)[NC][N])
 {
   if(D.first_level)
-    rct_fwd<NC>(D, x);
+    rct_fwd<NC, N>(D, x);
 }
 
 template <int NC>
@@ -211,6 +213,30 @@
 __device__ __forceinline__ void fetch53(const DwtLevelDesc& D, const Job& J, int v, int (&out)[NC][8])
 {
   fetch_int_rows<NC>(D, J, v, out);
+  to_coeffs53<NC>(D, out);
+}
+
+struct GhostCol
+{
+  int col;
+  int slot;
+};
+__device__ __forceinline__ GhostCol ghost_col(const DwtLevelDesc& D, const Job& J)
+{
+  const int x0 = J.ulane - 8 * J.lane;
+  GhostCol G;
+  G.slot = J.lane == 0 ? 0 : J.lane == 1 ? 1 : J.lane == 31 ? 2 : -1;
+  const int x = J.lane == 0 ? x0 - 1 : J.lane == 1 ? x0 - 2 : J.lane == 31 ? x0 + 256 : J.ulane;
+  G.col = mirror_rel(x - D.u0, J.wn);
+  return G;
+}
+template <int NC>
+__device__ __forceinline__ void fetch_ghost53(const DwtLevelDesc& D, const Job& J, const GhostCol& G, int v, int (&out)[NC][1])
+{
+  const int r = mirror_rel(v - D.v0, J.hn);
+#pragma unroll
+  for(int c = 0; c < NC; ++c)
+    out[c][0] = __ldg(reinterpret_cast<const int32_t*>(D.in[c]) + (size_t)r * D.in_pitch + G.col);
   to_coeffs53<NC>(D, out);
 }
 
@@ -304,14 +330,18 @@
 }
 
 template <bool DEGEN = true>
-__device__ __forceinline__ void hfwd53(const int (&r)[8], int wn, int (&lo)[4], int (&hi)[4])
-{
-  const int en = __shfl_down_sync(0xffffffffu, r[0], 1);
+__device__ __forceinline__ void hfwd53(const int (&r)[8], int g, int wn, int (&lo)[4], int (&hi)[4])
+{
+  const int lane = threadIdx.x & 31;
+  const int g2 = __shfl_down_sync(0xffffffffu, g, 1);
+  const int rn = __shfl_down_sync(0xffffffffu, r[0], 1);
+  const int en = lane == 31 ? g : rn;
   hi[0] = r[1] - ((r[0] + r[2]) >> 1);
   hi[1] = r[3] - ((r[2] + r[4]) >> 1);
   hi[2] = r[5] - ((r[4] + r[6]) >> 1);
   hi[3] = r[7] - ((r[6] + en) >> 1);
-  const int dp = __shfl_up_sync(0xffffffffu, hi[3], 1);
+  const int hp = __shfl_up_sync(0xffffffffu, hi[3], 1);
+  const int dp = lane == 0 ? g - ((g2 + r[0]) >> 1) : hp;
   lo[0] = r[0] + ((dp + hi[0] + 2) >> 2);
   lo[1] = r[2] + ((hi[0] + hi[1] + 2) >> 2);
   lo[2] = r[4] + ((hi[1] + hi[2] + 2) >> 2);
@@ -423,6 +453,11 @@
 
 constexpr int DWT_STAGES = 3;
 
+struct NoSideFill
+{
+  __device__ __forceinline__ void operator()(uint8_t*, int) const {}
+};
+
 template <class Stage>
 struct WarpPipe
 {
@@ -440,8 +475,8 @@
         tlast(tlast_), tfill(tfirst_), bulk(bulk_)
   {
   }
-  template <class Bulk, class Async>
-  __device__ __forceinline__ void refill(const Bulk& fill_bulk, const Async& fill_async)
+  template <class Bulk, class Async, class Side = NoSideFill>
+  __device__ __forceinline__ void refill(const Bulk& fill_bulk, const Async& fill_async, const Side& fill_side = Side())
   {
     if(tfill <= tlast)
     {
@@ -451,18 +486,19 @@
       {
         if((threadIdx.x & 31) == 0)
         {
-          mbar_expect_tx(bars + slot, Stage::PAIRB);
+          mbar_expect_tx(bars + slot, Stage::BODYB);
           fill_bulk(st, tfill, bars + slot);
         }
       }
       else
         fill_async(st, tfill);
+      fill_side(st, tfill);
     }
     cp_async_commit();
     ++tfill;
   }
-  template <class Bulk, class Async>
-  __device__ __forceinline__ void prime(const Bulk& fill_bulk, const Async& fill_async)
+  template <class Bulk, class Async, class Side = NoSideFill>
+  __device__ __forceinline__ void prime(const Bulk& fill_bulk, const Async& fill_async, const Side& fill_side = Side())
   {
     if(bulk)
     {
@@ -477,17 +513,22 @@
     }
 #pragma unroll
     for(int s = 0; s < DWT_STAGES - 1; ++s)
-      refill(fill_bulk, fill_async);
-  }
-  template <class Bulk, class Async>
-  __device__ __forceinline__ const uint8_t* acquire(int t, const Bulk& fill_bulk, const Async& fill_async)
+      refill(fill_bulk, fill_async, fill_side);
+  }
+  template <class Bulk, class Async, class Side = NoSideFill>
+  __device__ __forceinline__ const uint8_t* acquire(int t, const Bulk& fill_bulk, const Async& fill_async,
+                                                    const Side& fill_side = Side())
   {
     if(Stage::COOPERATIVE || bulk)
       __syncwarp();
-    refill(fill_bulk, fill_async);
+    refill(fill_bulk, fill_async, fill_side);
     const int k = t - tfirst;
     if(bulk)
+    {
       mbar_wait(bars + k % DWT_STAGES, (unsigned)((k / DWT_STAGES) & 1));
+      if(Stage::GHOSTS)
+        cp_async_wait<DWT_STAGES - 1>();
+    }
     else
     {
       cp_async_wait<DWT_STAGES - 1>();
@@ -499,16 +540,19 @@
   __device__ __forceinline__ void drain() const { cp_async_wait<0>(); }
 };
 
-template <int NC>
+template <int NC, bool GHOSTS_ = false>
 struct RowStage
 {
   static constexpr int ROWB = 1024;
-  static constexpr int PAIRB = 2 * NC * ROWB;
+  static constexpr int BODYB = 2 * NC * ROWB;
+  static constexpr bool GHOSTS = GHOSTS_;
+  static constexpr int PAIRB = BODYB + (GHOSTS ? 2 * NC * 16 : 0);
   static constexpr bool COOPERATIVE = true;
   static __device__ __forceinline__ int swz(int k) { return k ^ ((k >> 3) & 1); }
 
+  template <class MCol>
   static __device__ __forceinline__ void fill(uint8_t* stage, int which, const DwtLevelDesc& D, const Job& J, int v,
-                                              bool fast, unsigned fastmask, const int (&mcol)[8])
+                                              bool fast, unsigned fastmask, const MCol& mcol)
   {
     const int r = mirror_rel(v - D.v0, J.hn);
     const int rel = J.ulane - D.u0;
@@ -532,11 +576,32 @@
 #pragma unroll
         for(int i = 0; i < 4; ++i)
         {
-          cp_async4(d0 + 4 * i, row + mcol[i]);
-          cp_async4(d1 + 4 * i, row + mcol[4 + i]);
+          cp_async4(d0 + 4 * i, row + mcol(i));
+          cp_async4(d1 + 4 * i, row + mcol(4 + i));
         }
       }
     }
+  }
+  static __device__ __forceinline__ void fill_ghost(uint8_t* stage, int which, const DwtLevelDesc& D, const Job& J, int v,
+                                                    const GhostCol& G)
+  {
+    static_assert(GHOSTS, "stage without ghost columns");
+    const int r = mirror_rel(v - D.v0, J.hn);
+#pragma unroll
+    for(int c = 0; c < NC; ++c)
+      if(G.slot >= 0)
+        cp_async4(stage + BODYB + (which * NC + c) * 16 + 4 * G.slot,
+                  reinterpret_cast<const int32_t*>(D.in[c]) + (size_t)r * D.in_pitch + G.col);
+  }
+  static __device__ __forceinline__ int2 ghost_at(const Job& J, const GhostCol& G)
+  {
+    return G.slot >= 0 ? make_int2(BODYB + 4 * G.slot, 16) : make_int2(32 * J.lane, ROWB);
+  }
+  static __device__ __forceinline__ void read_ghost(const uint8_t* stage, int which, int2 at, int (&out)[NC][1])
+  {
+#pragma unroll
+    for(int c = 0; c < NC; ++c)
+      out[c][0] = *reinterpret_cast<const int*>(stage + at.x + (which * NC + c) * at.y);
   }
   static __device__ __forceinline__ void fill_bulk(uint8_t* stage, int which, const DwtLevelDesc& D, const Job& J, int v, uint64_t* bar)
   {
@@ -583,29 +648,43 @@
 {
   const DwtLevelDesc& D = *dptr;
   const BandGeom g = band_geom(D);
-  int E[NC][8], DP[NC][8];
-  {
-    int A[NC][8], B[NC][8];
-    fetch53<NC>(D, J, 2 * J.jbeg - 2, A);
-    fetch53<NC>(D, J, 2 * J.jbeg - 1, B);
-    fetch53<NC>(D, J, 2 * J.jbeg, E);
-#pragma unroll
-    for(int c = 0; c < NC; ++c)
+  const GhostCol G = ghost_col(D, J);
+  int E[NC][9], DP[NC][9];
+  auto fetch = [&](int v, int (&x)[NC][9]) {
+    int b[NC][8], gh[NC][1];
+    fetch53<NC>(D, J, v, b);
+    fetch_ghost53<NC>(D, J, G, v, gh);
+#pragma unroll
+    for(int c = 0; c < NC; ++c)
+    {
 #pragma unroll
       for(int i = 0; i < 8; ++i)
+        x[c][i] = b[c][i];
+      x[c][8] = gh[c][0];
+    }
+  };
+  {
+    int A[NC][9], B[NC][9];
+    fetch(2 * J.jbeg - 2, A);
+    fetch(2 * J.jbeg - 1, B);
+    fetch(2 * J.jbeg, E);
+#pragma unroll
+    for(int c = 0; c < NC; ++c)
+#pragma unroll
+      for(int i = 0; i < 9; ++i)
         DP[c][i] = B[c][i] - ((A[c][i] + E[c][i]) >> 1);
   }
   for(int j = J.jbeg; j < J.jend; ++j)
   {
-    int O[NC][8], E2[NC][8];
-    fetch53<NC>(D, J, 2 * j + 1, O);
-    fetch53<NC>(D, J, 2 * j + 2, E2);
+    int O[NC][9], E2[NC][9];
+    fetch(2 * j + 1, O);
+    fetch(2 * j + 2, E2);
 #pragma unroll 1
     for(int c = 0; c < NC; ++c)
     {
-      int s[8], d[8];
-#pragma unroll
-      for(int i = 0; i < 8; ++i)
+      int s[9], d[9];
+#pragma unroll
+      for(int i = 0; i < 9; ++i)
       {
         d[i] = O[c][i] - ((E[c][i] + E2[c][i]) >> 1);
         s[i] = E[c][i] + ((DP[c][i] + d[i] + 2) >> 2);
@@ -617,23 +696,29 @@
         DP[c][i] = d[i];
         E[c][i] = E2[c][i];
       }
-      int lo[4], hi[4];
-      hfwd53<true>(s, J.wn, lo, hi);
+      int s8[8], d8[8], lo[4], hi[4];
+#pragma unroll
+      for(int i = 0; i < 8; ++i)
+      {
+        s8[i] = s[i];
+        d8[i] = d[i];
+      }
+      hfwd53<true>(s8, s[8], J.wn, lo, hi);
       store_rows(D, g, store_ctx(D, J, g), c, j, false, lo, hi);
-      hfwd53<true>(d, J.wn, lo, hi);
+      hfwd53<true>(d8, d[8], J.wn, lo, hi);
       store_rows(D, g, store_ctx(D, J, g), c, j, true, lo, hi);
     }
   }
 }
 
 template <int NC>
-__global__ void __launch_bounds__(B2K_WARPS_PER_CTA * 32) k_dwt53_fwd(const DwtLevelDesc* __restrict__ descs)
+__global__ void __launch_bounds__(B2K_WARPS_PER_CTA * 32, 3) k_dwt53_fwd(const DwtLevelDesc* __restrict__ descs)
 {
   extern __shared__ __align__(16) uint8_t smem_dwt[];
-  typedef RowStage<NC> RS;
+  typedef RowStage<NC, true> RS;
   const DwtLevelDesc D = descs[blockIdx.y];
   Job J;
-  if(!decode_job(D, J))
+  if(!decode_job<true>(D, J))
     return;
   if(J.hn == 1 || J.wn == 1)
   {
@@ -644,10 +729,8 @@
   const StoreCtx SC = store_ctx(D, J, g);
   const bool fast = RS::lane_fast(D, J);
   const unsigned fastmask = __ballot_sync(0xffffffffu, fast);
-  int mcol[8];
-#pragma unroll
-  for(int i = 0; i < 8; ++i)
-    mcol[i] = mirror_rel(J.ulane - D.u0 + i, J.wn);
+  const GhostCol G = ghost_col(D, J);
+  const int2 gat = RS::ghost_at(J, G);
 
   const int tfirst = J.jbeg - 1, tlast = J.jend - 1;
   WarpPipe<RS> pipe(smem_dwt, fastmask == 0xffffffffu, tfirst, tlast);
@@ -655,27 +738,40 @@
     RS::fill_bulk(st, 0, D, J, 2 * tf + 1, bar);
     RS::fill_bulk(st, 1, D, J, 2 * tf + 2, bar);
   };
+  auto mcol = [&](int i) { return mirror_rel(J.ulane - D.u0 + i, J.wn); };
   auto fill_async = [&](uint8_t* st, int tf) {
     RS::fill(st, 0, D, J, 2 * tf + 1, fast, fastmask, mcol);
     RS::fill(st, 1, D, J, 2 * tf + 2, fast, fastmask, mcol);
   };
-  pipe.prime(fill_bulk, fill_async);
-  int E[NC][8], DP[NC][8];
+  auto fill_ghost = [&](uint8_t* st, int tf) {
+    RS::fill_ghost(st, 0, D, J, 2 * tf + 1, G);
+    RS::fill_ghost(st, 1, D, J, 2 * tf + 2, G);
+  };
+  pipe.prime(fill_bulk, fill_async, fill_ghost);
+  int E[NC][8], DP[NC][8], gE[NC][1], gDP[NC];
   fetch53<NC>(D, J, 2 * tfirst, E);
+  fetch_ghost53<NC>(D, J, G, 2 * tfirst, gE);
 #pragma unroll
   for(int c = 0; c < NC; ++c)
+  {
 #pragma unroll
     for(int i = 0; i < 8; ++i)
       DP[c][i] = 0;
+    gDP[c] = 0;
+  }
 
   for(int t = tfirst; t <= tlast; ++t)
   {
-    const uint8_t* st = pipe.acquire(t, fill_bulk, fill_async);
-    int O[NC][8], E2[NC][8];
+    const uint8_t* st = pipe.acquire(t, fill_bulk, fill_async, fill_ghost);
+    int O[NC][8], E2[NC][8], gO[NC][1], gE2[NC][1];
     RS::read(st, 0, J, pipe.bulk, O);
     RS::read(st, 1, J, pipe.bulk, E2);
+    RS::read_ghost(st, 0, gat, gO);
+    RS::read_ghost(st, 1, gat, gE2);
     to_coeffs53<NC>(D, O);
     to_coeffs53<NC>(D, E2);
+    to_coeffs53<NC>(D, gO);
+    to_coeffs53<NC>(D, gE2);
     const bool emit = t >= J.jbeg;
 #pragma unroll
     for(int c = 0; c < NC; ++c)
@@ -689,12 +785,16 @@
         DP[c][i] = d[i];
         E[c][i] = E2[c][i];
       }
+      const int gd = gO[c][0] - ((gE[c][0] + gE2[c][0]) >> 1);
+      const int gs = gE[c][0] + ((gDP[c] + gd + 2) >> 2);
+      gDP[c] = gd;
+      gE[c][0] = gE2[c][0];
       if(emit)
       {
         int lo[4], hi[4];
-        hfwd53<false>(s, J.wn, lo, hi);
+        hfwd53<false>(s, gs, J.wn, lo, hi);
         store_rows(D, g, SC, c, t, false, lo, hi);
-        hfwd53<false>(d, J.wn, lo, hi);
+        hfwd53<false>(d, gd, J.wn, lo, hi);
         store_rows(D, g, SC, c, t, true, lo, hi);
       }
     }
@@ -765,7 +865,7 @@
   typedef RowStage<NC> RS;
   const DwtLevelDesc D = descs[blockIdx.y];
   Job J;
-  if(!decode_job(D, J))
+  if(!decode_job<false>(D, J))
     return;
   if(J.hn == 1 || J.wn == 1)
   {
@@ -789,9 +889,10 @@
     RS::fill_bulk(st, 0, D, J, 2 * tf + 1, bar);
     RS::fill_bulk(st, 1, D, J, 2 * tf + 2, bar);
   };
+  auto mc = [&](int i) { return mcol[i]; };
   auto fill_async = [&](uint8_t* st, int tf) {
-    RS::fill(st, 0, D, J, 2 * tf + 1, fast, fastmask, mcol);
-    RS::fill(st, 1, D, J, 2 * tf + 2, fast, fastmask, mcol);
+    RS::fill(st, 0, D, J, 2 * tf + 1, fast, fastmask, mc);
+    RS::fill(st, 1, D, J, 2 * tf + 2, fast, fastmask, mc);
   };
   pipe.prime(fill_bulk, fill_async);
   float Ev[NC][8], D1[NC][8], S1[NC][8], D2[NC][8];
@@ -879,16 +980,54 @@
   }
 }
 
+struct GhostBand
+{
+  int a, b;
+};
+__device__ __forceinline__ GhostBand ghost_band(const DwtLevelDesc& D, const Job& J, const BandGeom& g)
+{
+  const int x0 = J.ulane - 8 * J.lane;
+  const int ua = J.lane == 0 ? x0 - 1 : J.lane == 31 ? x0 + 257 : J.ulane + 1;
+  const int ub = J.lane == 31 ? x0 + 256 : J.ulane;
+  const int uam = D.u0 + mirror_rel(ua - D.u0, J.wn), ubm = D.u0 + mirror_rel(ub - D.u0, J.wn);
+  GhostBand G;
+  G.a = g.snx + (uam >> 1) - g.x0h;
+  G.b = (ubm >> 1) - g.x0l;
+  return G;
+}
+template <int NC>
+__device__ __forceinline__ void fetch_band_ghosts(const DwtLevelDesc& D, const Job& J, const BandGeom& g, const GhostBand& G,
+                                                  int j, bool vhigh, int (&ga)[NC], int (&gb)[NC])
+{
+  const int vm = D.v0 + mirror_rel(2 * j + (vhigh ? 1 : 0) - D.v0, J.hn);
+  const int jm = vm >> 1;
+#pragma unroll
+  for(int c = 0; c < NC; ++c)
+  {
+    ga[c] = gb[c] = 0;
+    if(J.wn == 1 || (vm & 1) != (vhigh ? 1 : 0))
+      continue;
+    const int32_t* lrow = !vhigh ? reinterpret_cast<const int32_t*>(D.out_ll[c]) + (size_t)(jm - g.y0l) * D.ll_pitch
+                                 : reinterpret_cast<const int32_t*>(D.out_c[c]) + (size_t)(g.sny + jm - g.y0h) * D.c_pitch;
+    const int32_t* hrow = !vhigh ? reinterpret_cast<const int32_t*>(D.out_c[c]) + (size_t)(jm - g.y0l) * D.c_pitch : lrow;
+    ga[c] = __ldg(hrow + G.a);
+    gb[c] = __ldg(lrow + G.b);
+  }
+}
+
 template <bool DEGEN = true>
-__device__ __forceinline__ void hinv53(const int (&lo)[4], const int (&hi)[4], int wn, int (&r)[8])
-{
-  const int dm = __shfl_up_sync(0xffffffffu, hi[3], 1);
+__device__ __forceinline__ void hinv53(const int (&lo)[4], const int (&hi)[4], int ga, int gb, int wn, int (&r)[8])
+{
+  const int lane = threadIdx.x & 31;
+  const int hp = __shfl_up_sync(0xffffffffu, hi[3], 1);
+  const int dm = lane == 0 ? ga : hp;
   int e[5];
   e[0] = lo[0] - ((dm + hi[0] + 2) >> 2);
   e[1] = lo[1] - ((hi[0] + hi[1] + 2) >> 2);
   e[2] = lo[2] - ((hi[1] + hi[2] + 2) >> 2);
   e[3] = lo[3] - ((hi[2] + hi[3] + 2) >> 2);
-  e[4] = __shfl_down_sync(0xffffffffu, e[0], 1);
+  const int en = __shfl_down_sync(0xffffffffu, e[0], 1);
+  e[4] = lane == 31 ? gb - ((hi[3] + ga + 2) >> 2) : en;
 #pragma unroll
   for(int i = 0; i < 4; ++i)
   {
@@ -1023,6 +1162,7 @@
 {
   const DwtLevelDesc& D = *dptr;
   const BandGeom g = band_geom(D);
+  const GhostBand G = ghost_band(D, J, g);
   int DV[NC][8], EP[NC][8];
 #pragma unroll
   for(int c = 0; c < NC; ++c)
@@ -1032,16 +1172,18 @@
 
   for(int t = J.jbeg - 1; t <= J.jend; ++t)
   {
-    int lo[NC][4], hi[NC][4];
+    int lo[NC][4], hi[NC][4], ga[NC], gb[NC];
     int sv[NC][8], dv[NC][8];
     fetch_band_rows<NC>(D, J, g, t, false, lo, hi);
-#pragma unroll
-    for(int c = 0; c < NC; ++c)
-      hinv53(lo[c], hi[c], J.wn, sv[c]);
+    fetch_band_ghosts<NC>(D, J, g, G, t, false, ga, gb);
+#pragma unroll
+    for(int c = 0; c < NC; ++c)
+      hinv53(lo[c], hi[c], ga[c], gb[c], J.wn, sv[c]);
     fetch_band_rows<NC>(D, J, g, t, true, lo, hi);
-#pragma unroll
-    for(int c = 0; c < NC; ++c)
-      hinv53(lo[c], hi[c], J.wn, dv[c]);
+    fetch_band_ghosts<NC>(D, J, g, G, t, true, ga, gb);
+#pragma unroll
+    for(int c = 0; c < NC; ++c)
+      hinv53(lo[c], hi[c], ga[c], gb[c], J.wn, dv[c]);
     int Er[NC][8], Or[NC][8];
 #pragma unroll
     for(int c = 0; c < NC; ++c)
@@ -1077,11 +1219,13 @@
 }
 
 
-template <int NC>
+template <int NC, bool WHOLE = false>
 struct BandStage
 {
   static constexpr int ROWB = 512;
-  static constexpr int PAIRB = 4 * NC * ROWB;
+  static constexpr int BODYB = 4 * NC * ROWB;
+  static constexpr bool GHOSTS = WHOLE;
+  static constexpr int PAIRB = BODYB + (GHOSTS ? 2 * NC * 16 : 0);
   static constexpr bool COOPERATIVE = false;
   struct Lane
   {
@@ -1090,16 +1234,23 @@
     int col[4];
     int mlo[4], mhi[4];
   };
+  static __device__ __forceinline__ int mirrored(const DwtLevelDesc& D, const Job& J, const BandGeom& g, int i, int odd)
+  {
+    const int u = D.u0 + mirror_rel(2 * ((J.ulane >> 1) + i) + odd - D.u0, J.wn);
+    return (u >> 1) - (odd ? g.x0h : g.x0l);
+  }
   static __device__ __forceinline__ void setup(const DwtLevelDesc& D, const Job& J, const BandGeom& g, Lane& L)
   {
     const int k0 = J.ulane >> 1;
     L.need = J.need;
-#pragma unroll
-    for(int i = 0; i < 4; ++i)
-    {
-      const int ul = D.u0 + mirror_rel(2 * (k0 + i) - D.u0, J.wn), uh = D.u0 + mirror_rel(2 * (k0 + i) + 1 - D.u0, J.wn);
-      L.mlo[i] = (ul >> 1) - g.x0l;
-      L.mhi[i] = (uh >> 1) - g.x0h;
+    if(!WHOLE)
+    {
+#pragma unroll
+      for(int i = 0; i < 4; ++i)
+      {
+        L.mlo[i] = mirrored(D, J, g, i, 0);
+        L.mhi[i] = mirrored(D, J, g, i, 1);
+      }
     }
     const bool in_lo = 2 * k0 >= D.u0 && 2 * k0 + 6 < D.u1, in_hi = 2 * k0 + 1 >= D.u0 && 2 * k0 + 7 < D.u1;
     const int clo = k0 - g.x0l, chi = k0 - g.x0h;
@@ -1135,10 +1286,46 @@
           const int base = (b & 1) ? g.snx : 0;
 #pragma unroll
           for(int i = 0; i < 4; ++i)
-            cp_async4(dst + 4 * i, src[b] + base + ((b & 1) ? L.mhi[i] : L.mlo[i]));
+          {
+            const int m = WHOLE ? mirrored(D, J, g, i, b & 1) : ((b & 1) ? L.mhi[i] : L.mlo[i]);
+            cp_async4(dst + 4 * i, src[b] + base + m);
+          }
         }
       }
     }
+  }
+  static __device__ __forceinline__ void fill_ghost(uint8_t* stage, const DwtLevelDesc& D, const Job& J, const BandGeom& g,
+                                                    const GhostBand& G, int t)
+  {
+    static_assert(GHOSTS, "stage without ghost samples");
+    const int jl = ((D.v0 + mirror_rel(2 * t - D.v0, J.hn)) >> 1), jh = ((D.v0 + mirror_rel(2 * t + 1 - D.v0, J.hn)) >> 1);
+    const bool right = J.lane == 31, on = J.lane == 0 || right;
+#pragma unroll
+    for(int c = 0; c < NC; ++c)
+    {
+      const int32_t* lsrc[2];
+      const int32_t* hsrc[2];
+      lsrc[0] = reinterpret_cast<const int32_t*>(D.out_ll[c]) + (jl - g.y0l) * (int)D.ll_pitch;
+      hsrc[0] = reinterpret_cast<const int32_t*>(D.out_c[c]) + (jl - g.y0l) * (int)D.c_pitch;
+      lsrc[1] = hsrc[1] = reinterpret_cast<const int32_t*>(D.out_c[c]) + (g.sny + jh - g.y0h) * (int)D.c_pitch;
+#pragma unroll
+      for(int v = 0; v < 2; ++v)
+      {
+        uint8_t* dst = stage + BODYB + (v * NC + c) * 16;
+        if(on)
+          cp_async4(dst + (right ? 8 : 0), hsrc[v] + G.a);
+        if(right)
+          cp_async4(dst + 12, lsrc[v] + G.b);
+      }
+    }
+  }
+  static __device__ __forceinline__ int2 ghost_at(const Job& J)
+  {
+    return J.lane == 0 ? make_int2(BODYB, 16) : J.lane == 31 ? make_int2(BODYB + 8, 16) : make_int2(16 * J.lane, ROWB);
+  }
+  static __device__ __forceinline__ int2 read_ghost(const uint8_t* stage, int2 at, int v, int c)
+  {
+    return *reinterpret_cast<const int2*>(stage + at.x + (v * NC + c) * at.y);
   }
   static __device__ __forceinline__ void fill_bulk(uint8_t* stage, const DwtLevelDesc& D, const Job& J, const BandGeom& g,
                                                    const Lane& L, int t, uint64_t* bar)
@@ -1169,13 +1356,13 @@
 };
 
 template <int NC>
-__global__ void __launch_bounds__(B2K_WARPS_PER_CTA * 32) k_dwt53_inv(const DwtLevelDesc* __restrict__ descs)
+__global__ void __launch_bounds__(B2K_WARPS_PER_CTA * 32, 3) k_dwt53_inv(const DwtLevelDesc* __restrict__ descs)
 {
   extern __shared__ __align__(16) uint8_t smem_dwt[];
-  typedef BandStage<NC> BS;
+  typedef BandStage<NC, true> BS;
   const DwtLevelDesc D = descs[blockIdx.y];
   Job J;
-  if(!decode_job(D, J))
+  if(!decode_job<true>(D, J))
     return;
   if(J.hn == 1 || J.wn == 1)
   {
@@ -1186,12 +1373,15 @@
   typename BS::Lane L;
   BS::setup(D, J, g, L);
   const OutCtx OC = out_ctx(D, J);
+  const GhostBand G = ghost_band(D, J, g);
+  const int2 gat = BS::ghost_at(J);
 
   const int tfirst = J.jbeg - 1, tlast = J.jend;
   WarpPipe<BS> pipe(smem_dwt, BS::all_fast(L), tfirst, tlast);
   auto fill_bulk = [&](uint8_t* st, int tf, uint64_t* bar) { BS::fill_bulk(st, D, J, g, L, tf, bar); };
   auto fill_async = [&](uint8_t* st, int tf) { BS::fill(st, D, J, g, L, tf); };
-  pipe.prime(fill_bulk, fill_async);
+  auto fill_ghost = [&](uint8_t* st, int tf) { BS::fill_ghost(st, D, J, g, G, tf); };
+  pipe.prime(fill_bulk, fill_async, fill_ghost);
   int DV[NC][8], EP[NC][8];
 #pragma unroll
   for(int c = 0; c < NC; ++c)
@@ -1201,7 +1391,7 @@
 
   for(int t = tfirst; t <= tlast; ++t)
   {
-    const uint8_t* st = pipe.acquire(t, fill_bulk, fill_async);
+    const uint8_t* st = pipe.acquire(t, fill_bulk, fill_async, fill_ghost);
     int Er[NC][8], Or[NC][8];
 #pragma unroll
     for(int c = 0; c < NC; ++c)
@@ -1209,10 +1399,12 @@
       int lo[4], hi[4], sv[8], dv[8];
       BS::read(st, J, 0, c, lo);
       BS::read(st, J, 1, c, hi);
-      hinv53<false>(lo, hi, J.wn, sv);
+      int2 gh = BS::read_ghost(st, gat, 0, c);
+      hinv53<false>(lo, hi, gh.x, gh.y, J.wn, sv);
       BS::read(st, J, 2, c, lo);
       BS::read(st, J, 3, c, hi);
-      hinv53<false>(lo, hi, J.wn, dv);
+      gh = BS::read_ghost(st, gat, 1, c);
+      hinv53<false>(lo, hi, gh.x, gh.y, J.wn, dv);
 #pragma unroll
       for(int i = 0; i < 8; ++i)
       {
@@ -1298,7 +1490,7 @@
   typedef BandStage<NC> BS;
   const DwtLevelDesc D = descs[blockIdx.y];
   Job J;
-  if(!decode_job(D, J))
+  if(!decode_job<false>(D, J))
     return;
   if(J.hn == 1 || J.wn == 1)
   {
@@ -1606,8 +1798,8 @@
   dim3 grid((max_jobs + B2K_WARPS_PER_CTA - 1) / B2K_WARPS_PER_CTA, ndesc), block(B2K_WARPS_PER_CTA * 32);
   if(!irreversible)
   {
-    if(nc == 3) launch_dwt<RowStage<3>, k_dwt53_fwd<3>>(grid, block, st, d);
-    else launch_dwt<RowStage<1>, k_dwt53_fwd<1>>(grid, block, st, d);
+    if(nc == 3) launch_dwt<RowStage<3, true>, k_dwt53_fwd<3>>(grid, block, st, d);
+    else launch_dwt<RowStage<1, true>, k_dwt53_fwd<1>>(grid, block, st, d);
   }
   else
   {
@@ -1706,8 +1898,8 @@
   dim3 grid((max_jobs + B2K_WARPS_PER_CTA - 1) / B2K_WARPS_PER_CTA, ndesc), block(B2K_WARPS_PER_CTA * 32);
   if(!irreversible)
   {
-    if(nc == 3) launch_dwt<BandStage<3>, k_dwt53_inv<3>>(grid, block, st, d);
-    else launch_dwt<BandStage<1>, k_dwt53_inv<1>>(grid, block, st, d);
+    if(nc == 3) launch_dwt<BandStage<3, true>, k_dwt53_inv<3>>(grid, block, st, d);
+    else launch_dwt<BandStage<1, true>, k_dwt53_inv<1>>(grid, block, st, d);
   }
   else
   {
diff --git a/grok_b200/csrc/engine.cu b/grok_b200/csrc/engine.cu
--- a/grok_b200/csrc/engine.cu
+++ b/grok_b200/csrc/engine.cu
@@ -438,11 +438,11 @@
   return (int64_t)v.size();
 }
 
-static void fill_strips(DwtLevelDesc& d, int pairs_per_seg)
+static void fill_strips(DwtLevelDesc& d, int pairs_per_seg, bool whole_warp)
 {
   const int span = d.u1 - (d.u0 & ~7);
-  const int nstrips = std::max(1, (span + 239) / 240);
-  int sw = (span + nstrips - 1) / nstrips;
+  const int nstrips = std::max(1, whole_warp ? (span + 255) / 256 : (span + 239) / 240);
+  int sw = whole_warp ? 256 : (span + nstrips - 1) / nstrips;
   sw = (sw + 7) & ~7;
   d.nstrips = (uint16_t)nstrips;
   d.strip_w = (uint16_t)sw;
@@ -578,7 +578,7 @@
             d.lo[k] = lo;
             d.hi[k] = hi;
           }
-          fill_strips(d, P);
+          fill_strips(d, P, !cp.irreversible);
           (group ? mctL : sglL).descs.push_back(d);
           const uint64_t samples = (uint64_t)r.w() * r.h() * nc;
           (group ? mctL : sglL).alg_bytes += samples * 8;
@@ -600,7 +600,7 @@
         {
           Pl >>= 1;
           for(DwtLevelDesc& d : LL->descs)
-            fill_strips(d, Pl);
+            fill_strips(d, Pl, !cp.irreversible);
         }
       }
       if(dir == 0)
```

Measured after the change: 14240, median of 6. +3.5%, better.
